# radiocosmology/cora

Hardware: AMD Instinct MI355X
Metric: sky-maps/sec (nside=1024, lmax=2048, 256 freq) (higher is better)
Workload: dtype f64

## Files before the change

### cora_amd/_lib.py

```python
import ctypes
import os

import numpy as np

_HERE = os.path.dirname(os.path.abspath(__file__))
LIB_PATH = os.environ.get("CORAHIP_LIB", os.path.join(_HERE, "libcorahip.so"))

c_int, c_double, c_void_p, c_size_t = ctypes.c_int, ctypes.c_double, ctypes.c_void_p, ctypes.c_size_t
c_u64, c_char_p = ctypes.c_uint64, ctypes.c_char_p
PTR = c_void_p

SIGNATURES = {
    "corahip_abi_version": (c_int, []),
    "corahip_abi_minor": (c_int, []),
    "corahip_last_error": (c_char_p, []),
    "corahip_device_count": (c_int, [ctypes.POINTER(c_int)]),
    "corahip_ctx_create": (c_int, [c_int, ctypes.POINTER(c_void_p)]),
    "corahip_ctx_destroy": (c_int, [c_void_p]),
    "corahip_ctx_set_stream": (c_int, [c_void_p, c_void_p]),
    "corahip_ctx_sync": (c_int, [c_void_p]),
    "corahip_timer_begin": (c_int, [c_void_p]),
    "corahip_timer_end": (c_int, [c_void_p, ctypes.POINTER(ctypes.c_float)]),
    "corahip_profile_enable": (c_int, [c_void_p, c_int]),
    "corahip_profile_get": (c_int, [c_void_p, c_char_p, ctypes.POINTER(c_double), ctypes.POINTER(c_int)]),
    "corahip_profile_reset": (c_int, [c_void_p]),
    "corahip_malloc": (c_int, [c_void_p, c_size_t, ctypes.POINTER(c_void_p)]),
    "corahip_free": (c_int, [c_void_p, c_void_p]),
    "corahip_memcpy_h2d": (c_int, [c_void_p, c_void_p, c_void_p, c_size_t]),
    "corahip_memcpy_d2h": (c_int, [c_void_p, c_void_p, c_void_p, c_size_t]),
    "corahip_clarray_table21cm": (c_int, [c_void_p, PTR, PTR, PTR, c_int, c_int, c_double, c_double, c_double,
                                          PTR, PTR, PTR, PTR, c_int, c_int, PTR, PTR, c_int, PTR]),
    "corahip_clarray_table21cm_pairs": (c_int, [c_void_p, PTR, PTR, PTR, c_int, c_int, c_double, c_double, c_double,
                                                PTR, PTR, PTR, PTR, c_int, c_int, PTR, PTR, c_int, c_int, c_int, c_int,
                                                PTR]),
    "corahip_clarray_pairs_finish": (c_int, [c_void_p, PTR, c_int, c_int, c_int, c_int, PTR]),
    "corahip_clarray_tables_pin": (c_int, [c_void_p, PTR, PTR, PTR, c_u64]),
    "corahip_aps_table21cm_points": (c_int, [c_void_p, PTR, PTR, PTR, c_int, c_int, c_double, c_double, c_double,
                                             ctypes.c_long, PTR, PTR, PTR, PTR, PTR, PTR, PTR]),
    "corahip_clarray_separable": (c_int, [c_void_p, PTR, c_int, PTR, c_int, c_int, PTR, PTR]),
    "corahip_romb_reduce": (c_int, [c_void_p, PTR, c_int, c_int, c_int, PTR, PTR]),
    "corahip_factor_batched": (c_int, [c_void_p, PTR, c_int, c_int, c_double, c_double, PTR, PTR]),
    "corahip_normals_philox": (c_int, [c_void_p, c_u64, c_int, c_int, PTR]),
    "corahip_normals_pcg64": (c_int, [c_void_p, ctypes.POINTER(c_u64), ctypes.POINTER(c_u64), ctypes.c_int64, PTR,
                                      ctypes.POINTER(c_u64)]),
    "corahip_normals_mt19937_legacy": (c_int, [c_void_p, c_void_p, ctypes.c_int64, PTR]),
    "corahip_glibc_exp": (c_int, [c_void_p, PTR, ctypes.c_int64, PTR]),
    "corahip_pcg64_advance": (c_int, [ctypes.POINTER(c_u64), ctypes.POINTER(c_u64), c_u64, ctypes.POINTER(c_u64)]),
    "corahip_draw_alm_philox": (c_int, [c_void_p, PTR, PTR, c_u64, c_int, c_int, c_int, c_int, PTR]),
    "corahip_draw_alm_philox_rows": (c_int, [c_void_p, PTR, PTR, c_u64, c_int, c_int, c_int, c_int, PTR]),
    "corahip_draw_alm": (c_int, [c_void_p, PTR, PTR, PTR, c_int, c_int, c_int, c_int, PTR]),
    "corahip_draw_alm_rows": (c_int, [c_void_p, PTR, PTR, PTR, c_int, c_int, c_int, c_int, PTR]),
    "corahip_draw_alm_numpy_prepare": (c_int, [c_void_p, c_void_p, c_int, c_int, c_size_t, ctypes.POINTER(c_void_p)]),
    "corahip_draw_alm_numpy_run": (c_int, [c_void_p, c_void_p, PTR, c_int, PTR, c_void_p, PTR]),
    "corahip_draw_alm_numpy": (c_int, [c_void_p, PTR, c_int, PTR, c_void_p, c_int, c_int, c_int, c_int, PTR, c_size_t]),
    "corahip_draw_alm_numpy_begin": (c_int, [c_void_p, PTR, c_int, PTR, c_void_p, c_int, c_int, c_int, c_int, PTR, c_size_t,
                                             ctypes.POINTER(c_void_p)]),
    "corahip_draw_alm_numpy_end": (c_int, [c_void_p, c_void_p, c_void_p]),
    "corahip_draw_alm_numpy_begin_set": (c_int, [c_void_p, PTR, PTR, c_void_p, c_int, c_int, c_void_p, PTR, c_size_t,
                                                 ctypes.POINTER(c_void_p)]),
    "corahip_draw_alm_philox_rows_set": (c_int, [c_void_p, PTR, PTR, c_u64, c_int, c_int, c_void_p, PTR]),
    "corahip_mkfullsky_workspace_bytes": (c_int, [c_void_p, c_int, c_int, c_int, c_int, c_int, ctypes.POINTER(c_size_t)]),
    "corahip_mkfullsky": (c_int, [c_void_p, c_void_p, PTR, c_int, c_void_p, c_int, c_int, c_int, PTR, c_void_p, c_size_t]),
    "corahip_shard_plan": (c_int, [c_int, c_int, c_int, c_int, PTR]),
    "corahip_factor_rows_pack": (c_int, [c_void_p, PTR, c_int, c_int, c_int, c_int, PTR]),
    "corahip_factor_rows_unpack": (c_int, [c_void_p, PTR, PTR, c_int, c_int, c_int, c_int, PTR]),
    "corahip_alm_dev_to_square": (c_int, [c_void_p, PTR, c_int, c_int, PTR]),
    "corahip_alm_packed_to_dev": (c_int, [c_void_p, PTR, c_int, c_int, PTR]),
    "corahip_sht_plan_create": (c_int, [c_void_p, c_int, c_int, ctypes.POINTER(c_void_p)]),
    "corahip_sht_plan_create_ex": (c_int, [c_void_p, c_int, c_int, c_int, ctypes.POINTER(c_void_p)]),
    "corahip_sht_plan_cut_exp": (c_int, [c_void_p, ctypes.POINTER(c_int)]),
    "corahip_sht_plan_k4_mfma_count": (c_int, [c_void_p, c_void_p, c_int, ctypes.POINTER(c_u64)]),
    "corahip_sht_plan_destroy": (c_int, [c_void_p, c_void_p]),
    "corahip_alm2map_workspace_bytes": (c_int, [c_void_p, c_int, ctypes.POINTER(c_size_t)]),
    "corahip_alm2map": (c_int, [c_void_p, c_void_p, PTR, c_int, PTR, c_void_p, c_size_t]),
    "corahip_map2alm_workspace_bytes": (c_int, [c_void_p, c_int, ctypes.POINTER(c_size_t)]),
    "corahip_map2alm": (c_int, [c_void_p, c_void_p, PTR, c_int, PTR, PTR, c_void_p, c_size_t]),
    "corahip_alm2map_spin2": (c_int, [c_void_p, c_void_p, PTR, c_int, PTR, c_void_p, c_size_t]),
    "corahip_spin2_ring_scale": (c_int, [c_void_p, c_void_p, PTR, c_int, PTR]),
    "corahip_spin2_combine": (c_int, [c_void_p, c_void_p, PTR, c_int, c_int, PTR, c_int]),
    "corahip_xi_table_average": (c_int, [c_void_p, PTR, PTR, PTR, c_int, c_int, c_double, c_double, PTR, c_int, PTR, PTR,
                                         c_int, c_int, PTR]),
    "corahip_ps_table21cm": (c_int, [c_void_p, PTR, PTR, PTR, c_int, c_int, c_double, PTR, c_int, PTR, c_int, c_double,
                                     PTR, PTR, PTR, PTR]),
    "corahip_dct1_workspace_bytes": (c_int, [ctypes.c_long, c_int, ctypes.POINTER(c_size_t)]),
    "corahip_dct1_rows": (c_int, [c_void_p, PTR, ctypes.c_long, c_int, c_double, c_void_p, c_size_t]),
    "corahip_legendre_project": (c_int, [c_void_p, PTR, PTR, c_int, c_int, PTR, ctypes.c_long, PTR]),
    "corahip_fft_c2c": (c_int, [c_void_p, PTR, c_int, PTR, c_int, c_int]),
    "corahip_irfftn": (c_int, [c_void_p, PTR, c_int, PTR, c_int, PTR]),
    "corahip_rfftn": (c_int, [c_void_p, PTR, c_int, PTR, c_int, PTR]),
    "corahip_randomfield_draw": (c_int, [c_void_p, PTR, ctypes.c_int64, ctypes.c_uint64, PTR]),
    "corahip_fg_mix": (c_int, [c_void_p, PTR, PTR, PTR, c_int, c_int, ctypes.c_int64, PTR]),
    "corahip_randomfield_irfftn": (c_int, [c_void_p, PTR, c_int, PTR, ctypes.c_uint64, PTR, PTR]),
    "corahip_spec_mul_real": (c_int, [c_void_p, PTR, PTR, ctypes.c_int64]),
    "corahip_cube_affine": (c_int, [c_void_p, PTR, PTR, PTR, PTR, PTR, c_int, ctypes.c_int64, PTR]),
    "corahip_raytrace_slices": (c_int, [c_void_p, PTR, c_int, c_int, c_int, PTR, PTR, PTR, PTR, c_double, c_double,
                                        c_int, c_int, c_int, PTR]),
    "corahip_healpix_neighbours": (c_int, [c_void_p, c_int, PTR]),
    "corahip_za_density_sph": (c_int, [c_void_p, PTR, PTR, PTR, PTR, c_int, c_int, c_double, c_double, PTR]),
    "corahip_der1_alm_prep": (c_int, [c_void_p, c_void_p, PTR, c_int, c_int, c_int, PTR]),
    "corahip_der1_combine": (c_int, [c_void_p, c_void_p, PTR, c_int, c_int, PTR, PTR, c_int, PTR, PTR]),
    "corahip_radial_gradient": (c_int, [c_void_p, PTR, PTR, PTR, c_int, ctypes.c_long, PTR]),
    "corahip_sht_plan_rings": (c_int, [c_void_p, PTR, PTR, PTR, PTR]),
    "corahip_sht_plan_ring_classes": (c_int, [c_void_p, PTR]),
    "corahip_sht_lambda": (c_int, [c_void_p, c_void_p, c_int, c_int, PTR]),
    "corahip_sht_lambda_entry": (c_int, [c_void_p, c_void_p, c_int, c_int, c_int, PTR]),
}


class CoraHipError(RuntimeError):

    status = 0


_lib = None


def load():
    global _lib
    if _lib is None:
        if not os.path.exists(LIB_PATH):
            raise ImportError(
                "cora_amd: %s not found. Build it with `make -C cora_amd/csrc` (needs hipcc, gfx950). "
                "There is no CPU fallback for the compute path." % LIB_PATH
            )
        try:
            import torch
        except ImportError:
            pass
        lib = ctypes.CDLL(LIB_PATH)
        for name, (res, args) in SIGNATURES.items():
            fn = getattr(lib, name)
            fn.restype = res
            fn.argtypes = args
        if lib.corahip_abi_version() != 1:
            raise ImportError("cora_amd: ABI version mismatch in %s" % LIB_PATH)
        _lib = lib
    return _lib


def pcg64_advance(state, inc, delta):
    M = 2**64 - 1
    st = (c_u64 * 2)((int(state) >> 64) & M, int(state) & M)
    ic = (c_u64 * 2)((int(inc) >> 64) & M, int(inc) & M)
    out = (c_u64 * 2)()
    _check(load().corahip_pcg64_advance(st, ic, c_u64(int(delta)), out))
    return (int(out[0]) << 64) | int(out[1])


def _check(rc):
    if rc != 0:
        msg = load().corahip_last_error()
        err = CoraHipError("libcorahip status %d: %s" % (rc, msg.decode() if msg else "?"))
        err.status = int(rc)
        raise err


def _torch():
    import torch

    return torch


class _MtState(ctypes.Structure):
    _fields_ = [("key", ctypes.c_uint32 * 624), ("pos", ctypes.c_int32), ("has_gauss", ctypes.c_int32), ("gauss", c_double)]


class _Rng(ctypes.Structure):
    _fields_ = [("kind", ctypes.c_int32), ("reserved", ctypes.c_int32), ("stream", c_void_p), ("seed", c_u64),
                ("state", c_u64 * 2), ("inc", c_u64 * 2), ("legacy", ctypes.POINTER(_MtState))]


class _ChanSet(ctypes.Structure):
    _fields_ = [("nchunks", ctypes.c_int32), ("chunk_nnu", ctypes.c_int32), ("nu0", ctypes.c_int32 * 2)]


def _chanset(chunks):
    cs = _ChanSet()
    chunks = [(int(a), int(n)) for a, n in chunks]
    if len(chunks) not in (1, 2) or (len(chunks) == 2 and chunks[0][1] != chunks[1][1]):
        raise ValueError("a channel set is one block or two equal chunks")
    cs.nchunks, cs.chunk_nnu = len(chunks), chunks[0][1]
    cs.nu0[0] = chunks[0][0]
    cs.nu0[1] = chunks[1][0] if len(chunks) == 2 else 0
    return cs


def _rng_struct(rng):
    r = _Rng()
    M = 2**64 - 1
    if rng[0] == "pcg64":
        r.kind = 2
        r.state[0], r.state[1] = (int(rng[1]) >> 64) & M, int(rng[1]) & M
        r.inc[0], r.inc[1] = (int(rng[2]) >> 64) & M, int(rng[2]) & M
        return r, None
    if rng[0] != "legacy" or rng[1]["bit_generator"] != "MT19937":
        raise ValueError("numpy stream on the device: ('pcg64', state, inc) or ('legacy', MT19937 state dict)")
    ms = _MtState()
    key = np.ascontiguousarray(rng[1]["state"]["key"], dtype=np.uint32)
    ctypes.memmove(ms.key, key.ctypes.data, 624 * 4)
    ms.pos, ms.has_gauss, ms.gauss = int(rng[1]["state"]["pos"]), int(rng[1]["has_gauss"]), float(rng[1]["gauss"])
    r.kind = 3
    r.legacy = ctypes.pointer(ms)
    return r, ms


class Context:

    def __init__(self, device=0):
        torch = _torch()
        self.lib = load()
        if not torch.cuda.is_available():
            raise CoraHipError(
                "cora_amd needs an AMD MI355X (gfx950) GPU: torch.cuda.is_available() is False "
                "and there is no CPU fallback"
            )
        self.device = torch.device("cuda", device)
        torch.cuda.set_device(self.device)
        h = c_void_p()
        _check(self.lib.corahip_ctx_create(device, ctypes.byref(h)))
        self.h = h
        self._plans = {}
        self._workspace = None
        self.use_current_stream()

    def use_current_stream(self):
        torch = _torch()
        s = torch.cuda.current_stream(self.device).cuda_stream
        _check(self.lib.corahip_ctx_set_stream(self.h, c_void_p(s)))

    def sync(self):
        _check(self.lib.corahip_ctx_sync(self.h))

    def timer_begin(self):
        _check(self.lib.corahip_timer_begin(self.h))

    def timer_end(self):
        ms = ctypes.c_float()
        _check(self.lib.corahip_timer_end(self.h, ctypes.byref(ms)))
        return float(ms.value)

    def profile_enable(self, on=True):
        _check(self.lib.corahip_profile_enable(self.h, 1 if on else 0))

    def profile_reset(self):
        _check(self.lib.corahip_profile_reset(self.h))

    def profile_get(self, name):
        ms, n = c_double(), c_int()
        _check(self.lib.corahip_profile_get(self.h, name.encode(), ctypes.byref(ms), ctypes.byref(n)))
        return float(ms.value), int(n.value)

    def empty(self, shape, dtype=None):
        torch = _torch()
        return torch.empty(shape, dtype=dtype or torch.float64, device=self.device)

    def to_device(self, a, dtype=np.float64):
        torch = _torch()
        a = np.ascontiguousarray(a, dtype=dtype)
        return torch.from_numpy(a).to(self.device)

    @staticmethod
    def _p(t):
        assert t.is_contiguous(), "device array must be contiguous"
        return c_void_p(t.data_ptr())

    def _f64(self, t):
        torch = _torch()
        assert t.dtype == torch.float64 and t.device == self.device
        return self._p(t)

    _PINNED_MIN_BYTES = 1 << 24

    @property
    def copy_stream(self):
        torch = _torch()
        if getattr(self, "_copy_stream", None) is None:
            self._copy_stream = torch.cuda.Stream(device=self.device)
        return self._copy_stream

    def to_host_async(self, t):
        torch = _torch()
        host = torch.empty(t.shape, dtype=t.dtype, pin_memory=True)
        ready = torch.cuda.Event()
        ready.record(torch.cuda.current_stream(self.device))
        cs = self.copy_stream
        cs.wait_event(ready)
        with torch.cuda.stream(cs):
            host.copy_(t, non_blocking=True)
            done = torch.cuda.Event()
            done.record(cs)
        t.record_stream(cs)
        return host, done

    def to_host(self, t):
        if t.numel() * t.element_size() < self._PINNED_MIN_BYTES:
            return t.cpu().numpy()
        host, done = self.to_host_async(t)
        done.synchronize()
        return host.numpy()

    def pin_tables(self, dd, dv, vv, generation):
        _check(self.lib.corahip_clarray_tables_pin(self.h, self._f64(dd), self._f64(dv), self._f64(vv), c_u64(int(generation))))

    def unpin_tables(self, generation=0):
        if self.h:
            _check(self.lib.corahip_clarray_tables_pin(self.h, None, None, None, c_u64(int(generation))))

    def clarray_table21cm(self, dd, dv, vv, kperpmin, kperpmax, kparmax, chi, pfd, f, b, F, zint, w, log10l):
        nl = log10l.numel()
        out = self.empty((nl, F, F))
        nkperp, nkpar = dd.shape
        _check(self.lib.corahip_clarray_table21cm(
            self.h, self._f64(dd), self._f64(dv), self._f64(vv), nkperp, nkpar, kperpmin, kperpmax, kparmax,
            self._f64(chi), self._f64(pfd), self._f64(f), self._f64(b), F, zint, self._f64(w), self._f64(log10l),
            nl, self._f64(out)))
        return out

    def clarray_table21cm_pairs(self, dd, dv, vv, kperpmin, kperpmax, kparmax, chi, pfd, f, b, F, zint, w, log10l,
                                pair_first, pair_step, l_block, nblocks=None):
        torch = _torch()
        nl = log10l.numel()
        npl = (F * (F + 1) // 2 + pair_step - 1) // pair_step
        nblk = (nl + l_block - 1) // l_block
        if nblocks is not None:
            assert nblocks >= nblk
            nblk = nblocks
        out = torch.zeros((nblk, npl, l_block), dtype=torch.float64, device=self.device)
        nkperp, nkpar = dd.shape
        _check(self.lib.corahip_clarray_table21cm_pairs(
            self.h, self._f64(dd), self._f64(dv), self._f64(vv), nkperp, nkpar, kperpmin, kperpmax, kparmax,
            self._f64(chi), self._f64(pfd), self._f64(f), self._f64(b), F, zint, self._f64(w), self._f64(log10l),
            nl, pair_first, pair_step, l_block, self._f64(out)))
        return out

    def clarray_pairs_finish(self, slabs, F, nl):
        nranks, npl, l_stride = slabs.shape
        assert npl == (F * (F + 1) // 2 + nranks - 1) // nranks and nl <= l_stride
        out = self.empty((nl, F, F))
        _check(self.lib.corahip_clarray_pairs_finish(self.h, self._f64(slabs), F, nranks, l_stride, nl, self._f64(out)))
        return out

    def aps_table21cm_points(self, dd, dv, vv, kperpmin, kperpmax, kparmax, lx, chi1, chi2, cdd, cdv, cvv):
        n = lx.numel()
        out = self.empty((n,))
        nkperp, nkpar = dd.shape
        _check(self.lib.corahip_aps_table21cm_points(
            self.h, self._f64(dd), self._f64(dv), self._f64(vv), nkperp, nkpar, kperpmin, kperpmax, kparmax, n,
            self._f64(lx), self._f64(chi1), self._f64(chi2), self._f64(cdd), self._f64(cdv), self._f64(cvv),
            self._f64(out)))
        return out

    def clarray_separable(self, al, bcov, F, zint, w):
        nl = al.numel()
        out = self.empty((nl, F, F))
        _check(self.lib.corahip_clarray_separable(self.h, self._f64(al), nl, self._f64(bcov), F, zint,
                                                  self._f64(w), self._f64(out)))
        return out

    def romb_reduce(self, clt, nl, F, zint, w):
        out = self.empty((nl, F, F))
        _check(self.lib.corahip_romb_reduce(self.h, self._f64(clt), nl, F, zint, self._f64(w), self._f64(out)))
        return out

    def ps_table21cm(self, kperp, kpar, spline=None, kstar=0.0, freq_window=0.0, dd=None):
        nkperp, nkpar = kperp.numel(), kpar.numel()
        dv, vv = self.empty((nkperp, nkpar)), self.empty((nkperp, nkpar))
        if dd is None:
            loglog, kx, ky, ky2 = spline
            dd = self.empty((nkperp, nkpar))
            _check(self.lib.corahip_ps_table21cm(self.h, self._f64(kx), self._f64(ky), self._f64(ky2), kx.numel(),
                                                 1 if loglog else 0, float(kstar), self._f64(kperp), nkperp,
                                                 self._f64(kpar), nkpar, float(freq_window), None, self._f64(dd),
                                                 self._f64(dv), self._f64(vv)))
        else:
            _check(self.lib.corahip_ps_table21cm(self.h, None, None, None, 0, 0, 0.0, self._f64(kperp), nkperp,
                                                 self._f64(kpar), nkpar, 0.0, self._f64(dd), None, self._f64(dv),
                                                 self._f64(vv)))
        return dd, dv, vv

    def dct1_rows(self, data, scale=1.0):
        nrows, n = data.shape
        b = c_size_t()
        _check(self.lib.corahip_dct1_workspace_bytes(nrows, n, ctypes.byref(b)))
        ws = self.workspace(int(b.value))
        _check(self.lib.corahip_dct1_rows(self.h, self._f64(data), nrows, n, float(scale), self._p(ws), int(b.value)))
        return data

    def factor_batched(self, C, jitter_rel=1e-14, eig_thresh=1e-16):
        torch = _torch()
        nl, F, F2 = C.shape
        assert F == F2
        T = self.empty((nl, F, F))
        info = torch.empty((nl,), dtype=torch.int32, device=self.device)
        _check(self.lib.corahip_factor_batched(self.h, self._f64(C), nl, F, jitter_rel, eig_thresh, self._f64(T),
                                               self._p(info)))
        return T, info

    def normals_philox(self, seed, lmax, F, out=None):
        n = 2 * F * (lmax + 1) * (lmax + 2) // 2
        g = out if out is not None else self.empty((n,))
        assert g.numel() >= n
        _check(self.lib.corahip_normals_philox(self.h, c_u64(int(seed) & (2**64 - 1)), lmax, F, self._f64(g)))
        return g

    def normals_pcg64(self, state, inc, n, out=None):
        g = out if out is not None else self.empty((n,))
        assert g.numel() >= n
        M = 2**64 - 1
        st = (c_u64 * 2)((int(state) >> 64) & M, int(state) & M)
        ic = (c_u64 * 2)((int(inc) >> 64) & M, int(inc) & M)
        nraw = c_u64(0)
        _check(self.lib.corahip_normals_pcg64(self.h, st, ic, int(n), self._f64(g), ctypes.byref(nraw)))
        return g, int(nraw.value)

    def glibc_exp(self, x):
        y = self.empty(tuple(x.shape))
        _check(self.lib.corahip_glibc_exp(self.h, self._f64(x), int(x.numel()), self._f64(y)))
        return y

    def normals_legacy(self, state, n, out=None):
        import numpy as np

        class MtState(ctypes.Structure):
            _fields_ = [("key", ctypes.c_uint32 * 624), ("pos", ctypes.c_int32), ("has_gauss", ctypes.c_int32),
                        ("gauss", c_double)]

        if state["bit_generator"] != "MT19937":
            raise ValueError("legacy stream on the device: MT19937 only")
        ms = MtState()
        key = np.ascontiguousarray(state["state"]["key"], dtype=np.uint32)
        ctypes.memmove(ms.key, key.ctypes.data, 624 * 4)
        ms.pos, ms.has_gauss, ms.gauss = int(state["state"]["pos"]), int(state["has_gauss"]), float(state["gauss"])
        g = out if out is not None else self.empty((n,))
        assert g.numel() >= n
        _check(self.lib.corahip_normals_mt19937_legacy(self.h, ctypes.byref(ms), int(n), self._f64(g)))
        new = {"bit_generator": "MT19937", "state": {"key": np.frombuffer(ms.key, dtype=np.uint32).copy(), "pos": int(ms.pos)},
               "has_gauss": int(ms.has_gauss), "gauss": float(ms.gauss)}
        return g, new

    def draw_alm(self, T, info, g, lmax, F, nu0=0, nnu=None, out=None):
        nnu = F if nnu is None else nnu
        nalm = (lmax + 1) * (lmax + 2) // 2
        G = (nnu + 3) // 4
        alm = out if out is not None else self.empty((nalm, G, 2, 4))
        _check(self.lib.corahip_draw_alm(self.h, self._f64(T), self._p(info) if info is not None else None,
                                         self._f64(g), lmax, F, nu0, nnu, self._f64(alm)))
        return alm

    def draw_alm_rows(self, T_rows, info, g, lmax, F, nu0, nnu, out=None):
        assert tuple(T_rows.shape) == (lmax + 1, nnu, F), T_rows.shape
        nalm = (lmax + 1) * (lmax + 2) // 2
        G = (nnu + 3) // 4
        alm = out if out is not None else self.empty((nalm, G, 2, 4))
        _check(self.lib.corahip_draw_alm_rows(self.h, self._f64(T_rows), self._p(info) if info is not None else None,
                                              self._f64(g), lmax, F, nu0, nnu, self._f64(alm)))
        return alm

    def draw_alm_numpy_prepare(self, rng, lmax, F, ring_bytes=0):
        r, ms = _rng_struct(rng)
        pend = c_void_p()
        _check(self.lib.corahip_draw_alm_numpy_prepare(self.h, ctypes.byref(r), int(lmax), int(F), int(ring_bytes), ctypes.byref(pend)))
        ctx = self

        class Prepared:
            rng_struct, mt_state, pending, shape, live = r, ms, pend, (int(lmax), int(F)), True

            def abort(self):
                if self.live:
                    self.live = False
                    _check(ctx.lib.corahip_draw_alm_numpy_end(ctx.h, self.pending, ctypes.byref(self.rng_struct)))

        return Prepared()

    def draw_alm_numpy(self, T, info, rng, lmax, F, nu0=0, nnu=None, out=None, rows=False, ring_bytes=0, defer=False,
                       chunks=None, prepared=None):
        import numpy as np

        if chunks is not None:
            rows, nu0, nnu = True, chunks[0][0], sum(c[1] for c in chunks)
        nnu = F if nnu is None else nnu
        assert tuple(T.shape) == ((lmax + 1, nnu, F) if rows else (lmax + 1, F, F)), T.shape
        nalm = (lmax + 1) * (lmax + 2) // 2
        alm = out if out is not None else self.empty((nalm, (nnu + 3) // 4, 2, 4))
        if prepared is not None:
            assert prepared.live and prepared.shape == (int(lmax), int(F)), "the prepared session is for another shape"
            r, ms, pend = prepared.rng_struct, prepared.mt_state, prepared.pending
            cs = _chanset(chunks if chunks is not None and len(chunks) > 1 else [(nu0, nnu)])
            prepared.live = False
            try:
                _check(self.lib.corahip_draw_alm_numpy_run(self.h, pend, self._f64(T), 1 if rows else 0,
                                                           self._p(info) if info is not None else None, ctypes.byref(cs), self._f64(alm)))
            except CoraHipError:
                self.lib.corahip_draw_alm_numpy_end(self.h, pend, ctypes.byref(r))
                raise
        else:
            r, ms = _rng_struct(rng)
            pend = c_void_p()
            if chunks is not None and len(chunks) > 1:
                cs = _chanset(chunks)
                _check(self.lib.corahip_draw_alm_numpy_begin_set(self.h, self._f64(T), self._p(info) if info is not None else None,
                                                                 ctypes.byref(r), lmax, F, ctypes.byref(cs), self._f64(alm),
                                                                 int(ring_bytes), ctypes.byref(pend)))
            else:
                _check(self.lib.corahip_draw_alm_numpy_begin(self.h, self._f64(T), 1 if rows else 0,
                                                             self._p(info) if info is not None else None, ctypes.byref(r), lmax,
                                                             F, nu0, nnu, self._f64(alm), int(ring_bytes), ctypes.byref(pend)))
        keep = [T, info, alm]

        def finish():
            _check(self.lib.corahip_draw_alm_numpy_end(self.h, pend, ctypes.byref(r)))
            keep.clear()
            if ms is not None:
                return {"bit_generator": "MT19937", "state": {"key": np.frombuffer(ms.key, dtype=np.uint32).copy(), "pos": int(ms.pos)},
                        "has_gauss": int(ms.has_gauss), "gauss": float(ms.gauss)}
            return (int(r.state[0]) << 64) | int(r.state[1])

        if defer:
            return alm, finish
        return alm, finish()

    def draw_alm_philox(self, T, info, seed, lmax, F, nu0=0, nnu=None, out=None):
        nnu = F if nnu is None else nnu
        nalm = (lmax + 1) * (lmax + 2) // 2
        G = (nnu + 3) // 4
        alm = out if out is not None else self.empty((nalm, G, 2, 4))
        _check(self.lib.corahip_draw_alm_philox(self.h, self._f64(T), self._p(info) if info is not None else None,
                                                c_u64(int(seed) & (2**64 - 1)), lmax, F, nu0, nnu, self._f64(alm)))
        return alm

    def draw_alm_philox_rows(self, T_rows, info, seed, lmax, F, nu0, nnu, out=None):
        assert tuple(T_rows.shape) == (lmax + 1, nnu, F), T_rows.shape
        nalm = (lmax + 1) * (lmax + 2) // 2
        G = (nnu + 3) // 4
        alm = out if out is not None else self.empty((nalm, G, 2, 4))
        _check(self.lib.corahip_draw_alm_philox_rows(self.h, self._f64(T_rows), self._p(info) if info is not None else None,
                                                     c_u64(int(seed) & (2**64 - 1)), lmax, F, nu0, nnu, self._f64(alm)))
        return alm

    def draw_alm_philox_chunks(self, T_rows, info, seed, lmax, F, chunks, out=None):
        nnu = sum(int(c[1]) for c in chunks)
        assert tuple(T_rows.shape) == (lmax + 1, nnu, F), T_rows.shape
        nalm = (lmax + 1) * (lmax + 2) // 2
        alm = out if out is not None else self.empty((nalm, (nnu + 3) // 4, 2, 4))
        cs = _chanset(chunks)
        _check(self.lib.corahip_draw_alm_philox_rows_set(self.h, self._f64(T_rows), self._p(info) if info is not None else None,
                                                         c_u64(int(seed) & (2**64 - 1)), lmax, F, ctypes.byref(cs),
                                                         self._f64(alm)))
        return alm

    def factor_rows_pack(self, T_local, l_stride, world):
        n_local, F, _ = T_local.shape
        send = self.empty((world, l_stride, F // world, F))
        _check(self.lib.corahip_factor_rows_pack(self.h, self._f64(T_local) if n_local else None, n_local, l_stride, F,
                                                 world, self._f64(send)))
        return send

    def factor_rows_unpack(self, recv, counts):
        world, l_stride, nnu, F = recv.shape
        cnt = (ctypes.c_int32 * world)(*[int(c) for c in counts])
        out = self.empty((int(sum(counts)), nnu, F))
        _check(self.lib.corahip_factor_rows_unpack(self.h, self._f64(recv), cnt, world, l_stride, nnu, F, self._f64(out)))
        return out

    def alm_dev_to_square(self, alm, lmax, nnu):
        torch = _torch()
        L = lmax + 1
        sq = torch.empty((nnu, 1, L, L), dtype=torch.complex128, device=self.device)
        _check(self.lib.corahip_alm_dev_to_square(self.h, self._f64(alm), lmax, nnu, self._p(sq)))
        return sq

    def alm_packed_to_dev(self, packed, lmax):
        torch = _torch()
        assert packed.dtype == torch.complex128
        nnu, nalm = packed.shape
        assert nalm == (lmax + 1) * (lmax + 2) // 2
        alm = self.empty((nalm, (nnu + 3) // 4, 2, 4))
        _check(self.lib.corahip_alm_packed_to_dev(self.h, self._p(packed), lmax, nnu, self._f64(alm)))
        return alm

    sht_cut_exp = 0

    def sht_plan(self, nside, lmax, cut_exp=None):
        cut = int(self.sht_cut_exp if cut_exp is None else cut_exp)
        key = (int(nside), int(lmax)) if cut == 0 else (int(nside), int(lmax), cut)
        if key not in self._plans:
            h = c_void_p()
            _check(self.lib.corahip_sht_plan_create_ex(self.h, key[0], key[1], cut, ctypes.byref(h)))
            self._plans[key] = h
        return self._plans[key]

    def k4_mfma_count(self, nside, lmax, nnu, cut_exp=None):
        n = c_u64()
        _check(self.lib.corahip_sht_plan_k4_mfma_count(self.h, self.sht_plan(nside, lmax, cut_exp), int(nnu), ctypes.byref(n)))
        return int(n.value)

    def alm2map_workspace_bytes(self, plan, nnu):
        b = c_size_t()
        _check(self.lib.corahip_alm2map_workspace_bytes(plan, nnu, ctypes.byref(b)))
        return int(b.value)

    def workspace(self, nbytes):
        torch = _torch()
        if self._workspace is None or self._workspace.numel() < nbytes:
            self._workspace = None
            self._workspace = torch.empty((nbytes,), dtype=torch.uint8, device=self.device)
        return self._workspace

    def alm2map(self, alm, nside, lmax, nnu, out=None, max_workspace_bytes=None, cut_exp=None):
        plan = self.sht_plan(nside, lmax, cut_exp)
        npix = 12 * nside * nside
        maps = out if out is not None else self.empty((nnu, npix))
        need = self.alm2map_workspace_bytes(plan, nnu)
        if max_workspace_bytes is not None:
            need = min(need, int(max_workspace_bytes))
        ws = self.workspace(need)
        _check(self.lib.corahip_alm2map(self.h, plan, self._f64(alm), nnu, self._f64(maps), self._p(ws), need))
        return maps

    def mkfullsky_fused(self, C, nside, rng, nu0=0, nnu=None, alms=False, workspace_bytes=None, workspace=None):
        torch = _torch()
        L, F = int(C.shape[0]), int(C.shape[1])
        lmax = L - 1
        nnu = F if nnu is None else nnu
        plan = self.sht_plan(nside, lmax)

        class MtState(ctypes.Structure):
            _fields_ = [("key", ctypes.c_uint32 * 624), ("pos", ctypes.c_int32), ("has_gauss", ctypes.c_int32),
                        ("gauss", c_double)]

        class Rng(ctypes.Structure):
            _fields_ = [("kind", ctypes.c_int32), ("reserved", ctypes.c_int32), ("stream", c_void_p), ("seed", c_u64),
                        ("state", c_u64 * 2), ("inc", c_u64 * 2), ("legacy", ctypes.POINTER(MtState))]

        r = Rng()
        M = 2**64 - 1
        kind = {"stream": 0, "philox": 1, "pcg64": 2, "legacy": 3}[rng[0]]
        ms = None
        if kind == 3:
            import numpy as np

            ms = MtState()
            key = np.ascontiguousarray(rng[1]["state"]["key"], dtype=np.uint32)
            ctypes.memmove(ms.key, key.ctypes.data, 624 * 4)
            ms.pos, ms.has_gauss, ms.gauss = int(rng[1]["state"]["pos"]), int(rng[1]["has_gauss"]), float(rng[1]["gauss"])
            r.legacy = ctypes.pointer(ms)
        r.kind = kind
        if kind == 0:
            r.stream = self._f64(rng[1])
        elif kind == 1:
            r.seed = int(rng[1]) & M
        elif kind == 2:
            r.state[0], r.state[1] = (int(rng[1]) >> 64) & M, int(rng[1]) & M
            r.inc[0], r.inc[1] = (int(rng[2]) >> 64) & M, int(rng[2]) & M
        b = c_size_t()
        _check(self.lib.corahip_mkfullsky_workspace_bytes(plan, F, nu0, nnu, kind, 1 if alms else 0, ctypes.byref(b)))
        need = int(b.value) if workspace_bytes is None else int(workspace_bytes)
        if workspace is None:
            ws = torch.empty((max(need, 1),), dtype=torch.uint8, device=self.device)
        else:
            ws = workspace
            assert ws.dtype == torch.uint8 and ws.device == self.device and ws.numel() >= need, (ws.numel(), need)
        out = (torch.empty((nnu, 1, L, L), dtype=torch.complex128, device=self.device) if alms
               else self.empty((nnu, 12 * nside * nside)))
        _check(self.lib.corahip_mkfullsky(self.h, plan, self._f64(C), F, ctypes.byref(r), nu0, nnu, 1 if alms else 0,
                                          c_void_p(out.data_ptr()), self._p(ws), need))
        if kind == 3:
            import numpy as np

            return out, {"bit_generator": "MT19937", "state": {"key": np.frombuffer(ms.key, dtype=np.uint32).copy(), "pos": int(ms.pos)},
                         "has_gauss": int(ms.has_gauss), "gauss": float(ms.gauss)}
        return out, ((int(r.state[0]) << 64) | int(r.state[1])) if kind == 2 else None

    def map2alm_workspace_bytes(self, plan, nnu):
        b = c_size_t()
        _check(self.lib.corahip_map2alm_workspace_bytes(plan, nnu, ctypes.byref(b)))
        return int(b.value)

    def map2alm(self, maps, nside, lmax, ring_w=None, chunk=None, out=None):
        torch = _torch()
        plan = self.sht_plan(nside, lmax)
        nnu, npix = maps.shape
        assert npix == 12 * nside * nside
        nalm = (lmax + 1) * (lmax + 2) // 2
        G4 = (nnu + 3) // 4
        if chunk is None:
            per8 = self.map2alm_workspace_bytes(plan, 8)
            chunk = max(8, min((int(96e9 // per8)) * 8, (nnu + 7) // 8 * 8))
        assert chunk % 8 == 0
        if out is None:
            out = self.empty((nalm, G4, 2, 4))
        assert tuple(out.shape) == (nalm, G4, 2, 4), out.shape
        for c0 in range(0, nnu, chunk):
            n = min(chunk, nnu - c0)
            G8 = (n + 7) // 8 * 2
            need = self.map2alm_workspace_bytes(plan, n)
            ws = self.workspace(need)
            part = out if (c0 == 0 and n == nnu and G8 == G4) else self.empty((nalm, G8, 2, 4))
            _check(self.lib.corahip_map2alm(self.h, plan, self._f64(maps[c0:c0 + n]), n,
                                            self._f64(ring_w) if ring_w is not None else None, self._f64(part),
                                            self._p(ws), need))
            if part is not out:
                g0 = c0 // 4
                gn = min(G8, G4 - g0)
                out[:, g0:g0 + gn].copy_(part[:, :gn])
        return out

    def alm2map_spin2(self, alm, nside, lmax, nnu, out=None):
        plan = self.sht_plan(nside, lmax)
        maps = out if out is not None else self.empty((nnu, 12 * nside * nside))
        need = self.alm2map_workspace_bytes(plan, nnu)
        ws = self.workspace(need)
        _check(self.lib.corahip_alm2map_spin2(self.h, plan, self._f64(alm), nnu, self._f64(maps), self._p(ws), need))
        return maps

    def map2alm_spin2(self, maps_qu, nside, lmax, ring_w=None, out=None):
        plan = self.sht_plan(nside, lmax)
        n2, npix = maps_qu.shape
        assert n2 % 2 == 0 and npix == 12 * nside * nside
        nf = n2 // 2
        nalm = (lmax + 1) * (lmax + 2) // 2
        maps6 = self.empty((6 * nf, npix))
        _check(self.lib.corahip_spin2_ring_scale(self.h, plan, self._f64(maps_qu), nf, self._f64(maps6)))
        a6 = self.map2alm(maps6, nside, lmax, ring_w)
        del maps6
        gout = (2 * nf + 7) // 8 * 2
        if out is None:
            out = self.empty((nalm, gout, 2, 4))
        assert tuple(out.shape) == (nalm, gout, 2, 4), out.shape
        _check(self.lib.corahip_spin2_combine(self.h, plan, self._f64(a6), a6.shape[1], nf, self._f64(out), gout))
        return out

    def der1_alm_prep(self, alm, nside, lmax, g0=0, g_in=None, out=None):
        plan = self.sht_plan(nside, lmax)
        nalm = (lmax + 1) * (lmax + 2) // 2
        G = int(alm.shape[1])
        g_in = G - g0 if g_in is None else int(g_in)
        assert tuple(alm.shape) == (nalm, G, 2, 4), alm.shape
        a3 = out if out is not None else self.empty((nalm, 3 * g_in, 2, 4))
        assert tuple(a3.shape) == (nalm, 3 * g_in, 2, 4), a3.shape
        _check(self.lib.corahip_der1_alm_prep(self.h, plan, self._f64(alm), G, int(g0), g_in, self._f64(a3)))
        return a3

    def der1_combine(self, maps3, nside, lmax, g_in, nfields, out_theta, out_phi, scale_theta=None, scale_phi=None,
                     phi_extra=0):
        plan = self.sht_plan(nside, lmax)
        npix = 12 * nside * nside
        assert tuple(maps3.shape) == (12 * g_in, npix), maps3.shape
        assert tuple(out_theta.shape) == (nfields, npix) and tuple(out_phi.shape) == (nfields, npix)
        for s in (scale_theta, scale_phi):
            assert s is None or s.numel() == nfields
        _check(self.lib.corahip_der1_combine(self.h, plan, self._f64(maps3), int(g_in), int(nfields),
                                             None if scale_theta is None else self._f64(scale_theta),
                                             None if scale_phi is None else self._f64(scale_phi), int(phi_extra),
                                             self._f64(out_theta), self._f64(out_phi)))
        return out_theta, out_phi

    def alm2map_der1_bytes(self, nside, lmax, nfields=16):
        g = (int(nfields) + 3) // 4
        nalm = (lmax + 1) * (lmax + 2) // 2
        ws = self.alm2map_workspace_bytes(self.sht_plan(nside, lmax), 12 * g)
        return nalm * 3 * g * 64 + 12 * g * 12 * nside * nside * 8 + ws

    def alm2map_der1(self, alm, nside, lmax, nnu, scale_theta=None, scale_phi=None, phi_extra=0, out=None,
                     max_bytes=None):
        npix = 12 * nside * nside
        G = int(alm.shape[1])
        assert 1 <= nnu <= 4 * G
        if out is None:
            out = (self.empty((nnu, npix)), self.empty((nnu, npix)))
        ot, op = out
        assert tuple(ot.shape) == (nnu, npix) and tuple(op.shape) == (nnu, npix)
        budget = self.alm2map_der1_bytes(nside, lmax, 16) if max_bytes is None else int(max_bytes)
        gall = (nnu + 3) // 4
        gc = gall
        while gc > 1 and self.alm2map_der1_bytes(nside, lmax, 4 * gc) > budget:
            gc -= 1
        plan = self.sht_plan(nside, lmax)
        for g0 in range(0, gall, gc):
            g = min(gc, gall - g0)
            f0, nf = 4 * g0, min(4 * g, nnu - 4 * g0)
            a3 = self.der1_alm_prep(alm, nside, lmax, g0, g)
            maps3 = self.empty((12 * g, npix))
            need = self.alm2map_workspace_bytes(plan, 12 * g)
            ws = self.workspace(need)
            _check(self.lib.corahip_alm2map(self.h, plan, self._f64(a3), 12 * g, self._f64(maps3), self._p(ws), need))
            del a3
            self.der1_combine(maps3, nside, lmax, g, nf, ot[f0:f0 + nf], op[f0:f0 + nf],
                              None if scale_theta is None else scale_theta[f0:f0 + nf],
                              None if scale_phi is None else scale_phi[f0:f0 + nf], phi_extra)
            del maps3
        return ot, op

    @staticmethod
    def gradient_coefficients(x):
        x = np.asarray(x, dtype=np.float64)
        n = x.size
        if x.ndim != 1 or n < 2:
            raise ValueError("gradient needs at least 2 coordinates along the axis (got shape %r)" % (x.shape,))
        d = np.diff(x)
        coef = np.zeros((n, 3))
        hs, hd = d[:-1], d[1:]
        coef[1:-1, 0] = -hd / (hs * (hd + hs))
        coef[1:-1, 1] = (hd - hs) / (hd * hs)
        coef[1:-1, 2] = hs / (hd * (hd + hs))
        coef[0, 1], coef[0, 2] = -1.0 / d[0], 1.0 / d[0]
        coef[-1, 0], coef[-1, 1] = -1.0 / d[-1], 1.0 / d[-1]
        return coef

    def radial_gradient(self, f, x, scale=None, out=None):
        torch = _torch()
        if f.dim() != 2:
            raise ValueError("radial_gradient takes a [n, npix] array (got %r)" % (tuple(f.shape),))
        n, npix = f.shape
        coef = self.gradient_coefficients(x)
        if coef.shape[0] != n:
            raise ValueError("x has %d entries, f %d rows" % (coef.shape[0], n))
        if out is None:
            out = self.empty((n, npix))
        if tuple(out.shape) != (n, npix):
            raise ValueError("out has shape %r, expected %r" % (tuple(out.shape), (n, npix)))
        nbytes = n * npix * 8
        if out.data_ptr() < f.data_ptr() + nbytes and f.data_ptr() < out.data_ptr() + nbytes:
            raise ValueError("radial_gradient: out overlaps f")
        if scale is not None and not isinstance(scale, torch.Tensor):
            scale = self.to_device(np.asarray(scale, dtype=np.float64))
        if scale is not None and scale.numel() != n:
            raise ValueError("scale has %d entries, f %d rows" % (scale.numel(), n))
        cdev = self.to_device(coef)
        _check(self.lib.corahip_radial_gradient(self.h, self._f64(f), self._f64(cdev),
                                                None if scale is None else self._f64(scale), int(n), int(npix),
                                                self._f64(out)))
        return out

    def xi_table_average(self, kx, ky, ky2, kind, x_t, f_t, mu, xa, xw, F, xint):
        nm = mu.numel()
        out = self.empty((nm, F, F))
        _check(self.lib.corahip_xi_table_average(self.h, self._f64(kx), self._f64(ky), self._f64(ky2), kx.numel(), kind,
                                                 float(x_t), float(f_t), self._f64(mu), nm, self._f64(xa), self._f64(xw),
                                                 F, xint, self._f64(out)))
        return out

    def legendre_project(self, mu, wt, lmax, xi):
        nm = mu.numel()
        ncol = xi.numel() // nm
        out = self.empty((lmax + 1, ncol))
        _check(self.lib.corahip_legendre_project(self.h, self._f64(mu), self._f64(wt), nm, lmax, self._f64(xi),
                                                 ncol, self._f64(out)))
        return out

    def _c128(self, t):
        torch = _torch()
        assert t.dtype == torch.complex128 and t.device == self.device
        return self._p(t)

    @staticmethod
    def _dims(shape):
        return (ctypes.c_int64 * len(shape))(*[int(x) for x in shape])

    def fft_c2c(self, data, axis, inverse=False):
        axis = axis % data.dim()
        _check(self.lib.corahip_fft_c2c(self.h, self._c128(data), data.dim(), self._dims(data.shape), axis,
                                        1 if inverse else 0))
        return data

    def irfftn(self, spec, naxes=None, last=None):
        nd = spec.dim()
        naxes = nd if naxes is None else naxes
        rshape = list(spec.shape)
        rshape[-1] = 2 * (spec.shape[-1] - 1) if last is None else int(last)
        if rshape[-1] // 2 + 1 != spec.shape[-1]:
            raise CoraHipError("irfftn: last axis %d does not match %d spectral bins" % (rshape[-1], spec.shape[-1]))
        out = self.empty(tuple(rshape))
        _check(self.lib.corahip_irfftn(self.h, self._c128(spec), nd, self._dims(rshape), naxes, self._f64(out)))
        return out

    def rfftn(self, arr, naxes=None):
        torch = _torch()
        nd = arr.dim()
        naxes = nd if naxes is None else naxes
        cshape = list(arr.shape)
        cshape[-1] = arr.shape[-1] // 2 + 1
        spec = torch.empty(tuple(cshape), dtype=torch.complex128, device=self.device)
        _check(self.lib.corahip_rfftn(self.h, self._f64(arr), nd, self._dims(arr.shape), naxes, self._c128(spec)))
        return spec

    def randomfield_draw(self, kweight, seed):
        torch = _torch()
        spec = torch.empty(tuple(kweight.shape), dtype=torch.complex128, device=self.device)
        _check(self.lib.corahip_randomfield_draw(self.h, self._f64(kweight), kweight.numel(), int(seed),
                                                 self._c128(spec)))
        return spec

    def randomfield_irfftn(self, kweight, seed, last=None, spec=None):
        torch = _torch()
        nd = kweight.dim()
        rshape = list(kweight.shape)
        rshape[-1] = 2 * (kweight.shape[-1] - 1) if last is None else int(last)
        if rshape[-1] // 2 + 1 != kweight.shape[-1]:
            raise CoraHipError("randomfield_irfftn: last axis %d does not match %d spectral bins" % (rshape[-1], kweight.shape[-1]))
        if spec is None:
            spec = torch.empty(tuple(kweight.shape), dtype=torch.complex128, device=self.device)
        out = self.empty(tuple(rshape))
        _check(self.lib.corahip_randomfield_irfftn(self.h, self._f64(kweight), nd, self._dims(rshape), int(seed) & (2**64 - 1),
                                                   self._c128(spec), self._f64(out)))
        return out

    def fg_mix(self, freq_weight, normals, aff):
        torch = _torch()
        F, ncorr = freq_weight.shape
        assert normals.shape[0] == ncorr and tuple(normals.shape[1:]) == tuple(aff.shape)
        out = torch.empty((F,) + tuple(aff.shape), dtype=torch.complex128, device=self.device)
        _check(self.lib.corahip_fg_mix(self.h, self._f64(freq_weight), self._f64(normals), self._c128(aff), F, ncorr,
                                       aff.numel(), self._c128(out)))
        return out

    def spec_mul_real(self, spec, weight):
        assert tuple(spec.shape) == tuple(weight.shape)
        _check(self.lib.corahip_spec_mul_real(self.h, self._c128(spec), self._f64(weight), spec.numel()))
        return spec

    def cube_affine(self, df, vf, a, b, c):
        n0 = df.shape[0]
        out = self.empty(tuple(df.shape))
        _check(self.lib.corahip_cube_affine(self.h, self._f64(df), None if vf is None else self._f64(vf), self._f64(a),
                                            None if vf is None else self._f64(b), self._f64(c), n0, df.numel() // n0,
                                            self._f64(out)))
        return out

    def raytrace_slices(self, cube, zc, scale, tx, ty, wx, wy):
        n0, n1, n2 = cube.shape
        numz, numx, numy = zc.numel(), tx.numel(), ty.numel()
        out = self.empty((numz, numx, numy))
        _check(self.lib.corahip_raytrace_slices(self.h, self._f64(cube), n0, n1, n2, self._f64(zc), self._f64(scale),
                                                self._f64(tx), self._f64(ty), float(wx), float(wy), numz, numx, numy,
                                                self._f64(out)))
        return out

    def healpix_neighbours(self, nside):
        torch = _torch()
        out = torch.empty((12 * int(nside) ** 2, 9), dtype=torch.int32, device=self.device)
        _check(self.lib.corahip_healpix_neighbours(self.h, int(nside), self._p(out)))
        return out

    def za_density_sph(self, psi, delta_bias, delta_m, chi, out, sigma_ang, sigma_chi):
        nchi, npix = delta_bias.shape
        nside = int(round((npix // 12) ** 0.5))
        _check(self.lib.corahip_za_density_sph(self.h, self._f64(psi), self._f64(delta_bias), self._f64(delta_m),
                                               self._f64(chi), int(nchi), nside, float(sigma_ang), float(sigma_chi),
                                               self._f64(out)))
        return out

    def sht_rings(self, nside, lmax):
        plan = self.sht_plan(nside, lmax)
        nring = 4 * nside - 1
        start = np.zeros(nring, dtype=np.int64)
        nphi = np.zeros(nring, dtype=np.int32)
        z = np.zeros(nring)
        phi0 = np.zeros(nring)
        _check(self.lib.corahip_sht_plan_rings(plan, start.ctypes.data_as(c_void_p), nphi.ctypes.data_as(c_void_p),
                                               z.ctypes.data_as(c_void_p), phi0.ctypes.data_as(c_void_p)))
        return dict(start=start, nphi=nphi, z=z, phi0=phi0)

    def sht_ring_classes(self, nside, lmax):
        cls = np.zeros(4 * nside - 1, dtype=np.int32)
        _check(self.lib.corahip_sht_plan_ring_classes(self.sht_plan(nside, lmax), cls.ctypes.data_as(c_void_p)))
        return cls

    def sht_lambda(self, nside, lmax, m, ring_pair):
        plan = self.sht_plan(nside, lmax)
        out = self.empty((lmax - m + 1,))
        _check(self.lib.corahip_sht_lambda(self.h, plan, m, ring_pair, self._f64(out)))
        return out

    def sht_lambda_entry(self, nside, lmax, m, ring_pair, kq):
        plan = self.sht_plan(nside, lmax)
        out = self.empty((lmax - m + 1,))
        _check(self.lib.corahip_sht_lambda_entry(self.h, plan, m, ring_pair, kq, self._f64(out)))
        return out


_contexts = {}


def get_context(device=None):
    torch = _torch()
    if device is None:
        device = torch.cuda.current_device() if torch.cuda.is_available() else 0
    if device not in _contexts:
        _contexts[device] = Context(device)
    ctx = _contexts[device]
    ctx.use_current_stream()
    return ctx
```

### cora_amd/csrc/clarray.hip

```cpp
#include "common.h"

#include <cstring>
#include <type_traits>

#ifndef CL_BUILD_BY_ROW
#define CL_BUILD_BY_ROW 1
#endif
#ifndef CL_BUILD_X4
#define CL_BUILD_X4 1
#endif
#ifndef CL_ABLATE
#define CL_ABLATE 0
#endif
#define CL_MAXZ 17

#define CL_XS 512
#define CL_LPT 9

__global__ void cl_transpose_kernel(const double *__restrict__ dd, const double *__restrict__ dv,
                                    const double *__restrict__ vv, int nkperp, int nkpar, double *__restrict__ tt) {
    __shared__ double tile[32][33];
    const double *src = blockIdx.z == 0 ? dd : (blockIdx.z == 1 ? dv : vv);
    double *dst = tt + (size_t)blockIdx.z * nkpar * CL_XS;
    const int x0 = blockIdx.y * 32, y0 = blockIdx.x * 32;
    const int tx = threadIdx.x & 31, ty = threadIdx.x >> 5;
    for (int r = ty; r < 32; r += 8) {
        const int x = x0 + r, y = y0 + tx;
        tile[r][tx] = (x < nkperp && y < nkpar) ? src[(size_t)x * nkpar + y] : 0.0;
    }
    __syncthreads();
    for (int r = ty; r < 32; r += 8) {
        const int y = y0 + r, x = x0 + tx;
        if (y < nkpar && x < CL_XS) dst[(size_t)y * CL_XS + x] = (x < nkperp) ? tile[tx][r] : 0.0;
    }
}

template <int ZINT>
__global__ void __launch_bounds__(256)
clarray21_kernel(const double *__restrict__ tt, int nkperp, int nkpar, double kperpmin, double xscale, double yscale,
                 const double *__restrict__ chi, const double *__restrict__ pfd, const double *__restrict__ fz,
                 const double *__restrict__ bz, int F, int zint_rt, const double *__restrict__ w,
                 const double *__restrict__ log10l, int nl, int l_base, const int2 *__restrict__ pairs,
                 double *__restrict__ scratch, int nl_total, int l_block) {
    const int zint = ZINT > 0 ? ZINT : zint_rt;
    extern __shared__ __attribute__((aligned(16))) double sm[];
    double *prof = sm;
    double *lxcs_s = sm + zint * (CL_XS + 2);
    double *par = lxcs_s + zint;
    int *ipar = reinterpret_cast<int *>(par + zint * zint * 8);
    const int PS = CL_XS + 2;
    const int tid = threadIdx.x;
    const int i = pairs[blockIdx.x].x, j = pairs[blockIdx.x].y;
    if (i < 0) return;
    const double ux = (double)nkperp - 1e-5, uy = (double)nkpar - 1e-5;
    const size_t tsz = (size_t)nkpar * CL_XS;

    double lxs[CL_LPT], acc[CL_LPT];
#pragma unroll
    for (int k = 0; k < CL_LPT; k++) {
        const int li = l_base + tid + 256 * k;
        lxs[k] = log10l[min(li, nl_total - 1)] * xscale;
        acc[k] = 0.0;
    }
    const int l_end = min(nl_total, l_base + 256 * CL_LPT);
    const double lx_lo = log10l[l_base] * xscale, lx_hi = log10l[l_end - 1] * xscale;
    const int kmax = (l_end - l_base + 255) / 256;

    int noclamp = 1;
    for (int t = tid; t < zint * zint; t += 256) {
        const int a = t / zint, b = t - a * zint;
        const int za = i * zint + a, zb = j * zint + b;
        const double x1 = chi[za], x2 = chi[zb];
        const double xc = 0.5 * (x1 + x2);
        const double lxc = log10(xc * kperpmin) * xscale;
        double yy = fabs(x2 - x1) * yscale;
        yy = yy < 0.0 ? 0.0 : (yy > uy ? uy : yy);
        int y0 = (int)yy;
        double wy = yy - (double)y0;
        if (y0 + 1 > nkpar - 1) {
            y0 = nkpar - 2;
            wy = 1.0;
        }
        const double W = w[a] * w[b] * pfd[za] * pfd[zb] / (xc * xc * M_PI);
        const double cdd = W * bz[za] * bz[zb];
        const double cdv = W * (fz[za] * bz[zb] + fz[zb] * bz[za]);
        const double cvv = W * fz[za] * fz[zb];
        double *pp = par + t * 8;
        pp[0] = cdd * (1.0 - wy);
        pp[1] = cdd * wy;
        pp[2] = cdv * (1.0 - wy);
        pp[3] = cdv * wy;
        pp[4] = cvv * (1.0 - wy);
        pp[5] = cvv * wy;
        pp[6] = lxc;
        double xhi = lx_hi - lxc, xlo = lx_lo - lxc;
        xhi = xhi < 0.0 ? 0.0 : (xhi > ux ? ux : xhi);
        xlo = xlo < 0.0 ? 0.0 : (xlo > ux ? ux : xlo);
        ipar[t * 4 + 0] = y0;
        ipar[t * 4 + 1] = (int)xlo;
        ipar[t * 4 + 2] = min((int)xhi + 2, nkperp);
        const double x2nd = (l_base + 1 < l_end ? log10l[l_base + 1] * xscale : lx_hi) - lxc;
        if (!(x2nd >= 0.0 && lx_hi - lxc <= ux)) noclamp = 0;
    }
    const bool all_fast = __syncthreads_and(noclamp) != 0;
    __shared__ int s_nsp;
    __shared__ double s_lxk[32];
    if (tid < 32) s_lxk[tid] = log10l[min(l_base + tid, nl_total - 1)] * xscale;
    if (tid < 64) {
        bool wide = false;
        if (l_base + tid + 1 < l_end) wide = (log10l[l_base + tid + 1] - log10l[l_base + tid]) * xscale >= 2.0;
        const unsigned long long m = __ballot(wide);
        if (tid == 0) s_nsp = m == ~0ull ? 32 : min(32, (int)__builtin_ctzll(~m));
    }

    for (int a = 0; a < zint; a++) {
        __syncthreads();
#if (CL_ABLATE == 0 || CL_ABLATE >= 3) && CL_BUILD_BY_ROW
        if (ZINT > 0 && all_fast) {
            constexpr int ZN = ZINT > 0 ? ZINT : 1;
            const int nsp = min(s_nsp, l_end - l_base);
            const double lxd = log10l[min(l_base + nsp, nl_total - 1)] * xscale;
            int xlo = nkperp, xhi = 0;
#pragma unroll
            for (int b = 0; b < ZN; b++) {
                const double xx = fmin(fmax(lxd - par[(a * ZN + b) * 8 + 6], 0.0), ux);
                xlo = min(xlo, (int)xx);
                xhi = max(xhi, ipar[(a * ZN + b) * 4 + 2]);
            }
            if (nsp >= l_end - l_base) xlo = xhi;
            auto row_of = [&](int b, int x, double (&v)[6]) {
                const double *r0 = tt + (size_t)ipar[(a * ZN + b) * 4 + 0] * CL_XS + x, *r1 = r0 + CL_XS;
                v[0] = r0[0];
                v[1] = r1[0];
                v[2] = r0[tsz];
                v[3] = r1[tsz];
                v[4] = r0[2 * tsz];
                v[5] = r1[2 * tsz];
            };
            auto combine = [&](int b, const double (&v)[6]) {
                const double *pp = par + (a * ZN + b) * 8;
                return pp[0] * v[0] + pp[1] * v[1] + pp[2] * v[2] + pp[3] * v[3] + pp[4] * v[4] + pp[5] * v[5];
            };
#if CL_BUILD_X4
            {
                constexpr int ZH = (ZN + 1) / 2;
                const int hb = tid >> 7, b0 = hb ? ZH : 0, nb = hb ? ZN - ZH : ZH;
                constexpr int QB = 3;
                for (int x = (xlo & ~1) + 2 * (tid & 127); x < xhi; x += 256) {
#pragma unroll
                    for (int q0 = 0; q0 < ZH; q0 += QB) {
                        double2 v[QB][6];
#pragma unroll
                        for (int q = 0; q < QB; q++) {
#if CL_ABLATE >= 3
                            if (q0 + q < nb) {
                                for (int i6 = 0; i6 < 6; i6++) v[q][i6] = make_double2((double)x, 1.0 + i6);
                            } else
#endif
                            if (q0 + q < nb) {
                                const double *r0 = tt + (size_t)ipar[(a * ZN + b0 + q0 + q) * 4 + 0] * CL_XS + x, *r1 = r0 + CL_XS;
                                v[q][0] = *reinterpret_cast<const double2 *>(r0);
                                v[q][1] = *reinterpret_cast<const double2 *>(r1);
                                v[q][2] = *reinterpret_cast<const double2 *>(r0 + tsz);
                                v[q][3] = *reinterpret_cast<const double2 *>(r1 + tsz);
                                v[q][4] = *reinterpret_cast<const double2 *>(r0 + 2 * tsz);
                                v[q][5] = *reinterpret_cast<const double2 *>(r1 + 2 * tsz);
                            }
                        }
#pragma unroll
                        for (int q = 0; q < QB; q++) {
                            if (q0 + q < nb) {
                                const double *pp = par + (a * ZN + b0 + q0 + q) * 8;
                                double2 o;
                                o.x = pp[0] * v[q][0].x + pp[1] * v[q][1].x + pp[2] * v[q][2].x + pp[3] * v[q][3].x + pp[4] * v[q][4].x + pp[5] * v[q][5].x;
                                o.y = pp[0] * v[q][0].y + pp[1] * v[q][1].y + pp[2] * v[q][2].y + pp[3] * v[q][3].y + pp[4] * v[q][4].y + pp[5] * v[q][5].y;
                                *reinterpret_cast<double2 *>(prof + (b0 + q0 + q) * PS + x) = o;
                            }
                        }
                    }
                }
            }
#else
            for (int x = xlo + tid; x < xhi; x += 256) {
                double v[ZN][6];
#pragma unroll
                for (int b = 0; b < ZN; b++) row_of(b, x, v[b]);
#pragma unroll
                for (int b = 0; b < ZN; b++) prof[b * PS + x] = combine(b, v[b]);
            }
#endif
            for (int e = tid; e < nsp * ZN; e += 256) {
                const int b = e % ZN, k = e / ZN;
                const double xx = fmin(fmax(s_lxk[k] - par[(a * ZN + b) * 8 + 6], 0.0), ux);
                const int x = (int)xx;
                typedef double d2u __attribute__((ext_vector_type(2), aligned(8)));
                const double *r0 = tt + (size_t)ipar[(a * ZN + b) * 4 + 0] * CL_XS + x, *r1 = r0 + CL_XS;
                const d2u t0 = *reinterpret_cast<const d2u *>(r0), t1 = *reinterpret_cast<const d2u *>(r1);
                const d2u t2 = *reinterpret_cast<const d2u *>(r0 + tsz), t3 = *reinterpret_cast<const d2u *>(r1 + tsz);
                const d2u t4 = *reinterpret_cast<const d2u *>(r0 + 2 * tsz), t5 = *reinterpret_cast<const d2u *>(r1 + 2 * tsz);
                const double v0[6] = {t0.x, t1.x, t2.x, t3.x, t4.x, t5.x};
                const double v1[6] = {t0.y, t1.y, t2.y, t3.y, t4.y, t5.y};
                const double p0 = combine(b, v0);
                prof[b * PS + x] = p0;
                prof[b * PS + x + 1] = x + 1 < nkperp ? combine(b, v1) : p0;
            }
            if (tid < ZN) lxcs_s[tid] = par[(a * ZN + tid) * 8 + 6];
            if (xhi == nkperp) {
                __syncthreads();
                if (tid < ZN) prof[tid * PS + nkperp] = prof[tid * PS + nkperp - 1];
            }
        } else
#endif
        for (int b = 0; b < zint; b++) {
            const int t = a * zint + b;
            const double *pp = par + t * 8;
            const double c0 = pp[0], c1 = pp[1], c2 = pp[2], c3 = pp[3], c4 = pp[4], c5 = pp[5];
            const int y0 = ipar[t * 4 + 0], x0r = ipar[t * 4 + 1], nx = ipar[t * 4 + 2];
            const double *r0 = tt + (size_t)y0 * CL_XS, *r1 = r0 + CL_XS;
            double *pb = prof + b * PS;
#if CL_ABLATE == 1
            for (int x = x0r + tid; x < nx; x += 256) pb[x] = c0 + c1 * x;
            (void)r0; (void)r1; (void)c2; (void)c3; (void)c4; (void)c5;
#else
            for (int x = x0r + tid; x < nx; x += 256)
                pb[x] = c0 * r0[x] + c1 * r1[x] + c2 * r0[tsz + x] + c3 * r1[tsz + x] + c4 * r0[2 * tsz + x] +
                        c5 * r1[2 * tsz + x];
#endif
            if (tid == 0) lxcs_s[b] = pp[6];
            if (nx == nkperp && tid == ((nkperp - 1 - x0r) & 255)) pb[nkperp] = pb[nkperp - 1];
        }
        __syncthreads();
        double lxc_r[ZINT > 0 ? ZINT : 1];
        if constexpr (ZINT > 0) {
#pragma unroll
            for (int b = 0; b < ZINT; b++) lxc_r[b] = lxcs_s[b];
        }
        auto interp = [&](int b, double lx, double lxc, bool clamp) {
            double xx = lx - lxc;
            if (clamp) xx = fmin(fmax(xx, 0.0), ux);
            const int x0 = (int)xx;
            const double wx = __builtin_amdgcn_fract(xx);
            const double *pr = prof + b * PS + x0;
            const double s0 = pr[0], s1 = pr[1];
            return fma(wx, s1 - s0, s0);
        };
        auto interp_all = [&](auto fast_c) {
            constexpr bool FAST = decltype(fast_c)::value;
#pragma unroll
            for (int k = 0; k < CL_LPT; k++) {
#if CL_ABLATE == 2 || CL_ABLATE == 4
                if (k >= 1) continue;
#endif
                if (k < kmax && (k < kmax - 1 || l_base + tid + 256 * k < nl_total)) {
                    const bool clamp = !FAST || (k == 0 && tid == 0);
                    double s = 0.0;
                    if constexpr (ZINT > 0) {
#pragma unroll
                        for (int b = 0; b < ZINT; b++) s += interp(b, lxs[k], lxc_r[b], clamp);
                    } else {
                        for (int b = 0; b < zint; b++) s += interp(b, lxs[k], lxcs_s[b], clamp);
                    }
                    acc[k] += s;
                }
            }
        };
        if (all_fast) interp_all(std::true_type{});
        else interp_all(std::false_type{});
    }
#pragma unroll
    for (int k = 0; k < CL_LPT; k++) {
        const int li = l_base + tid + 256 * k;
        if (li < nl_total)
            scratch[((size_t)(li / l_block) * gridDim.x + blockIdx.x) * l_block + li % l_block] = acc[k];
    }
}

#define CL_BAND 32
#ifndef CL_XCD_ORDER
#define CL_XCD_ORDER 1
#endif
__host__ __device__ static inline long cl_band_count(int n) {
    return n >= CL_BAND ? (long)CL_BAND * (n - (CL_BAND - 1)) + (long)(CL_BAND - 1) * CL_BAND / 2 : (long)n * (n + 1) / 2;
}
__host__ __device__ static inline int2 pair_of_index(long p, int F) {
    int B = 0;
    for (;; B++) {
        const long c = cl_band_count(F - CL_BAND * B);
        if (p < c) break;
        p -= c;
    }
    const int n = F - CL_BAND * B;
    const int nfull = n >= CL_BAND ? n - (CL_BAND - 1) : 0;
    int i, dd;
    if (p < (long)nfull * CL_BAND) {
#if CL_XCD_ORDER
        const int xq = (int)(p & 7), sq = (int)(p >> 3);
        i = sq >> 2;
        dd = 4 * xq + (sq & 3);
#else
        i = (int)(p / CL_BAND);
        dd = (int)(p % CL_BAND);
#endif
    } else {
        p -= (long)nfull * CL_BAND;
        int e = n >= CL_BAND ? CL_BAND - 1 : n;
        i = nfull;
        while (p >= e) {
            p -= e;
            e--;
            i++;
        }
        dd = (int)p;
    }
    return make_int2(i, i + CL_BAND * B + dd);
}

__global__ void cl_finish_kernel(const double *__restrict__ scratch, long npairs, int W, long npl, int lstride, int nl,
                                 int F, double *__restrict__ out) {
    __shared__ double tile[32][33];
    const long s0 = (long)blockIdx.x * 32;
    const int l0 = blockIdx.y * 32;
    const int tx = threadIdx.x & 31, ty = threadIdx.x >> 5;
    const long nslot = npl * W;
    for (int r = ty; r < 32; r += 8) {
        const long sl = s0 + r;
        const int l = l0 + tx;
        tile[r][tx] = (sl < nslot && l < nl) ? scratch[(size_t)sl * lstride + l] : 0.0;
    }
    __syncthreads();
    const long sl = s0 + tx;
    const long p = sl < nslot ? (sl % npl) * W + sl / npl : npairs;
    if (p >= npairs) return;
    const int2 ij = pair_of_index(p, F);
    for (int r = ty; r < 32; r += 8) {
        const int l = l0 + r;
        if (l < nl) {
            out[((size_t)l * F + ij.x) * F + ij.y] = tile[tx][r];
        }
    }
}

__global__ void cl_mirror_kernel(double *__restrict__ out, int F) {
    __shared__ double tile[32][33];
    const int nt = (F + 31) / 32;
    int ti = 0, rem = blockIdx.x;
    while (rem >= nt - ti) {
        rem -= nt - ti;
        ti++;
    }
    const int tj = ti + rem;
    double *o = out + (size_t)blockIdx.y * F * F;
    const int tx = threadIdx.x & 31, ty = threadIdx.x >> 5;
    for (int r = ty; r < 32; r += 8) {
        const int i = ti * 32 + r, j = tj * 32 + tx;
        tile[r][tx] = (i < F && j < F) ? o[(size_t)i * F + j] : 0.0;
    }
    __syncthreads();
    for (int r = ty; r < 32; r += 8) {
        const int j = tj * 32 + r, i = ti * 32 + tx;
        if (j < F && i < F && j > i) o[(size_t)j * F + i] = tile[tx][r];
    }
}
static int launch_mirror(corahip_ctx *ctx, double *out, int nl, int F) {
    const int nt = (F + 31) / 32;
    dim3 grid((unsigned)(nt * (nt + 1) / 2), (unsigned)nl);
    cl_mirror_kernel<<<grid, 256, 0, ctx->stream>>>(out, F);
    LAUNCH_CHECK();
    return 0;
}

__global__ void separable_kernel(const double *__restrict__ al, int nl, const double *__restrict__ bcov, int F, int zint,
                                 const double *__restrict__ w, double *__restrict__ out) {
    const long n = (long)nl * F * F;
    const int nz = F * zint;
    for (long q = (long)blockIdx.x * blockDim.x + threadIdx.x; q < n; q += (long)gridDim.x * blockDim.x) {
        const int j = (int)(q % F), i = (int)((q / F) % F);
        const long l = q / ((long)F * F);
        double s = 0.0;
        for (int a = 0; a < zint; a++) {
            double t = 0.0;
            for (int b = 0; b < zint; b++) t += w[b] * bcov[(size_t)(i * zint + a) * nz + j * zint + b];
            s += w[a] * t;
        }
        out[q] = al[l] * s;
    }
}

__global__ void romb_reduce_kernel(const double *__restrict__ clt, int nl, int F, int zint,
                                   const double *__restrict__ w, double *__restrict__ out) {
    const long n = (long)nl * F * F;
    for (long q = (long)blockIdx.x * blockDim.x + threadIdx.x; q < n; q += (long)gridDim.x * blockDim.x) {
        const int j = (int)(q % F), i = (int)((q / F) % F);
        const long l = q / ((long)F * F);
        const double *base = clt + (((size_t)l * F + i) * zint * F + j) * zint;
        double s = 0.0;
        for (int a = 0; a < zint; a++) {
            double t = 0.0;
            for (int b = 0; b < zint; b++) t += w[b] * base[(size_t)a * F * zint + b];
            s += w[a] * t;
        }
        out[q] = s;
    }
}

__global__ void aps21_points_kernel(const double *__restrict__ dd, const double *__restrict__ dv,
                                    const double *__restrict__ vv, int nkperp, int nkpar, double kperpmin,
                                    double xscale, double yscale, long n, const double *__restrict__ lx,
                                    const double *__restrict__ chi1, const double *__restrict__ chi2,
                                    const double *__restrict__ cdd, const double *__restrict__ cdv,
                                    const double *__restrict__ cvv, double *__restrict__ out) {
    const double ux = (double)nkperp - 1e-5, uy = (double)nkpar - 1e-5;
    for (long q = (long)blockIdx.x * blockDim.x + threadIdx.x; q < n; q += (long)gridDim.x * blockDim.x) {
        const double x1 = chi1[q], x2 = chi2[q];
        const double xc = 0.5 * (x1 + x2);
        double xx = (lx[q] - log10(xc * kperpmin)) * xscale;
        double yy = fabs(x2 - x1) * yscale;
        xx = xx < 0.0 ? 0.0 : (xx > ux ? ux : xx);
        yy = yy < 0.0 ? 0.0 : (yy > uy ? uy : yy);
        const int x0 = (int)xx, y0 = (int)yy;
        const double wx = xx - (double)x0, wy = yy - (double)y0;
        const int xb = min(x0 + 1, nkperp - 1), yb = min(y0 + 1, nkpar - 1);
        const size_t o00 = (size_t)x0 * nkpar + y0, o01 = (size_t)x0 * nkpar + yb;
        const size_t o10 = (size_t)xb * nkpar + y0, o11 = (size_t)xb * nkpar + yb;
        const double wa = (1.0 - wx) * (1.0 - wy), wb = (1.0 - wx) * wy, wc = wx * (1.0 - wy), wd = wx * wy;
        const double vdd = wa * dd[o00] + wb * dd[o01] + wc * dd[o10] + wd * dd[o11];
        const double vdv = wa * dv[o00] + wb * dv[o01] + wc * dv[o10] + wd * dv[o11];
        const double vvv = wa * vv[o00] + wb * vv[o01] + wc * vv[o10] + wd * vv[o11];
        out[q] = (cdd[q] * vdd + cdv[q] * vdv + cvv[q] * vvv) / (xc * xc * M_PI);
    }
}

extern "C" {

static int clarray21_pairs(corahip_ctx *ctx, const double *dd, const double *dv, const double *vv, int nkperp,
                           int nkpar, double kperpmin, double kperpmax, double kparmax, const double *chi,
                           const double *pfd, const double *f, const double *b, int F, int zint, const double *w,
                           const double *log10l, int nl, int pair_first, int pair_step, long npl_pad, int l_block,
                           double *out_pairs) {
    const size_t tt_bytes = sizeof(double) * 3 * (size_t)nkpar * CL_XS;
    double *tt = nullptr;
    int2 *dpairs = nullptr;
    int rc;
    if ((rc = corahip_ctx_scratch(ctx, 0, tt_bytes, (void **)&tt))) return rc;
    if ((rc = corahip_ctx_scratch(ctx, 2, sizeof(int2) * npl_pad, (void **)&dpairs))) return rc;
    const long key[4] = {F, pair_first, pair_step, npl_pad};
    if (ctx->pairs_ptr != (void *)dpairs || memcmp(key, ctx->pairs_key, sizeof(key)) != 0) {
        std::vector<int2> pairs((size_t)npl_pad, make_int2(-1, -1));
        long p = 0, k = 0;
        const long npairs_all = (long)F * (F + 1) / 2;
        for (; p < npairs_all; p++)
            if (p >= pair_first && (p - pair_first) % pair_step == 0) pairs[(size_t)k++] = pair_of_index(p, F);
        HIP_TRY(hipMemcpyAsync(dpairs, pairs.data(), sizeof(int2) * npl_pad, hipMemcpyHostToDevice, ctx->stream));
        HIP_TRY(hipStreamSynchronize(ctx->stream));
        memcpy(ctx->pairs_key, key, sizeof(key));
        ctx->pairs_ptr = (void *)dpairs;
    }
    const bool pinned = ctx->tt_pinned && ctx->tt_pin[0] == dd && ctx->tt_pin[1] == dv && ctx->tt_pin[2] == vv;
    if (!(pinned && ctx->tt_valid && ctx->tt_stream == ctx->stream && ctx->scratch_bytes[0] == tt_bytes)) {
        dim3 grid((nkpar + 31) / 32, CL_XS / 32, 3);
        cl_transpose_kernel<<<grid, 256, 0, ctx->stream>>>(dd, dv, vv, nkperp, nkpar, tt);
        LAUNCH_CHECK();
        ctx->tt_valid = pinned;
        ctx->tt_stream = ctx->stream;
    }
    const double xscale = (double)(nkperp - 1) / log10(kperpmax / kperpmin);
    const double yscale = kparmax / M_PI;
    const size_t shm = sizeof(double) * ((size_t)zint * (CL_XS + 2) + zint + (size_t)zint * zint * 10);
    auto kern = zint == 9 ? clarray21_kernel<9> : (zint == 5 ? clarray21_kernel<5> : (zint == 3 ? clarray21_kernel<3> : clarray21_kernel<0>));
    HIP_TRY(hipFuncSetAttribute((const void *)kern, hipFuncAttributeMaxDynamicSharedMemorySize, (int)shm));
    for (int l_base = 0; l_base < nl; l_base += 256 * CL_LPT) {
        kern<<<(unsigned)npl_pad, 256, shm, ctx->stream>>>(tt, nkperp, nkpar, kperpmin, xscale, yscale, chi, pfd, f, b, F, zint, w,
                                                          log10l, nl, l_base, dpairs, out_pairs, nl, l_block);
        LAUNCH_CHECK();
    }
    return 0;
}

int corahip_clarray_tables_pin(corahip_ctx *ctx, const double *dd, const double *dv, const double *vv, uint64_t generation) {
    ARG_CHECK(ctx != nullptr);
    if (dd == nullptr && generation != 0 && !(ctx->tt_pinned && ctx->tt_pin_gen == generation))
        return 0;
    const bool same = ctx->tt_pinned && dd && ctx->tt_pin[0] == dd && ctx->tt_pin[1] == dv && ctx->tt_pin[2] == vv &&
                      ctx->tt_pin_gen == generation;
    if (same) return 0;
    ctx->tt_pin[0] = dd;
    ctx->tt_pin[1] = dv;
    ctx->tt_pin[2] = vv;
    ctx->tt_pin_gen = generation;
    ctx->tt_pinned = dd != nullptr;
    ctx->tt_valid = false;
    return 0;
}

int corahip_clarray_table21cm(corahip_ctx *ctx, const double *dd, const double *dv, const double *vv, int nkperp,
                              int nkpar, double kperpmin, double kperpmax, double kparmax, const double *chi,
                              const double *pfd, const double *f, const double *b, int F, int zint, const double *w,
                              const double *log10l, int nl, double *out) {
    ARG_CHECK(ctx != nullptr && dd && dv && vv && chi && pfd && f && b && w && log10l && out);
    ARG_CHECK(nkperp >= 2 && nkperp < CL_XS && nkpar >= 2 && F >= 1 && zint >= 1 && zint <= CL_MAXZ && nl >= 1);
    ARG_CHECK(kperpmin > 0 && kperpmax > kperpmin && kparmax > 0);
    StageTimer t(ctx, "clarray");
    const long npairs = (long)F * (F + 1) / 2;
    double *scratch = nullptr;
    int rc;
    if ((rc = corahip_ctx_scratch(ctx, 1, sizeof(double) * (size_t)npairs * nl, (void **)&scratch))) return rc;
    if ((rc = clarray21_pairs(ctx, dd, dv, vv, nkperp, nkpar, kperpmin, kperpmax, kparmax, chi, pfd, f, b, F, zint, w,
                              log10l, nl, 0, 1, npairs, nl, scratch)))
        return rc;
    dim3 grid((unsigned)((npairs + 31) / 32), (nl + 31) / 32);
    cl_finish_kernel<<<grid, 256, 0, ctx->stream>>>(scratch, npairs, 1, npairs, nl, nl, F, out);
    LAUNCH_CHECK();
    return launch_mirror(ctx, out, nl, F);
}

int corahip_clarray_table21cm_pairs(corahip_ctx *ctx, const double *dd, const double *dv, const double *vv, int nkperp,
                                    int nkpar, double kperpmin, double kperpmax, double kparmax, const double *chi,
                                    const double *pfd, const double *f, const double *b, int F, int zint,
                                    const double *w, const double *log10l, int nl, int pair_first, int pair_step,
                                    int l_block, double *out_pairs) {
    ARG_CHECK(ctx != nullptr && dd && dv && vv && chi && pfd && f && b && w && log10l && out_pairs);
    ARG_CHECK(nkperp >= 2 && nkperp < CL_XS && nkpar >= 2 && F >= 1 && zint >= 1 && zint <= CL_MAXZ && nl >= 1);
    ARG_CHECK(kperpmin > 0 && kperpmax > kperpmin && kparmax > 0);
    ARG_CHECK(pair_step >= 1 && pair_first >= 0 && pair_first < pair_step && l_block >= 1);
    StageTimer t(ctx, "clarray");
    const long npairs = (long)F * (F + 1) / 2;
    const long npl = (npairs + pair_step - 1) / pair_step;
    return clarray21_pairs(ctx, dd, dv, vv, nkperp, nkpar, kperpmin, kperpmax, kparmax, chi, pfd, f, b, F, zint, w,
                           log10l, nl, pair_first, pair_step, npl, l_block, out_pairs);
}

int corahip_clarray_pairs_finish(corahip_ctx *ctx, const double *pairs_in, int F, int nranks, int l_stride, int nl,
                                 double *out) {
    ARG_CHECK(ctx != nullptr && pairs_in && out && F >= 1 && nranks >= 1 && nl >= 1 && l_stride >= nl);
    StageTimer t(ctx, "clarray");
    const long npairs = (long)F * (F + 1) / 2;
    const long npl = (npairs + nranks - 1) / nranks;
    dim3 grid((unsigned)((npl * nranks + 31) / 32), (nl + 31) / 32);
    cl_finish_kernel<<<grid, 256, 0, ctx->stream>>>(pairs_in, npairs, nranks, npl, l_stride, nl, F, out);
    LAUNCH_CHECK();
    return launch_mirror(ctx, out, nl, F);
}

int corahip_clarray_separable(corahip_ctx *ctx, const double *al, int nl, const double *bcov, int F, int zint,
                              const double *w, double *out) {
    ARG_CHECK(ctx != nullptr && al && bcov && w && out && nl >= 1 && F >= 1 && zint >= 1);
    StageTimer t(ctx, "clarray");
    const long n = (long)nl * F * F;
    separable_kernel<<<(int)std::min<long>((n + 255) / 256, 4096), 256, 0, ctx->stream>>>(al, nl, bcov, F, zint, w, out);
    LAUNCH_CHECK();
    return 0;
}

int corahip_romb_reduce(corahip_ctx *ctx, const double *clt, int nl, int F, int zint, const double *w, double *out) {
    ARG_CHECK(ctx != nullptr && clt && w && out && nl >= 1 && F >= 1 && zint >= 1);
    StageTimer t(ctx, "clarray");
    const long n = (long)nl * F * F;
    romb_reduce_kernel<<<(int)std::min<long>((n + 255) / 256, 4096), 256, 0, ctx->stream>>>(clt, nl, F, zint, w, out);
    LAUNCH_CHECK();
    return 0;
}

int corahip_aps_table21cm_points(corahip_ctx *ctx, const double *dd, const double *dv, const double *vv, int nkperp,
                                 int nkpar, double kperpmin, double kperpmax, double kparmax, long n,
                                 const double *lx, const double *chi1, const double *chi2, const double *cdd,
                                 const double *cdv, const double *cvv, double *out) {
    ARG_CHECK(ctx != nullptr && dd && dv && vv && lx && chi1 && chi2 && cdd && cdv && cvv && out);
    ARG_CHECK(nkperp >= 2 && nkpar >= 2 && n >= 1 && kperpmin > 0 && kperpmax > kperpmin && kparmax > 0);
    StageTimer t(ctx, "clarray");
    const double xscale = (double)(nkperp - 1) / log10(kperpmax / kperpmin);
    const double yscale = kparmax / M_PI;
    aps21_points_kernel<<<(int)std::min<long>((n + 255) / 256, 4096), 256, 0, ctx->stream>>>(
        dd, dv, vv, nkperp, nkpar, kperpmin, xscale, yscale, n, lx, chi1, chi2, cdd, cdv, cvv, out);
    LAUNCH_CHECK();
    return 0;
}

}
```

### cora_amd/csrc/factor.hip

```cpp
#include "common.h"

#include <algorithm>
#include <vector>

#define CH_NB 32

__global__ void __launch_bounds__(256)
chol_kernel(const double *__restrict__ C, int F, double jitter_rel, double *__restrict__ T,
            int32_t *__restrict__ info) {
    extern __shared__ __attribute__((aligned(16))) double lds[];
    double *D = lds;
    double *PA = lds + CH_NB * (CH_NB + 1);
    double *PB = PA + 64 * (CH_NB + 1);
    double *red = PB + 64 * (CH_NB + 1);
    int *flag = reinterpret_cast<int *>(red + 256);

    const int tid = threadIdx.x;
    const size_t off = (size_t)blockIdx.x * F * F;
    const double *A = C + off;
    double *Tl = T + off;

    double dmax = -INFINITY;
    for (int i = tid; i < F; i += 256) dmax = fmax(dmax, A[(size_t)i * F + i]);
    red[tid] = dmax;
    if (tid == 0) *flag = 0;
    __syncthreads();
    for (int s = 128; s > 0; s >>= 1) {
        if (tid < s) red[tid] = fmax(red[tid], red[tid + s]);
        __syncthreads();
    }
    const double jit = red[0] * jitter_rel;
    __syncthreads();
    for (long q = tid; q < (long)F * F; q += 256) {
        const int i = (int)(q / F), j = (int)(q % F);
        double v = 0.0;
        if (j <= i) v = A[q] + (i == j ? jit : 0.0);
        Tl[q] = v;
    }
    __syncthreads();

    for (int kb = 0; kb < F; kb += CH_NB) {
        const int nb = min(CH_NB, F - kb);
        for (int q = tid; q < nb * nb; q += 256) {
            const int i = q / nb, j = q % nb;
            D[i * (CH_NB + 1) + j] = (j <= i) ? Tl[(size_t)(kb + i) * F + kb + j] : 0.0;
        }
        __syncthreads();
        if (tid < 64) {
            const int lane = tid;
            double row[CH_NB];
#pragma unroll
            for (int k = 0; k < CH_NB; k++) row[k] = (lane < nb && k <= lane) ? D[lane * (CH_NB + 1) + k] : 0.0;
            bool bad = false;
#pragma unroll
            for (int j = 0; j < CH_NB; j++) {
                if (j < nb && !bad) {
                    const double d = __shfl(row[j], j);
                    if (!(d > 0.0)) {
                        bad = true;
                    } else {
                        const double lij = row[j] / sqrt(d);
                        row[j] = lane == j ? sqrt(d) : lij;
#pragma unroll
                        for (int k = j + 1; k < CH_NB; k++) row[k] -= lij * __shfl(lij, k);
                    }
                }
            }
#pragma unroll
            for (int k = 0; k < CH_NB; k++)
                if (lane < nb && k <= lane) D[lane * (CH_NB + 1) + k] = row[k];
            if (bad && lane == 0) *flag = 1;
        }
        __syncthreads();
        if (*flag) break;
        for (int q = tid; q < nb * nb; q += 256) {
            const int i = q / nb, j = q % nb;
            if (j <= i) Tl[(size_t)(kb + i) * F + kb + j] = D[i * (CH_NB + 1) + j];
        }
        const int r0 = kb + nb;
        if (r0 >= F) break;
        for (int r = r0 + tid; r < F; r += 256) {
            double x[CH_NB];
            double *row = Tl + (size_t)r * F + kb;
#pragma unroll
            for (int j = 0; j < CH_NB; j++) x[j] = j < nb ? row[j] : 0.0;
#pragma unroll
            for (int j = 0; j < CH_NB; j++) {
                if (j < nb) {
                    double s = x[j];
#pragma unroll
                    for (int p = 0; p < CH_NB; p++)
                        if (p < j) s -= x[p] * D[j * (CH_NB + 1) + p];
                    x[j] = s / D[j * (CH_NB + 1) + j];
                }
            }
#pragma unroll
            for (int j = 0; j < CH_NB; j++)
                if (j < nb) row[j] = x[j];
        }
        __syncthreads();
        const int nt = (F - r0 + 63) / 64;
        for (int ti = 0; ti < nt; ti++) {
            const int i0 = r0 + ti * 64;
            for (int q = tid; q < 64 * CH_NB; q += 256) {
                const int rr = q / CH_NB, cc = q % CH_NB;
                PA[rr * (CH_NB + 1) + cc] = (i0 + rr < F && cc < nb) ? Tl[(size_t)(i0 + rr) * F + kb + cc] : 0.0;
            }
            for (int tj = 0; tj <= ti; tj++) {
                const int j0 = r0 + tj * 64;
                for (int q = tid; q < 64 * CH_NB; q += 256) {
                    const int rr = q / CH_NB, cc = q % CH_NB;
                    PB[rr * (CH_NB + 1) + cc] = (j0 + rr < F && cc < nb) ? Tl[(size_t)(j0 + rr) * F + kb + cc] : 0.0;
                }
                const int ty = tid >> 4, tx = tid & 15;
                double old[4][4];
#pragma unroll
                for (int u = 0; u < 4; u++)
#pragma unroll
                    for (int w = 0; w < 4; w++) {
                        const int i = i0 + ty + 16 * u, j = j0 + tx + 16 * w;
                        old[u][w] = (i < F && j <= i) ? Tl[(size_t)i * F + j] : 0.0;
                    }
                __syncthreads();
                double acc[4][4] = {};
                for (int p = 0; p < CH_NB; p++) {
                    double a[4], b[4];
#pragma unroll
                    for (int u = 0; u < 4; u++) {
                        a[u] = PA[(ty + 16 * u) * (CH_NB + 1) + p];
                        b[u] = PB[(tx + 16 * u) * (CH_NB + 1) + p];
                    }
#pragma unroll
                    for (int u = 0; u < 4; u++)
#pragma unroll
                        for (int w = 0; w < 4; w++) acc[u][w] += a[u] * b[w];
                }
#pragma unroll
                for (int u = 0; u < 4; u++)
#pragma unroll
                    for (int w = 0; w < 4; w++) {
                        const int i = i0 + ty + 16 * u, j = j0 + tx + 16 * w;
                        if (i < F && j <= i) Tl[(size_t)i * F + j] = old[u][w] - acc[u][w];
                    }
                __syncthreads();
            }
        }
    }
    if (tid == 0) info[blockIdx.x] = *flag;
}

#define CHM_S 34
#ifndef CHM_STAMPS
#define CHM_STAMPS 0
#endif
#if CHM_STAMPS
__device__ unsigned long long g_chm_stamps[8];
#define CSTAMP(k) { unsigned long long _t; asm volatile("s_memtime %0\n\ts_waitcnt lgkmcnt(0)" : "=s"(_t)::"memory"); c_acc[k] += _t - c_last; c_last = _t; }
#else
#define CSTAMP(k)
#endif
#ifndef CHM_ABLATE
#define CHM_ABLATE 0
#endif

template <bool TALL>
__global__ void __launch_bounds__(256)
chol_ll_kernel(const double *__restrict__ C, int F, double jitter_rel, double *__restrict__ T,
               int32_t *__restrict__ info) {
    extern __shared__ __attribute__((aligned(16))) double lds[];
    double *D = lds;
    double *red = lds + CH_NB * (CH_NB + 1);
    int *flag = reinterpret_cast<int *>(red + 256);
    double *rdiag = red + 256 + 2;
    double *stage = rdiag + CH_NB;

    const int tid = threadIdx.x, lane = tid & 63, wave = tid >> 6;
    const int ri = lane & 15, kq = lane >> 4;
    const size_t off = (size_t)blockIdx.x * F * F;
    const double *A = C + off;
    double *Tl = T + off;
    double *PA = stage + (size_t)wave * (TALL ? 1 : 2) * 32 * CHM_S, *PB = PA + 32 * CHM_S;
    double *PBS = stage + 4 * 32 * CHM_S;

    double dmax = -INFINITY;
    for (int i = tid; i < F; i += 256) dmax = fmax(dmax, A[(size_t)i * F + i]);
    red[tid] = dmax;
    if (tid == 0) *flag = 0;
    __syncthreads();
    for (int s = 128; s > 0; s >>= 1) {
        if (tid < s) red[tid] = fmax(red[tid], red[tid + s]);
        __syncthreads();
    }
    const double jit = red[0] * jitter_rel;
    __syncthreads();

#if CHM_STAMPS
    unsigned long long c_acc[8] = {0, 0, 0, 0, 0, 0, 0, 0}, c_last;
    { unsigned long long _t; asm volatile("s_memtime %0\n\ts_waitcnt lgkmcnt(0)" : "=s"(_t)::"memory"); c_last = _t; }
#endif
    const int nblk = (F + 31) / 32;
    const int srow = lane >> 1, scol = 16 * (lane & 1);
    auto load_block = [&](int row0, int col0, double2 (&v)[8]) {
        const double *src = Tl + (size_t)(row0 + srow < F ? row0 + srow : 0) * F + col0 + scol;
#pragma unroll
        for (int q = 0; q < 8; q++) v[q] = *reinterpret_cast<const double2 *>(src + 2 * q);
    };
    auto store_block = [&](double *P, const double2 (&v)[8], double sign, int row0) {
        const double sg = row0 + srow < F ? sign : 0.0;
#pragma unroll
        for (int q = 0; q < 8; q++)
            *reinterpret_cast<double2 *>(P + srow * CHM_S + scol + 2 * q) = make_double2(sg * v[q].x, sg * v[q].y);
    };

    for (int j = 0; j < nblk; j++) {
        const int kb = 32 * j;
        const int nb = min(CH_NB, F - kb);
        if (TALL) {
            const int ntile = (nblk - j + 1) / 2;
            const int nround = (ntile + 3) / 4;
            const int brow = 8 * wave + (lane >> 3), bcol = 4 * (lane & 7);
            auto load_bq = [&](int col0, double2 (&v)[2]) {
                const double *src = Tl + (size_t)(kb + brow < F ? kb + brow : 0) * F + col0 + bcol;
                v[0] = *reinterpret_cast<const double2 *>(src);
                v[1] = *reinterpret_cast<const double2 *>(src + 2);
            };
            auto store_bq = [&](double *P, const double2 (&v)[2]) {
                const double sg = kb + brow < F ? 1.0 : 0.0;
                *reinterpret_cast<double2 *>(P + brow * CHM_S + bcol) = make_double2(sg * v[0].x, sg * v[0].y);
                *reinterpret_cast<double2 *>(P + brow * CHM_S + bcol + 2) = make_double2(sg * v[1].x, sg * v[1].y);
            };
            for (int u = 0; u < nround; u++) {
                const int t = wave + 4 * u;
                const bool has = t < ntile;
                const int i0 = 32 * (j + 2 * t);
                d4_t acc[4][2];
#pragma unroll
                for (int a = 0; a < 4; a++)
#pragma unroll
                    for (int b = 0; b < 2; b++)
#pragma unroll
                        for (int r = 0; r < 4; r++) {
                            const int row = i0 + 16 * a + kq + 4 * r, col = kb + 16 * b + ri;
                            double v = 0.0;
                            if (has && row < F && col <= row) v = A[(size_t)row * F + col] + (row == col ? jit : 0.0);
                            acc[a][b][r] = v;
                        }
                if (j > 0 && CHM_ABLATE != 3) {
                    double2 va0[8], va1[8], vb[2];
                    if (has) {
                        load_block(i0, 0, va0);
                        load_block(i0 + 32, 0, va1);
                    }
                    load_bq(0, vb);
                    for (int k = 0; k < j; k++) {
                        double *PBc = PBS + (k & 1) * 32 * CHM_S;
                        store_bq(PBc, vb);
                        __syncthreads();
                        if (k + 1 < j) load_bq(32 * (k + 1), vb);
                        if (has) {
                            store_block(PA, va0, -1.0, i0);
                            if (k + 1 < j) load_block(i0, 32 * (k + 1), va0);
#pragma unroll
                            for (int s = 0; s < 8; s++) {
                                double af[2], bf[2];
#pragma unroll
                                for (int a = 0; a < 2; a++) {
                                    af[a] = PA[(16 * a + ri) * CHM_S + 4 * s + kq];
                                    bf[a] = PBc[(16 * a + ri) * CHM_S + 4 * s + kq];
                                }
#pragma unroll
                                for (int a = 0; a < 2; a++)
#pragma unroll
                                    for (int b = 0; b < 2; b++)
                                        acc[a][b] = __builtin_amdgcn_mfma_f64_16x16x4f64(af[a], bf[b], acc[a][b], 0, 0, 0);
                            }
                            store_block(PA, va1, -1.0, i0 + 32);
                            if (k + 1 < j) load_block(i0 + 32, 32 * (k + 1), va1);
#pragma unroll
                            for (int s = 0; s < 8; s++) {
                                double af[2], bf[2];
#pragma unroll
                                for (int a = 0; a < 2; a++) {
                                    af[a] = PA[(16 * a + ri) * CHM_S + 4 * s + kq];
                                    bf[a] = PBc[(16 * a + ri) * CHM_S + 4 * s + kq];
                                }
#pragma unroll
                                for (int a = 0; a < 2; a++)
#pragma unroll
                                    for (int b = 0; b < 2; b++)
                                        acc[2 + a][b] = __builtin_amdgcn_mfma_f64_16x16x4f64(af[a], bf[b], acc[2 + a][b], 0, 0, 0);
                            }
                        }
                    }
                    __syncthreads();
                }
                if (has) {
#pragma unroll
                    for (int hb = 0; hb < 2; hb++) {
                        const int r0b = i0 + 32 * hb;
                        if (r0b >= F) continue;
                        if (t == 0 && hb == 0) {
#pragma unroll
                            for (int a = 0; a < 2; a++)
#pragma unroll
                                for (int b = 0; b < 2; b++)
#pragma unroll
                                    for (int r = 0; r < 4; r++)
                                        D[(16 * a + kq + 4 * r) * (CH_NB + 1) + 16 * b + ri] = acc[a][b][r];
                        } else {
#pragma unroll
                            for (int a = 0; a < 2; a++)
#pragma unroll
                                for (int b = 0; b < 2; b++)
#pragma unroll
                                    for (int r = 0; r < 4; r++) {
                                        const int row = r0b + 16 * a + kq + 4 * r, col = kb + 16 * b + ri;
                                        if (row < F && col < F) Tl[(size_t)row * F + col] = acc[2 * hb + a][b][r];
                                    }
                            if (kb + srow < F) {
                                double *z = Tl + (size_t)(kb + srow) * F + r0b + scol;
#pragma unroll
                                for (int q = 0; q < 8; q++)
                                    if (r0b + scol + 2 * q < F) *reinterpret_cast<double2 *>(z + 2 * q) = make_double2(0.0, 0.0);
                            }
                        }
                    }
                }
            }
        } else
        for (int i = j + wave; i < nblk; i += 4) {
            const int i0 = 32 * i;
            d4_t acc[2][2];
#pragma unroll
            for (int a = 0; a < 2; a++)
#pragma unroll
                for (int b = 0; b < 2; b++)
#pragma unroll
                    for (int r = 0; r < 4; r++) {
                        const int row = i0 + 16 * a + kq + 4 * r, col = kb + 16 * b + ri;
                        double v = 0.0;
                        if (row < F && col <= row) v = A[(size_t)row * F + col] + (row == col ? jit : 0.0);
                        acc[a][b][r] = v;
                    }
            if (j > 0 && CHM_ABLATE != 3) {
                double2 va[8], vb[8];
                load_block(i0, 0, va);
                load_block(kb, 0, vb);
                for (int k = 0; k < j; k++) {
                    store_block(PA, va, -1.0, i0);
                    store_block(PB, vb, 1.0, kb);
                    if (k + 1 < j) {
                        load_block(i0, 32 * (k + 1), va);
                        load_block(kb, 32 * (k + 1), vb);
                    }
#pragma unroll
                    for (int s = 0; s < 8; s++) {
                        double af[2], bf[2];
#pragma unroll
                        for (int a = 0; a < 2; a++) {
                            af[a] = PA[(16 * a + ri) * CHM_S + 4 * s + kq];
                            bf[a] = PB[(16 * a + ri) * CHM_S + 4 * s + kq];
                        }
#pragma unroll
                        for (int a = 0; a < 2; a++)
#pragma unroll
                            for (int b = 0; b < 2; b++)
                                acc[a][b] = __builtin_amdgcn_mfma_f64_16x16x4f64(af[a], bf[b], acc[a][b], 0, 0, 0);
                    }
                }
            }
            if (i == j) {
#pragma unroll
                for (int a = 0; a < 2; a++)
#pragma unroll
                    for (int b = 0; b < 2; b++)
#pragma unroll
                        for (int r = 0; r < 4; r++) D[(16 * a + kq + 4 * r) * (CH_NB + 1) + 16 * b + ri] = acc[a][b][r];
            } else {
#pragma unroll
                for (int a = 0; a < 2; a++)
#pragma unroll
                    for (int b = 0; b < 2; b++)
#pragma unroll
                        for (int r = 0; r < 4; r++) {
                            const int row = i0 + 16 * a + kq + 4 * r, col = kb + 16 * b + ri;
                            if (row < F && col < F) Tl[(size_t)row * F + col] = acc[a][b][r];
                        }
                if (kb + srow < F) {
                    double *z = Tl + (size_t)(kb + srow) * F + i0 + scol;
#pragma unroll
                    for (int q = 0; q < 8; q++)
                        if (i0 + scol + 2 * q < F) *reinterpret_cast<double2 *>(z + 2 * q) = make_double2(0.0, 0.0);
                }
            }
        }
        CSTAMP(0);
        __syncthreads();
        CSTAMP(1);
        if (tid < 64 && CHM_ABLATE != 1) {
            auto bcast = [](double v, int src) {
                const int lo = __builtin_amdgcn_readlane(__double2loint(v), src);
                const int hi = __builtin_amdgcn_readlane(__double2hiint(v), src);
                return __hiloint2double(hi, lo);
            };
            double row[CH_NB];
#pragma unroll
            for (int k = 0; k < CH_NB; k++) row[k] = (lane < nb && k <= lane) ? D[lane * (CH_NB + 1) + k] : 0.0;
            bool bad = false;
#pragma unroll
            for (int jj = 0; jj < CH_NB; jj++) {
                if (jj < nb && !bad) {
                    const double d = bcast(row[jj], jj);
                    if (!(d > 0.0)) {
                        bad = true;
                    } else {
                        double y = __builtin_amdgcn_rsq(d);
                        const double hd = 0.5 * d;
                        y = fma(y, fma(-hd * y, y, 0.5), y);
                        y = fma(y, fma(-hd * y, y, 0.5), y);
                        const double lij = row[jj] * y;
                        row[jj] = lij;
                        if (lane == jj) rdiag[jj] = y;
#pragma unroll
                        for (int k = jj + 1; k < CH_NB; k++) row[k] = fma(-lij, bcast(lij, k), row[k]);
                    }
                }
            }
#pragma unroll
            for (int k = 0; k < CH_NB; k++)
                if (lane < nb && k <= lane) D[lane * (CH_NB + 1) + k] = row[k];
            if (bad && lane == 0) *flag = 1;
        }
        CSTAMP(2);
        __syncthreads();
        CSTAMP(3);
        if (*flag) break;
        for (int q = tid; q < nb * nb; q += 256) {
            const int i = q / nb, jj = q % nb;
            Tl[(size_t)(kb + i) * F + kb + jj] = (jj <= i) ? D[i * (CH_NB + 1) + jj] : 0.0;
        }
        const int r0 = kb + nb;
        for (int r = r0 + tid; r < F && CHM_ABLATE != 2; r += 256) {
            double x[CH_NB];
            double *row = Tl + (size_t)r * F + kb;
#pragma unroll
            for (int jj = 0; jj < CH_NB; jj += 2) {
                const double2 v = *reinterpret_cast<const double2 *>(row + jj);
                x[jj] = v.x;
                x[jj + 1] = v.y;
            }
#pragma unroll
            for (int jj = 0; jj < CH_NB; jj++) {
                if (jj < nb) {
                    double s[4] = {x[jj], 0.0, 0.0, 0.0};
#pragma unroll
                    for (int p = 0; p < CH_NB; p++)
                        if (p < jj) s[p & 3] = fma(-x[p], D[jj * (CH_NB + 1) + p], s[p & 3]);
                    x[jj] = ((s[0] + s[1]) + (s[2] + s[3])) * rdiag[jj];
                }
            }
#pragma unroll
            for (int jj = 0; jj < CH_NB; jj += 2) *reinterpret_cast<double2 *>(row + jj) = make_double2(x[jj], x[jj + 1]);
        }
        CSTAMP(4);
        __syncthreads();
        CSTAMP(5);
    }
    if (tid == 0) info[blockIdx.x] = *flag;
#if CHM_STAMPS
    if (lane == 0) {
        for (int k = 0; k < 6; k++) atomicAdd(&g_chm_stamps[k], c_acc[k]);
        atomicAdd(&g_chm_stamps[7], 1ull);
    }
#endif
}

__global__ void __launch_bounds__(256)
chol_coop_kernel(const double *__restrict__ C, int F, double jitter_rel, double *T, int32_t *__restrict__ info, int mat0, int nrem,
                 int G, unsigned *bar, int *gflag, double *rd, int *xcc_min, int *xcc_max) {
    extern __shared__ __attribute__((aligned(16))) double lds[];
    double *D = lds;
    double *red = lds + CH_NB * (CH_NB + 1);
    double *rdiag = red + 256 + 2;
    double *stage = rdiag + CH_NB;

    const int tid = threadIdx.x, lane = tid & 63, wave = tid >> 6;
    const int ri = lane & 15, kq = lane >> 4;
    const int xslot = blockIdx.x >> 3;
    const int mi = (xslot / G) * 8 + (blockIdx.x & 7), wgl = xslot % G;
    if (mi >= nrem) return;
    const int gw = 4 * wgl + wave, NW = 4 * G;
    const size_t off = (size_t)(mat0 + mi) * F * F;
    const double *A = C + off;
    double *Tl = T + off;
    double *PA = stage + (size_t)wave * 2 * 32 * CHM_S, *PB = PA + 32 * CHM_S;

    double dmax = -INFINITY;
    for (int i = tid; i < F; i += 256) dmax = fmax(dmax, A[(size_t)i * F + i]);
    red[tid] = dmax;
    __syncthreads();
    for (int s = 128; s > 0; s >>= 1) {
        if (tid < s) red[tid] = fmax(red[tid], red[tid + s]);
        __syncthreads();
    }
    const double jit = red[0] * jitter_rel;
    __syncthreads();

    unsigned nsync = 0;
    bool same_xcc = false;
    auto group_sync = [&]() {
        if (same_xcc) asm volatile("s_waitcnt vmcnt(0) lgkmcnt(0)" ::: "memory");
        else __threadfence();
        __syncthreads();
        nsync++;
        if (tid == 0) {
            __hip_atomic_fetch_add(&bar[mi], 1u, __ATOMIC_RELAXED, __HIP_MEMORY_SCOPE_AGENT);
            unsigned polls = 0;
            while (__hip_atomic_load(&bar[mi], __ATOMIC_RELAXED, __HIP_MEMORY_SCOPE_AGENT) < nsync * (unsigned)G) {
                __builtin_amdgcn_s_sleep(2);
                if ((++polls & 1023u) == 0) {
                    if (__hip_atomic_load(&gflag[mi], __ATOMIC_RELAXED, __HIP_MEMORY_SCOPE_AGENT) == 3) break;
                    if (polls >= (1u << 21)) {
                        __hip_atomic_store(&gflag[mi], 3, __ATOMIC_RELAXED, __HIP_MEMORY_SCOPE_AGENT);
                        break;
                    }
                }
            }
        }
        __syncthreads();
        if (same_xcc) asm volatile("buffer_inv sc1" ::: "memory");
        else __threadfence();
    };
    {
        const int xcc = (int)__builtin_amdgcn_s_getreg((3 << 11) | 20) & 15;
        if (tid == 0) {
            __hip_atomic_fetch_min(&xcc_min[mi], xcc, __ATOMIC_RELAXED, __HIP_MEMORY_SCOPE_AGENT);
            __hip_atomic_fetch_max(&xcc_max[mi], xcc, __ATOMIC_RELAXED, __HIP_MEMORY_SCOPE_AGENT);
        }
        group_sync();
        same_xcc = __hip_atomic_load(&xcc_min[mi], __ATOMIC_RELAXED, __HIP_MEMORY_SCOPE_AGENT) ==
                   __hip_atomic_load(&xcc_max[mi], __ATOMIC_RELAXED, __HIP_MEMORY_SCOPE_AGENT);
        if (__hip_atomic_load(&gflag[mi], __ATOMIC_RELAXED, __HIP_MEMORY_SCOPE_AGENT)) {
            if (wgl == 0 && tid == 0) info[mat0 + mi] = 3;
            return;
        }
    }

    const int nblk = (F + 31) / 32;
    const int srow = lane >> 1, scol = 16 * (lane & 1);
    auto load_block = [&](int row0, int col0, double2 (&v)[8]) {
        const double *src = Tl + (size_t)(row0 + srow < F ? row0 + srow : 0) * F + col0 + scol;
#pragma unroll
        for (int q = 0; q < 8; q++) v[q] = *reinterpret_cast<const double2 *>(src + 2 * q);
    };
    auto store_block = [&](double *P, const double2 (&v)[8], double sign, int row0) {
        const double sg = row0 + srow < F ? sign : 0.0;
#pragma unroll
        for (int q = 0; q < 8; q++)
            *reinterpret_cast<double2 *>(P + srow * CHM_S + scol + 2 * q) = make_double2(sg * v[q].x, sg * v[q].y);
    };
    int failed = 0;
    for (int j = 0; j < nblk; j++) {
        const int kb = 32 * j;
        const int nb = min(CH_NB, F - kb);
        for (int i = j + gw; i < nblk; i += NW) {
            const int i0 = 32 * i;
            d4_t acc[2][2];
#pragma unroll
            for (int a = 0; a < 2; a++)
#pragma unroll
                for (int b = 0; b < 2; b++)
#pragma unroll
                    for (int r = 0; r < 4; r++) {
                        const int row = i0 + 16 * a + kq + 4 * r, col = kb + 16 * b + ri;
                        double v = 0.0;
                        if (row < F && col <= row) v = A[(size_t)row * F + col] + (row == col ? jit : 0.0);
                        acc[a][b][r] = v;
                    }
            if (j > 0) {
                double2 va[8], vb[8];
                load_block(i0, 0, va);
                load_block(kb, 0, vb);
                for (int k = 0; k < j; k++) {
                    store_block(PA, va, -1.0, i0);
                    store_block(PB, vb, 1.0, kb);
                    if (k + 1 < j) {
                        load_block(i0, 32 * (k + 1), va);
                        load_block(kb, 32 * (k + 1), vb);
                    }
#pragma unroll
                    for (int s = 0; s < 8; s++) {
                        double af[2], bf[2];
#pragma unroll
                        for (int a = 0; a < 2; a++) {
                            af[a] = PA[(16 * a + ri) * CHM_S + 4 * s + kq];
                            bf[a] = PB[(16 * a + ri) * CHM_S + 4 * s + kq];
                        }
#pragma unroll
                        for (int a = 0; a < 2; a++)
#pragma unroll
                            for (int b = 0; b < 2; b++)
                                acc[a][b] = __builtin_amdgcn_mfma_f64_16x16x4f64(af[a], bf[b], acc[a][b], 0, 0, 0);
                    }
                }
            }
            if (i == j) {
#pragma unroll
                for (int a = 0; a < 2; a++)
#pragma unroll
                    for (int b = 0; b < 2; b++)
#pragma unroll
                        for (int r = 0; r < 4; r++) D[(16 * a + kq + 4 * r) * (CH_NB + 1) + 16 * b + ri] = acc[a][b][r];
            } else {
#pragma unroll
                for (int a = 0; a < 2; a++)
#pragma unroll
                    for (int b = 0; b < 2; b++)
#pragma unroll
                        for (int r = 0; r < 4; r++) {
                            const int row = i0 + 16 * a + kq + 4 * r, col = kb + 16 * b + ri;
                            if (row < F && col < F) Tl[(size_t)row * F + col] = acc[a][b][r];
                        }
                if (kb + srow < F) {
                    double *z = Tl + (size_t)(kb + srow) * F + i0 + scol;
#pragma unroll
                    for (int q = 0; q < 8; q++)
                        if (i0 + scol + 2 * q < F) *reinterpret_cast<double2 *>(z + 2 * q) = make_double2(0.0, 0.0);
                }
            }
        }
        if (gw == 0) {
            auto bcast = [](double v, int src) {
                const int lo = __builtin_amdgcn_readlane(__double2loint(v), src);
                const int hi = __builtin_amdgcn_readlane(__double2hiint(v), src);
                return __hiloint2double(hi, lo);
            };
            double row[CH_NB];
#pragma unroll
            for (int k = 0; k < CH_NB; k++) row[k] = (lane < nb && k <= lane) ? D[lane * (CH_NB + 1) + k] : 0.0;
            bool bad = false;
#pragma unroll
            for (int jj = 0; jj < CH_NB; jj++) {
                if (jj < nb && !bad) {
                    const double d = bcast(row[jj], jj);
                    if (!(d > 0.0)) {
                        bad = true;
                    } else {
                        double y = __builtin_amdgcn_rsq(d);
                        const double hd = 0.5 * d;
                        y = fma(y, fma(-hd * y, y, 0.5), y);
                        y = fma(y, fma(-hd * y, y, 0.5), y);
                        const double lij = row[jj] * y;
                        row[jj] = lij;
                        if (lane == jj) __hip_atomic_store(&rd[mi * CH_NB + jj], y, __ATOMIC_RELAXED, __HIP_MEMORY_SCOPE_AGENT);
#pragma unroll
                        for (int k = jj + 1; k < CH_NB; k++) row[k] = fma(-lij, bcast(lij, k), row[k]);
                    }
                }
            }
            if (lane < nb) {
                double *o = Tl + (size_t)(kb + lane) * F + kb;
#pragma unroll
                for (int k = 0; k < CH_NB; k++)
                    if (k < nb) o[k] = k <= lane ? row[k] : 0.0;
            }
            if (bad && lane == 0) __hip_atomic_store(&gflag[mi], 1, __ATOMIC_RELAXED, __HIP_MEMORY_SCOPE_AGENT);
        }
        group_sync();
        failed = __hip_atomic_load(&gflag[mi], __ATOMIC_RELAXED, __HIP_MEMORY_SCOPE_AGENT);
        if (failed) break;
        for (int q = tid; q < CH_NB * CH_NB; q += 256) {
            const int i = q >> 5, jj = q & 31;
            D[i * (CH_NB + 1) + jj] = (i < nb && jj <= i) ? Tl[(size_t)(kb + i) * F + kb + jj] : 0.0;
        }
        if (tid < CH_NB) rdiag[tid] = tid < nb ? __hip_atomic_load(&rd[mi * CH_NB + tid], __ATOMIC_RELAXED, __HIP_MEMORY_SCOPE_AGENT) : 0.0;
        __syncthreads();
        for (int r = kb + nb + wgl * 256 + tid; r < F; r += 256 * G) {
            double x[CH_NB];
            double *row = Tl + (size_t)r * F + kb;
#pragma unroll
            for (int jj = 0; jj < CH_NB; jj += 2) {
                const double2 v = *reinterpret_cast<const double2 *>(row + jj);
                x[jj] = v.x;
                x[jj + 1] = v.y;
            }
#pragma unroll
            for (int jj = 0; jj < CH_NB; jj++) {
                if (jj < nb) {
                    double s[4] = {x[jj], 0.0, 0.0, 0.0};
#pragma unroll
                    for (int p = 0; p < CH_NB; p++)
                        if (p < jj) s[p & 3] = fma(-x[p], D[jj * (CH_NB + 1) + p], s[p & 3]);
                    x[jj] = ((s[0] + s[1]) + (s[2] + s[3])) * rdiag[jj];
                }
            }
#pragma unroll
            for (int jj = 0; jj < CH_NB; jj += 2) *reinterpret_cast<double2 *>(row + jj) = make_double2(x[jj], x[jj + 1]);
        }
        group_sync();
    }
    if (wgl == 0 && tid == 0) {
        info[mat0 + mi] = failed;
        xcc_max[mi] = same_xcc ? 0x100 : 0x200;
    }
}

__global__ void __launch_bounds__(256)
jacobi_root_kernel(const double *__restrict__ C, const int32_t *__restrict__ list, int F, double jitter_rel,
                   double eig_thresh, double *__restrict__ Wall, double *__restrict__ Vall,
                   double *__restrict__ T) {
    extern __shared__ __attribute__((aligned(16))) double lds[];
    double *cs = lds;
    double *red = lds + 2 * (F / 2 + 1);
    double *ev = red + 256;
    int *perm = reinterpret_cast<int *>(ev + F);
    int *order = perm + (F + 2);
    const int tid = threadIdx.x;
    const int l = list[blockIdx.x];
    const double *A = C + (size_t)l * F * F;
    double *W = Wall + (size_t)blockIdx.x * F * F;
    double *V = Vall + (size_t)blockIdx.x * F * F;
    double *Tl = T + (size_t)l * F * F;

    double dmax = -INFINITY;
    for (int i = tid; i < F; i += 256) dmax = fmax(dmax, A[(size_t)i * F + i]);
    red[tid] = dmax;
    __syncthreads();
    for (int s = 128; s > 0; s >>= 1) {
        if (tid < s) red[tid] = fmax(red[tid], red[tid + s]);
        __syncthreads();
    }
    const double jit = red[0] * jitter_rel;
    __syncthreads();
    for (long q = tid; q < (long)F * F; q += 256) {
        const int i = (int)(q / F), j = (int)(q % F);
        const double v = (j <= i) ? A[(size_t)i * F + j] : A[(size_t)j * F + i];
        W[q] = v + (i == j ? jit : 0.0);
        V[q] = (i == j) ? 1.0 : 0.0;
    }
    const int np = (F + 1) / 2;
    const int nplayers = 2 * np;
    for (int i = tid; i < nplayers; i += 256) perm[i] = i;
    __syncthreads();

    for (int sweep = 0; sweep < 60; sweep++) {
        double offs = 0.0, dia = 0.0;
        for (long q = tid; q < (long)F * F; q += 256) {
            const int i = (int)(q / F), j = (int)(q % F);
            const double v = W[q];
            if (i == j) dia += v * v;
            else offs += v * v;
        }
        red[tid] = offs;
        __syncthreads();
        for (int s = 128; s > 0; s >>= 1) {
            if (tid < s) red[tid] += red[tid + s];
            __syncthreads();
        }
        offs = red[0];
        __syncthreads();
        red[tid] = dia;
        __syncthreads();
        for (int s = 128; s > 0; s >>= 1) {
            if (tid < s) red[tid] += red[tid + s];
            __syncthreads();
        }
        dia = red[0];
        __syncthreads();
        if (offs <= 1e-30 * dia || offs == 0.0) break;

        for (int round = 0; round < nplayers - 1; round++) {
            for (int k = tid; k < np; k += 256) {
                int p = perm[k], q = perm[nplayers - 1 - k];
                if (p > q) { int t = p; p = q; q = t; }
                double c = 1.0, s = 0.0;
                if (q < F) {
                    const double apq = W[(size_t)p * F + q];
                    if (apq != 0.0) {
                        const double app = W[(size_t)p * F + p], aqq = W[(size_t)q * F + q];
                        const double tau = (aqq - app) / (2.0 * apq);
                        const double t = (tau >= 0.0 ? 1.0 : -1.0) / (fabs(tau) + sqrt(1.0 + tau * tau));
                        c = 1.0 / sqrt(1.0 + t * t);
                        s = t * c;
                    }
                }
                cs[2 * k] = c;
                cs[2 * k + 1] = s;
            }
            __syncthreads();
            for (int it = tid; it < np * F; it += 256) {
                const int k = it / F, j = it % F;
                int p = perm[k], q = perm[nplayers - 1 - k];
                if (p > q) { int t = p; p = q; q = t; }
                if (q >= F) continue;
                const double c = cs[2 * k], s = cs[2 * k + 1];
                const double wp = W[(size_t)p * F + j], wq = W[(size_t)q * F + j];
                W[(size_t)p * F + j] = c * wp - s * wq;
                W[(size_t)q * F + j] = s * wp + c * wq;
            }
            __syncthreads();
            for (int it = tid; it < np * F; it += 256) {
                const int k = it / F, i = it % F;
                int p = perm[k], q = perm[nplayers - 1 - k];
                if (p > q) { int t = p; p = q; q = t; }
                if (q >= F) continue;
                const double c = cs[2 * k], s = cs[2 * k + 1];
                const double wp = W[(size_t)i * F + p], wq = W[(size_t)i * F + q];
                W[(size_t)i * F + p] = c * wp - s * wq;
                W[(size_t)i * F + q] = s * wp + c * wq;
                const double vp = V[(size_t)i * F + p], vq = V[(size_t)i * F + q];
                V[(size_t)i * F + p] = c * vp - s * vq;
                V[(size_t)i * F + q] = s * vp + c * vq;
            }
            __syncthreads();
            if (tid == 0) {
                const int last = perm[nplayers - 1];
                for (int k = nplayers - 1; k > 1; k--) perm[k] = perm[k - 1];
                perm[1] = last;
            }
            __syncthreads();
        }
    }
    for (int i = tid; i < F; i += 256) ev[i] = W[(size_t)i * F + i];
    __syncthreads();
    double emax = -INFINITY;
    for (int i = tid; i < F; i += 256) emax = fmax(emax, ev[i]);
    red[tid] = emax;
    __syncthreads();
    for (int s = 128; s > 0; s >>= 1) {
        if (tid < s) red[tid] = fmax(red[tid], red[tid + s]);
        __syncthreads();
    }
    emax = red[0];
    __syncthreads();
    for (int i = tid; i < F; i += 256) {
        int rank = 0;
        const double e = ev[i];
        for (int j = 0; j < F; j++) {
            const double f = ev[j];
            if (f < e || (f == e && j < i)) rank++;
        }
        order[i] = rank;
    }
    __syncthreads();
    for (long q = tid; q < (long)F * F; q += 256) {
        const int i = (int)(q / F), j = (int)(q % F);
        double e = ev[j];
        if (e < emax * eig_thresh) e = 0.0;
        Tl[(size_t)i * F + order[j]] = V[q] * sqrt(e);
    }
}

extern "C" int corahip_factor_batched(corahip_ctx *ctx, const double *C, int nl, int F, double jitter_rel,
                                      double eig_thresh, double *T, int32_t *info) {
    ARG_CHECK(ctx != nullptr && C != nullptr && T != nullptr && info != nullptr);
    ARG_CHECK(nl >= 1 && F >= 1);
    StageTimer t(ctx, "factor");
    static const bool no_mfma = getenv("CORAHIP_K2_VALU") != nullptr;
    if (F >= 64 && (F % 2) == 0 && !no_mfma) {
        static const char *tall_env = getenv("CORAHIP_K2_TALL");
        const bool tall = tall_env ? atoi(tall_env) != 0 : F >= 384;
        const size_t shm = sizeof(double) * (CH_NB * (CH_NB + 1) + 256 + 2 + CH_NB + (tall ? 6 : 8) * 32 * CHM_S) + 16;
        const char *coop_env = getenv("CORAHIP_K2_COOP");
        const int nblk = (F + 31) / 32;
        const int G = (nblk + 3) / 4;
        int nrem = 0;
        if (tall && (F % 32) == 0 && !(coop_env && atoi(coop_env) == 0) && !CHM_STAMPS) {
            const int slots = 2 * ctx->num_cu;
            const int r = nl % slots;
            if (nl > slots && r > 0 && ((r + 7) / 8) * 8 * G <= ctx->num_cu && r <= 16) nrem = r;
            if (coop_env && atoi(coop_env) == 2 && ((nl + 7) / 8) * 8 * G <= ctx->num_cu) nrem = nl;
        }
        const size_t shm2 = sizeof(double) * (CH_NB * (CH_NB + 1) + 256 + 2 + CH_NB + 8 * 32 * CHM_S) + 16;
        if (nrem > 0) {
            HIP_TRY(hipFuncSetAttribute((const void *)chol_coop_kernel, hipFuncAttributeMaxDynamicSharedMemorySize, (int)shm2));
            int per_cu = 0;
            HIP_TRY(hipOccupancyMaxActiveBlocksPerMultiprocessor(&per_cu, (const void *)chol_coop_kernel, 256, shm2));
            if ((long)per_cu * ctx->num_cu < (long)((nrem + 7) / 8) * 8 * G) nrem = 0;
        }
        const int nmain = nl - nrem;
        if (tall) {
            HIP_TRY(hipFuncSetAttribute((const void *)chol_ll_kernel<true>, hipFuncAttributeMaxDynamicSharedMemorySize, (int)shm));
            if (nmain > 0) chol_ll_kernel<true><<<nmain, 256, shm, ctx->stream>>>(C, F, jitter_rel, T, info);
            if (nrem > 0) {
                void *ws = nullptr;
                const size_t wsb = (size_t)nrem * (sizeof(unsigned) + 3 * sizeof(int) + CH_NB * sizeof(double)) + 64;
                int rcs = corahip_ctx_scratch(ctx, 8, wsb, &ws);
                if (rcs) return rcs;
                HIP_TRY(hipMemsetAsync(ws, 0, wsb, ctx->stream));
                double *rd = reinterpret_cast<double *>(ws);
                unsigned *bar = reinterpret_cast<unsigned *>(rd + (size_t)nrem * CH_NB);
                int *gflag = reinterpret_cast<int *>(bar + nrem);
                int *xmin = gflag + nrem, *xmax = xmin + nrem;
                HIP_TRY(hipMemsetAsync(xmin, 0x7f, sizeof(int) * nrem, ctx->stream));
                chol_coop_kernel<<<((nrem + 7) / 8) * 8 * G, 256, shm2, ctx->stream>>>(C, F, jitter_rel, T, info, nmain, nrem, G, bar, gflag, rd,
                                                                                     xmin, xmax);
                if (getenv("CORAHIP_K2_COOP_DEBUG")) {
                    std::vector<int> hx(nrem);
                    HIP_TRY(hipMemcpyAsync(hx.data(), xmax, sizeof(int) * nrem, hipMemcpyDeviceToHost, ctx->stream));
                    HIP_TRY(hipStreamSynchronize(ctx->stream));
                    int same = 0;
                    for (int v : hx) same += v == 0x100;
                    fprintf(stderr, "K2 cooperative kernel: %d matrices, %d workgroups each, %d groups on one XCC\n", nrem, G, same);
                }
            }
        } else {
            HIP_TRY(hipFuncSetAttribute((const void *)chol_ll_kernel<false>, hipFuncAttributeMaxDynamicSharedMemorySize, (int)shm));
            chol_ll_kernel<false><<<nl, 256, shm, ctx->stream>>>(C, F, jitter_rel, T, info);
        }
        LAUNCH_CHECK();
#if CHM_STAMPS
        {
            unsigned long long hs[8], z[8] = {0};
            HIP_TRY(hipStreamSynchronize(ctx->stream));
            HIP_TRY(hipMemcpyFromSymbol(hs, HIP_SYMBOL(g_chm_stamps), sizeof(hs)));
            const double per = 1.0 / (double)std::max<unsigned long long>(hs[7], 1);
            fprintf(stderr, "K2 F=%d nl=%d tall=%d: cycles/wave  A %.0f  bar %.0f  B %.0f  bar %.0f  C %.0f  bar %.0f\n", F, nl, (int)tall,
                    hs[0] * per, hs[1] * per, hs[2] * per, hs[3] * per, hs[4] * per, hs[5] * per);
            HIP_TRY(hipMemcpyToSymbol(HIP_SYMBOL(g_chm_stamps), z, sizeof(z)));
        }
#endif
    } else {
        const size_t shm = sizeof(double) * (CH_NB * (CH_NB + 1) + 2 * 64 * (CH_NB + 1) + 256) + 16;
        chol_kernel<<<nl, 256, shm, ctx->stream>>>(C, F, jitter_rel, T, info);
        LAUNCH_CHECK();
    }
    std::vector<int32_t> hinfo(nl);
    HIP_TRY(hipMemcpyAsync(hinfo.data(), info, sizeof(int32_t) * nl, hipMemcpyDeviceToHost, ctx->stream));
    HIP_TRY(hipStreamSynchronize(ctx->stream));
    {
        bool redo = false;
        for (int l = 0; l < nl; l++)
            if (hinfo[l] == 3) {
                const size_t shm = sizeof(double) * (CH_NB * (CH_NB + 1) + 256 + 2 + CH_NB + 6 * 32 * CHM_S) + 16;
                chol_ll_kernel<true><<<1, 256, shm, ctx->stream>>>(C + (size_t)l * F * F, F, jitter_rel, T + (size_t)l * F * F, info + l);
                LAUNCH_CHECK();
                redo = true;
            }
        if (redo) {
            HIP_TRY(hipMemcpyAsync(hinfo.data(), info, sizeof(int32_t) * nl, hipMemcpyDeviceToHost, ctx->stream));
            HIP_TRY(hipStreamSynchronize(ctx->stream));
        }
    }
    std::vector<int32_t> list;
    for (int l = 0; l < nl; l++)
        if (hinfo[l] != 0) list.push_back(l);
    if (list.empty()) return 0;
    const size_t per = (size_t)2 * F * F * sizeof(double);
    const size_t batch = std::max<size_t>(1, std::min<size_t>(list.size(), ((size_t)1 << 31) / per));
    int32_t *dlist = nullptr;
    double *scratch = nullptr;
    HIP_TRY(hipMalloc((void **)&dlist, sizeof(int32_t) * list.size()));
    HIP_TRY(hipMalloc((void **)&scratch, per * batch));
    HIP_TRY(hipMemcpyAsync(dlist, list.data(), sizeof(int32_t) * list.size(), hipMemcpyHostToDevice, ctx->stream));
    const size_t shm = sizeof(double) * (2 * (F / 2 + 1) + 256 + F) + sizeof(int) * (2 * F + 4) + 16;
    for (size_t b0 = 0; b0 < list.size(); b0 += batch) {
        const int nb = (int)std::min(batch, list.size() - b0);
        jacobi_root_kernel<<<nb, 256, shm, ctx->stream>>>(C, dlist + b0, F, jitter_rel, eig_thresh, scratch,
                                                         scratch + (size_t)nb * F * F, T);
        LAUNCH_CHECK();
    }
    HIP_TRY(hipStreamSynchronize(ctx->stream));
    (void)hipFree(dlist);
    (void)hipFree(scratch);
    return 0;
}
```

### cora_amd/parallel.py

```python
from dataclasses import dataclass


@dataclass
class ShardPlan:
    rank: int
    world: int
    l_lo: int
    l_hi: int
    l_shard: int
    l_pad: int
    nu0: int
    nnu: int
    L: int = 0
    chunks: tuple = ()


def fold_chunks(F, rank, world):
    if F % (2 * world) or (F // (2 * world)) % 4:
        raise ValueError("fold=True needs F divisible by 8 * world (F = %d, world = %d)" % (F, world))
    c = F // (2 * world)
    return ((rank * c, c), ((2 * world - 1 - rank) * c, c))


def fold_permutation(F, world):
    import numpy as np

    return np.concatenate([np.arange(a, a + n) for q in range(world) for a, n in fold_chunks(F, q, world)])


def shard_plan(L, F, rank, world, fold=False):
    l_shard = (L + world - 1) // world
    l_lo = min(rank * l_shard, L)
    l_hi = min(l_lo + l_shard, L)
    if fold and world > 1:
        ch = fold_chunks(F, rank, world)
        return ShardPlan(rank, world, l_lo, l_hi, l_shard, l_shard * world, ch[0][0], 2 * ch[0][1], L, ch)
    base, extra = divmod(F, world)
    nnu = base + (1 if rank < extra else 0)
    nu0 = rank * base + min(rank, extra)
    return ShardPlan(rank, world, l_lo, l_hi, l_shard, l_shard * world, nu0, nnu, L, ((nu0, nnu),))


import contextlib as _contextlib
import threading as _threading

_STAGE = {"name": None, "since": None, "last": None, "beat": None, "thread": None}


def dist_timeout():
    import datetime
    import os

    return datetime.timedelta(seconds=float(os.environ.get("CORA_DIST_TIMEOUT_S", "300")))


def start_watchdog(rank=0, world=1, exit_fn=None):
    import os
    import sys
    import time

    if _STAGE["thread"] is not None:
        return _STAGE["thread"]
    limit = dist_timeout().total_seconds()
    leave = exit_fn or (lambda code: os._exit(code))

    def run():
        while True:
            time.sleep(min(1.0, limit / 4.0))
            name, since = _STAGE["name"], _STAGE["since"]
            if name is not None and since is not None and time.time() - since > limit:
                sys.stderr.write("cora_amd.parallel: stage '%s' has not completed after %.0f s on rank %d of %d (last completed "
                                 "stage: %s): a peer is missing or a collective hangs - aborting\n"
                                 % (name, limit, rank, world, _STAGE["last"]))
                sys.stderr.flush()
                leave(3)
                return

    t = _threading.Thread(target=run, name="cora-dist-watchdog", daemon=True)
    _STAGE["thread"] = t
    t.start()
    return t


@_contextlib.contextmanager
def exchange_stage(name, sync=None):
    import os
    import time

    prev = (_STAGE["name"], _STAGE["since"])
    _STAGE["name"], _STAGE["since"] = name, time.time()
    try:
        yield
        if os.environ.get("CORA_DIST_SYNC_EXCHANGES") if sync is None else sync:
            import torch

            if torch.cuda.is_available():
                torch.cuda.synchronize()
        _STAGE["last"] = name
    finally:
        _STAGE["name"], _STAGE["since"] = prev


def allgather_factors(T_local, info_local, plan):
    import torch
    import torch.distributed as dist

    F = T_local.shape[1]
    pad_T = torch.zeros((plan.l_shard, F, F), dtype=T_local.dtype, device=T_local.device)
    pad_i = torch.zeros((plan.l_shard,), dtype=info_local.dtype, device=info_local.device)
    n = plan.l_hi - plan.l_lo
    pad_T[:n].copy_(T_local)
    pad_i[:n].copy_(info_local)
    T_all = torch.empty((plan.l_pad, F, F), dtype=T_local.dtype, device=T_local.device)
    i_all = torch.empty((plan.l_pad,), dtype=info_local.dtype, device=info_local.device)
    with exchange_stage("all-gather of the factor shards"):
        dist.all_gather_into_tensor(T_all, pad_T)
        dist.all_gather_into_tensor(i_all, pad_i)
    return T_all[: plan.L], i_all[: plan.L]


def allgather_channels(shard, F):
    import torch
    import torch.distributed as dist

    if shard.is_complex():
        return torch.view_as_complex(allgather_channels(torch.view_as_real(shard).contiguous(), F))
    world = dist.get_world_size()
    nmax = (F + world - 1) // world
    pad = torch.zeros((nmax,) + tuple(shard.shape[1:]), dtype=shard.dtype, device=shard.device)
    pad[: shard.shape[0]].copy_(shard)
    full = torch.empty((world * nmax,) + tuple(shard.shape[1:]), dtype=shard.dtype, device=shard.device)
    with exchange_stage("all-gather of the channel shards"):
        dist.all_gather_into_tensor(full, pad)
    parts = []
    for r in range(world):
        sp = shard_plan(1, F, r, world)
        parts.append(full[r * nmax : r * nmax + sp.nnu])
    return torch.cat(parts, dim=0)


def _all_to_all(send, world):
    import torch
    import torch.distributed as dist

    send = send.contiguous()
    recv = torch.empty_like(send)
    if dist.get_backend() == "nccl":
        dist.all_to_all_single(recv, send)
        return recv
    rank = dist.get_rank()
    parts = [torch.empty_like(send) for _ in range(world)]
    dist.all_gather(parts, send)
    for q in range(world):
        recv[q].copy_(parts[q][rank])
    return recv


def exchange_pair_slabs(slabs, plan):
    assert slabs.shape[0] == plan.world and slabs.shape[2] == plan.l_shard
    with exchange_stage("all-to-all #1 (C_l pair slabs -> multipole shards)"):
        return _all_to_all(slabs, plan.world)


def _rows_pack(T_local, l_stride, world):
    import torch

    if T_local.is_cuda:
        from . import _lib

        return _lib.get_context(T_local.device.index).factor_rows_pack(T_local.contiguous(), l_stride, world)
    n, F, _ = T_local.shape
    pad = torch.zeros((l_stride, F, F), dtype=T_local.dtype)
    pad[:n].copy_(T_local)
    return pad.view(l_stride, world, F // world, F).permute(1, 0, 2, 3).contiguous()


def _rows_unpack(recv, counts):
    import torch

    if recv.is_cuda and recv.shape[0] <= 64:
        from . import _lib

        return _lib.get_context(recv.device.index).factor_rows_unpack(recv, counts)
    return torch.cat([recv[r, : counts[r]] for r in range(recv.shape[0])], dim=0).contiguous()


def exchange_factor_rows(T_local, info_local, plan):
    import torch
    import torch.distributed as dist

    F = T_local.shape[1]
    W = plan.world
    assert F % W == 0 and plan.nnu == F // W
    if len(plan.chunks) > 1:
        perm = torch.as_tensor(fold_permutation(F, W), device=T_local.device)
        T_local = T_local.index_select(1, perm)
    n = plan.l_hi - plan.l_lo
    pad_i = torch.zeros((plan.l_shard,), dtype=info_local.dtype, device=info_local.device)
    pad_i[:n].copy_(info_local)
    send = _rows_pack(T_local, plan.l_shard, W)
    with exchange_stage("all-to-all #2 (factor row blocks -> channel shards)"):
        recv = _all_to_all(send, W)
        i_all = torch.empty((plan.l_pad,), dtype=info_local.dtype, device=info_local.device)
        dist.all_gather_into_tensor(i_all, pad_i)
    counts = [max(0, min(plan.L, (r + 1) * plan.l_shard) - min(plan.L, r * plan.l_shard)) for r in range(W)]
    return _rows_unpack(recv, counts), i_all[: plan.L]


def device_memory_bytes(default=288e9):
    try:
        import torch

        if torch.cuda.is_available():
            return float(torch.cuda.get_device_properties(torch.cuda.current_device()).total_memory)
    except Exception:
        pass
    return float(default)


def numpy_ring_bytes(F, lmax, device_bytes=None):
    import os

    if device_bytes is None:
        device_bytes = device_memory_bytes()
    L = lmax + 1
    if os.environ.get("CORAHIP_RING_MB"):
        ring = float(max(1, int(os.environ["CORAHIP_RING_MB"])) << 20)
        return int(min(8 * F * L * (L + 1), 2 * max(ring / 2, 16.0 * F * L)))
    stream = 8 * F * L * (L + 1)
    ring = 2.0**31 if stream <= device_bytes / 8 else max(device_bytes / 16, 2.0**31)
    slot = max(ring / 2, 16.0 * F * L)
    return int(min(stream, 2 * slot))


def rank_memory_bytes(kinds, F, nside, lmax, world, sum_mode="joint", rng="philox", fold=False, device_bytes=288e9):
    L = lmax + 1
    nalm = L * (L + 1) // 2
    npix = 12 * nside * nside
    npair, nring = 2 * nside, 4 * nside - 1
    nnu = -(-F // world)
    lsh = -(-L // world)
    ntab = sum(1 for k in kinds if k == "table21cm")
    joint = len(kinds) > 1 and sum_mode == "joint"
    out = {}
    out["maps"] = 8 * npix * nnu
    out["a_lm"] = 16 * nalm * (-(-nnu // 4) * 4) * (1 if (joint or len(kinds) == 1) else 2)
    out["synthesis workspace (F_m cells)"] = nring * (-(-nnu // 8) * 2) * L * 64
    out["plan (recurrence coefficients, polar seeds, first-l tables, ring FFT tables)"] = (
        2 * 16 * nalm + (2 * 16 + 64) * L * npair + 4 * L * npair + int(1.0e8 * (nside / 1024.0) ** 2))
    if ntab:
        out["21cm tables + their transposed copy"] = 2 * 3 * 500 * 32768 * 8
        pairs = F * (F + 1) // 2
        out["C_l: pair slabs (sent + received), block of this rank's multipoles, its factors"] = (
            (2 * 8 * (-(-pairs // world)) * (lsh * world) if world > 1 else 8 * pairs * L) + 2 * 8 * lsh * F * F)
    if joint:
        out["summed covariance block"] = 8 * lsh * F * F
    ndraw = 1 if joint else len(kinds)
    if world > 1:
        out["factor rows [L, nnu, F] (+ exchange slabs)"] = (ndraw * 8 * L * nnu * F + 2 * 8 * world * lsh * nnu * F
                                                             + (8 * lsh * F * F if fold else 0))
    elif not ntab:
        out["factor rows [L, nnu, F] (+ exchange slabs)"] = ndraw * 8 * L * nnu * F
    if rng == "numpy":
        nn = 2 * F * nalm
        out["numpy normal stream: ring of l ranges + generator tables"] = numpy_ring_bytes(F, lmax, device_bytes) + int(0.38 * nn)
    out["total"] = sum(out.values())
    return out


class SkyShard:

    def __init__(self, model, freq, nside, lmax, zromb=3, rank=0, world=1, ctx=None, distributed=None, emulate_world=0,
                 alm_buf=None, maps_buf=None, fold=False, emulate_rank=None):
        import numpy as np

        from . import _lib
        from .core import skysim

        self.ctx = ctx if ctx is not None else _lib.get_context()
        ctx = self.ctx
        self.freq = np.asarray(freq, dtype=np.float64)
        self.F = F = self.freq.size
        self.nside, self.lmax, self.L = int(nside), int(lmax), int(lmax) + 1
        self.rank, self.world = rank, world
        self.distributed = (world > 1) if distributed is None else bool(distributed)
        self.emulate_world = int(emulate_world)
        L = self.L
        self.fold = bool(fold)
        self.plan = shard_plan(L, F, rank, world, fold=self.fold)
        if self.emulate_world > 1:
            N = self.emulate_world
            er = N - 1 if emulate_rank is None else int(emulate_rank)
            self.plan = shard_plan(L, F, er, N, fold=self.fold)
            p0 = shard_plan(L, F, 0, N)
            self.plan.l_lo, self.plan.l_hi = p0.l_lo, p0.l_hi
        sp = self.plan
        self.nu0, self.nnu = sp.nu0, sp.nnu
        self.chunks = tuple(sp.chunks)
        self.folded = len(self.chunks) > 1
        self.channels = np.concatenate([np.arange(a, a + n) for a, n in self.chunks])
        self.zint = zint = 2**zromb + 1 if zromb else 1
        fsort = np.sort(self.freq)
        zhalf = abs(fsort[1] - fsort[0]) / 2.0 if F > 1 else 0.0
        za = (self.freq[:, None] + np.linspace(-zhalf, zhalf, zint)[None, :]).ravel() if zromb else self.freq.copy()
        self.w = ctx.to_device(skysim.romberg_weights(zromb))
        cplan = model._clarray_plan(model.angular_powerspectrum)
        if cplan is None:
            raise NotImplementedError(
                "SkyShard needs a model whose angular_powerspectrum is the library's table (21cm) or separable "
                "(ForegroundSCK) form; %s overrides it - integrate C_l with skysim.clarray_device and use "
                "skysim.mkfullsky_device(nu_range=...) instead" % type(model).__name__)
        nshard = max(world, self.emulate_world, 1)
        self.pair_sharded = (cplan["kind"] == "table21cm" and (self.distributed or self.emulate_world > 1)
                             and F % nshard == 0)
        if self.folded and not (self.pair_sharded or cplan["kind"] != "table21cm"):
            raise ValueError("fold=True needs the row-block exchange (F divisible by the number of ranks)")
        larr = np.arange(L, dtype=np.float64)
        if cplan["kind"] == "table21cm":
            p = cplan["prepare"](ctx, za)
            lx_full = np.log10(np.where(larr == 0.0, 1e-10, larr))
            self._lx = ctx.to_device(lx_full if self.pair_sharded else lx_full[sp.l_lo:sp.l_hi])
            self._k1 = [ctx.to_device(p[k]) for k in ("chi", "pfd", "f", "b")]
            self._tabs = (p["dd"], p["dv"], p["vv"], p["kperpmin"], p["kperpmax"], p["kparmax"])
            self._sep = None
        else:
            al, bcov = cplan["prepare"](larr.copy(), za)
            self._sep = (ctx.to_device(al[sp.l_lo:sp.l_hi]), ctx.to_device(bcov), ctx.to_device(al))
        nalm = L * (L + 1) // 2
        self.npix = 12 * self.nside * self.nside
        ctx.sht_plan(self.nside, self.lmax)
        self.alm_buf = alm_buf if alm_buf is not None else ctx.empty((nalm, (self.nnu + 3) // 4, 2, 4))
        self.maps_buf = maps_buf if maps_buf is not None else ctx.empty((self.nnu, self.npix))
        ctx.workspace(ctx.alm2map_workspace_bytes(ctx.sht_plan(self.nside, self.lmax), self.nnu))
        self._emulated = None
        if self.emulate_world > 1:
            import torch

            rows = self.pair_sharded
            Tf = ctx.empty((L, self.nnu, F) if rows else (L, F, F))
            inf = torch.empty((L,), dtype=torch.int32, device=ctx.device)
            eye = 0.1 * torch.eye(F, device=ctx.device, dtype=torch.float64)
            lc = max(1, min(L, (1 << 28) // (F * F)))
            for l0 in range(0, L, lc):
                Cc = ctx.empty((min(lc, L - l0), F, F)).normal_()
                Tc, ic = ctx.factor_batched(Cc @ Cc.transpose(1, 2) + eye)
                Tf[l0:l0 + Tc.shape[0]].copy_(Tc[:, self._chan_index(), :] if rows else Tc)
                inf[l0:l0 + Tc.shape[0]].copy_(ic)
                del Cc, Tc, ic
            self._emulated = (Tf, inf, rows)
            nl0 = sp.l_hi - sp.l_lo
            self._emu_C = ctx.empty((nl0, F, F))
            for l0 in range(0, nl0, lc):
                Cc = ctx.empty((min(lc, nl0 - l0), F, F)).normal_()
                self._emu_C[l0:l0 + Cc.shape[0]].copy_(Cc @ Cc.transpose(1, 2) + eye)
                del Cc

    def _chan_index(self):
        import torch

        if getattr(self, "_chan_idx", None) is None:
            self._chan_idx = torch.as_tensor(self.channels, device=self.ctx.device)
        return self._chan_idx

    def _clarray_local(self):
        ctx = self.ctx
        if self._sep is not None:
            return ctx.clarray_separable(self._sep[0], self._sep[1], self.F, self.zint, self.w)
        return ctx.clarray_table21cm(*self._tabs, *self._k1, self.F, self.zint, self.w, self._lx)

    def _separable_factors(self):
        import torch

        ctx = self.ctx
        one = torch.ones((1,), dtype=torch.float64, device=ctx.device)
        bbar = ctx.clarray_separable(one, self._sep[1], self.F, self.zint, self.w)
        tb, ib = ctx.factor_batched(bbar)
        rows = tb[0].index_select(0, self._chan_index())
        T = torch.sqrt(self._sep[2])[:, None, None] * rows[None, :, :]
        info = ib.expand(self.L).contiguous()
        return T.contiguous(), info, True

    def _clarray_pairs(self, first, step):
        return self.ctx.clarray_table21cm_pairs(*self._tabs, *self._k1, self.F, self.zint, self.w, self._lx, first, step,
                                                self.plan.l_shard, nblocks=step)

    def covariance_shard(self):
        ctx, sp = self.ctx, self.plan
        if self.emulate_world > 1:
            N = self.emulate_world
            if self._sep is None and self.pair_sharded:
                slab = self._clarray_pairs(N - 1, N)
                ctx.clarray_pairs_finish(slab.new_zeros((N,) + tuple(slab.shape[1:])), self.F, sp.l_hi - sp.l_lo)
            else:
                self._clarray_local()
            return self._emu_C
        if self.distributed and self._sep is None and self.pair_sharded:
            mine = exchange_pair_slabs(self._clarray_pairs(self.rank, self.world), sp)
            return ctx.clarray_pairs_finish(mine, self.F, sp.l_hi - sp.l_lo)
        return self._clarray_local()

    def share_factors(self, T, info):
        sp = self.plan
        if not self.distributed:
            return T, info, False
        if self.F % max(self.world, 1) == 0:
            Tr, ia = exchange_factor_rows(T, info, sp)
            return Tr, ia, True
        Ta, ia = allgather_factors(T, info, sp)
        return Ta, ia, False

    def factors(self):
        ctx, sp = self.ctx, self.plan
        if self._sep is not None:
            return self._separable_factors()
        if self.emulate_world > 1:
            N = self.emulate_world
            if self.pair_sharded:
                slab = self._clarray_pairs(N - 1, N)
                C = ctx.clarray_pairs_finish(slab.new_zeros((N,) + tuple(slab.shape[1:])), self.F, sp.l_hi - sp.l_lo)
                del C
            else:
                self._clarray_local()
            ctx.factor_batched(self._emu_C)
            return self._emulated
        if not self.distributed:
            T, info = ctx.factor_batched(self._clarray_local())
            return T, info, False
        if self.pair_sharded:
            mine = exchange_pair_slabs(self._clarray_pairs(self.rank, self.world), sp)
            T, info = ctx.factor_batched(ctx.clarray_pairs_finish(mine, self.F, sp.l_hi - sp.l_lo))
            Tr, ia = exchange_factor_rows(T, info, sp)
            return Tr, ia, True
        T, info = ctx.factor_batched(self._clarray_local())
        Ta, ia = allgather_factors(T, info, sp)
        return Ta, ia, False

    def draw(self, seed, factors=None, out=None):
        ctx = self.ctx
        out = self.alm_buf if out is None else out
        T, info, rows = factors if factors is not None else self.factors()
        if rows and self.folded:
            return ctx.draw_alm_philox_chunks(T, info, seed, self.lmax, self.F, self.chunks, out=out)
        if rows:
            return ctx.draw_alm_philox_rows(T, info, seed, self.lmax, self.F, self.nu0, self.nnu, out=out)
        return ctx.draw_alm_philox(T, info, seed, self.lmax, self.F, nu0=self.nu0, nnu=self.nnu, out=out)

    def realise(self, seed, factors=None):
        self.draw(seed, factors)
        return self.ctx.alm2map(self.alm_buf, self.nside, self.lmax, self.nnu, out=self.maps_buf)

    def realise_numpy(self, rng, factors=None, prepared=None):
        _, finish = self.draw_numpy(rng, factors, defer=True, prepared=prepared)
        try:
            return self.ctx.alm2map(self.alm_buf, self.nside, self.lmax, self.nnu, out=self.maps_buf)
        finally:
            finish()

    def prepare_numpy(self, rng):
        from .core import skysim

        return skysim.prepare_numpy_stream(self.ctx, rng, self.lmax, self.F)

    def draw_numpy(self, rng, factors=None, out=None, defer=False, prepared=None):
        from .core import skysim

        if factors is None:
            if prepared is None:
                prepared = self.prepare_numpy(rng)
            try:
                factors = self.factors()
            except BaseException:
                if prepared is not None:
                    prepared.abort()
                raise
        T, info, rows = factors
        return skysim.draw_numpy_stream(self.ctx, T, info, rng, self.lmax, self.F, nu0=self.nu0, nnu=self.nnu,
                                        out=self.alm_buf if out is None else out, rows=rows, defer=defer,
                                        chunks=self.chunks if (rows and self.folded) else None, prepared=prepared)


class SkySum:

    _SEED_STRIDE = 0x9E3779B97F4A7C15

    def __init__(self, components, freq, nside, lmax, rank=0, world=1, ctx=None, distributed=None, emulate_world=0,
                 mode="joint", fold=False, emulate_rank=None):
        from . import _lib

        if mode not in ("joint", "separate"):
            raise ValueError("mode must be 'joint' or 'separate'")
        self.mode = mode
        self.ctx = ctx if ctx is not None else _lib.get_context()
        self.shards = []
        alm_buf = maps_buf = None
        for model, zromb in components:
            sh = SkyShard(model, freq, nside, lmax, zromb=zromb, rank=rank, world=world, ctx=self.ctx,
                          distributed=distributed, emulate_world=emulate_world, alm_buf=alm_buf, maps_buf=maps_buf,
                          fold=fold, emulate_rank=emulate_rank)
            alm_buf, maps_buf = sh.alm_buf, sh.maps_buf
            self.shards.append(sh)
        s0 = self.shards[0]
        self.alm_buf, self.maps_buf = alm_buf, maps_buf
        self.nu0, self.nnu, self.F, self.nside, self.lmax, self.npix = s0.nu0, s0.nnu, s0.F, s0.nside, s0.lmax, s0.npix
        self.channels, self.chunks, self.folded = s0.channels, s0.chunks, s0.folded
        self._tmp = self.ctx.empty(tuple(alm_buf.shape)) if (len(self.shards) > 1 and mode == "separate") else None

    def covariance_shard(self):
        total = None
        for sh in self.shards:
            C = sh.covariance_shard()
            if sh.emulate_world > 1:
                total = C
                continue
            jit = C.diagonal(dim1=1, dim2=2).amax(dim=1) * 1e-14
            if total is None:
                total = C
            else:
                total.add_(C)
                del C
            total.diagonal(dim1=1, dim2=2).add_(jit[:, None])
        return total

    def factors(self):
        if self.mode == "separate":
            return [sh.factors() for sh in self.shards]
        s0 = self.shards[0]
        C = self.covariance_shard()
        T, info = self.ctx.factor_batched(C, jitter_rel=0.0)
        del C
        if s0.emulate_world > 1:
            return [s0._emulated]
        return [s0.share_factors(T, info)]

    def draw(self, seed, factors=None):
        factors = factors if factors is not None else self.factors()
        if self.mode == "joint":
            return self.shards[0].draw(int(seed), factors[0], out=self.alm_buf)
        for k, (sh, fac) in enumerate(zip(self.shards, factors)):
            sk = (int(seed) + k * self._SEED_STRIDE) & (2**64 - 1)
            if k == 0:
                sh.draw(sk, fac, out=self.alm_buf)
            else:
                sh.draw(sk, fac, out=self._tmp)
                self.alm_buf.add_(self._tmp)
        return self.alm_buf

    def realise(self, seed, factors=None):
        self.draw(seed, factors)
        return self.ctx.alm2map(self.alm_buf, self.nside, self.lmax, self.nnu, out=self.maps_buf)

    def realise_numpy(self, rng, factors=None):
        factors = factors if factors is not None else self.factors()
        finish = lambda: None
        if self.mode == "joint":
            _, finish = self.shards[0].draw_numpy(rng, factors[0], out=self.alm_buf, defer=True)
        else:
            for k, (sh, fac) in enumerate(zip(self.shards, factors)):
                last = k == len(self.shards) - 1
                if k == 0:
                    r = sh.draw_numpy(rng, fac, out=self.alm_buf, defer=last)
                else:
                    r = sh.draw_numpy(rng, fac, out=self._tmp, defer=last)
                    self.alm_buf.add_(self._tmp)
                if last:
                    finish = r[1]
        try:
            return self.ctx.alm2map(self.alm_buf, self.nside, self.lmax, self.nnu, out=self.maps_buf)
        finally:
            finish()


def getsky_shard(sky, seed, rank=0, world=1, lmax=None, fold=False):
    lmax = 3 * sky.nside - 1 if lmax is None else lmax
    zromb = getattr(sky, "oversample", 3)
    import numpy as np

    shard = SkyShard(sky, sky.nu_pixels, sky.nside, lmax, zromb=zromb if zromb is not None else 3, rank=rank, world=world,
                     fold=fold)
    maps = shard.realise(int(seed))
    freq = np.asarray(sky.nu_pixels, dtype=np.float64)[shard.channels]
    mean = shard.ctx.to_device(np.asarray(sky.mean_nu(freq), dtype=np.float64) * np.ones(shard.nnu))
    return maps + mean[:, None], (shard.channels if shard.folded else shard.nu0)


def mkfullsky_sharded(corr_local, global_shape, nside, rng=None, alms=False, ctx=None):
    import numpy as np
    import torch
    import torch.distributed as dist

    from . import _lib
    from .core import skysim
    from .util.nputil import DeviceRNG

    ctx = ctx if ctx is not None else _lib.get_context()
    world, rank = dist.get_world_size(), dist.get_rank()
    L, F, F2 = (int(v) for v in global_shape)
    if F2 != F:
        raise Exception("Correlation matrix is incorrect shape.")
    if not isinstance(corr_local, torch.Tensor):
        corr_local = ctx.to_device(np.asarray(corr_local, dtype=np.float64))
    n_local = int(corr_local.shape[0])
    counts = [None] * world
    dist.all_gather_object(counts, n_local)
    if sum(counts) != L:
        raise Exception("l blocks of the ranks do not add up to global_shape[0]")
    lc = max(max(counts), 1)
    sp = shard_plan(L, F, rank, world)
    nu0, nnu = sp.nu0, sp.nnu
    T_loc, i_loc = skysim.factor_device(corr_local) if n_local else (ctx.empty((0, F, F)), torch.empty(
        (0,), dtype=torch.int32, device=ctx.device))
    pad_i = torch.zeros((lc,), dtype=torch.int32, device=ctx.device)
    pad_i[:n_local].copy_(i_loc)
    i_all = torch.empty((world * lc,), dtype=torch.int32, device=ctx.device)
    rows = F % world == 0
    with exchange_stage("mkfullsky_sharded: factor exchange (l-distributed input -> channel shards)"):
        dist.all_gather_into_tensor(i_all, pad_i)
        if rows:
            recv = _all_to_all(_rows_pack(T_loc, lc, world), world)
        else:
            pad_T = torch.zeros((lc, F, F), dtype=torch.float64, device=ctx.device)
            pad_T[:n_local].copy_(T_loc)
            recv = torch.empty((world * lc, F, F), dtype=torch.float64, device=ctx.device)
            dist.all_gather_into_tensor(recv, pad_T)
    if rows:
        T = _rows_unpack(recv, counts)
    else:
        recv = recv.view(world, lc, F, F)
        T = torch.cat([recv[r, : counts[r]] for r in range(world)], dim=0).contiguous()
    info = torch.cat([i_all[r * lc : r * lc + counts[r]] for r in range(world)]).contiguous()
    lmax = L - 1
    if rng is None:
        box = [int(np.random.randint(0, 2**62)) if rank == 0 else 0]
        dist.broadcast_object_list(box, src=0)
        rng = DeviceRNG(box[0])
    if isinstance(rng, DeviceRNG):
        seed = rng.next_seed()
        alm = (ctx.draw_alm_philox_rows(T, info, seed, lmax, F, nu0, nnu) if rows
               else ctx.draw_alm_philox(T, info, seed, lmax, F, nu0=nu0, nnu=nnu))
    else:
        alm = skysim.draw_numpy_stream(ctx, T, info, rng, lmax, F, nu0=nu0, nnu=nnu, rows=rows)
    if alms:
        return ctx.alm_dev_to_square(alm, lmax, nnu), nu0
    return ctx.alm2map(alm, int(nside), lmax, nnu), nu0
```

### include/corahip.h

```cpp
#ifndef CORAHIP_H
#define CORAHIP_H

#include <stddef.h>
#include <stdint.h>

#ifdef __cplusplus
extern "C" {
#endif

#define CORAHIP_ABI_VERSION 1
#define CORAHIP_ABI_MINOR 6

#define CORAHIP_EINVAL (-1)
#define CORAHIP_ENOMEM (-2)
#define CORAHIP_ESTATE (-3)

typedef struct corahip_ctx corahip_ctx;
typedef struct corahip_sht_plan corahip_sht_plan;

int corahip_abi_version(void);
int corahip_abi_minor(void);
const char *corahip_last_error(void);
int corahip_device_count(int *count);
int corahip_ctx_create(int device_id, corahip_ctx **ctx);
int corahip_ctx_destroy(corahip_ctx *ctx);
int corahip_ctx_set_stream(corahip_ctx *ctx, void *hip_stream);
int corahip_ctx_sync(corahip_ctx *ctx);
int corahip_timer_begin(corahip_ctx *ctx);
int corahip_timer_end(corahip_ctx *ctx, float *elapsed_ms);
int corahip_profile_enable(corahip_ctx *ctx, int enable);
int corahip_profile_get(corahip_ctx *ctx, const char *name, double *total_ms, int *launches);
int corahip_profile_reset(corahip_ctx *ctx);

int corahip_malloc(corahip_ctx *ctx, size_t bytes, void **dptr);
int corahip_free(corahip_ctx *ctx, void *dptr);
int corahip_memcpy_h2d(corahip_ctx *ctx, void *dst, const void *host_src, size_t bytes);
int corahip_memcpy_d2h(corahip_ctx *ctx, void *host_dst, const void *src, size_t bytes);


int corahip_clarray_table21cm(corahip_ctx *ctx, const double *dd, const double *dv, const double *vv,
                              int nkperp, int nkpar, double kperpmin, double kperpmax, double kparmax,
                              const double *chi, const double *pfd, const double *f, const double *b,
                              int F, int zint, const double *w, const double *log10l, int nl,
                              double *out);

int corahip_clarray_table21cm_pairs(corahip_ctx *ctx, const double *dd, const double *dv, const double *vv,
                                    int nkperp, int nkpar, double kperpmin, double kperpmax, double kparmax,
                                    const double *chi, const double *pfd, const double *f, const double *b,
                                    int F, int zint, const double *w, const double *log10l, int nl,
                                    int pair_first, int pair_step, int l_block, double *out_pairs);
int corahip_clarray_pairs_finish(corahip_ctx *ctx, const double *pairs_in, int F, int nranks, int l_stride,
                                 int nl, double *out);

int corahip_clarray_tables_pin(corahip_ctx *ctx, const double *dd, const double *dv, const double *vv,
                               uint64_t generation);

int corahip_aps_table21cm_points(corahip_ctx *ctx, const double *dd, const double *dv, const double *vv,
                                 int nkperp, int nkpar, double kperpmin, double kperpmax, double kparmax,
                                 long n, const double *lx, const double *chi1, const double *chi2,
                                 const double *cdd, const double *cdv, const double *cvv, double *out);

int corahip_clarray_separable(corahip_ctx *ctx, const double *al, int nl, const double *bcov, int F,
                              int zint, const double *w, double *out);

int corahip_romb_reduce(corahip_ctx *ctx, const double *clt, int nl, int F, int zint, const double *w,
                        double *out);

int corahip_factor_batched(corahip_ctx *ctx, const double *C, int nl, int F, double jitter_rel,
                           double eig_thresh, double *T, int32_t *info);

int corahip_normals_philox(corahip_ctx *ctx, uint64_t seed, int lmax, int F, double *g);

int corahip_normals_pcg64(corahip_ctx *ctx, const uint64_t host_state[2], const uint64_t host_inc[2], int64_t n,
                          double *g, uint64_t *host_n_raw);
int corahip_glibc_exp(corahip_ctx *ctx, const double *x, int64_t n, double *y);
int corahip_pcg64_advance(const uint64_t host_state[2], const uint64_t host_inc[2], uint64_t delta,
                          uint64_t host_out_state[2]);

typedef struct corahip_mt_state {
    uint32_t key[624];
    int32_t pos, has_gauss;
    double gauss;
} corahip_mt_state;
int corahip_normals_mt19937_legacy(corahip_ctx *ctx, corahip_mt_state *host_state, int64_t n, double *g);

int corahip_draw_alm(corahip_ctx *ctx, const double *T, const int32_t *info, const double *g, int lmax,
                     int F, int nu0, int nnu, double *alm_dev);

int corahip_draw_alm_rows(corahip_ctx *ctx, const double *T_rows, const int32_t *info, const double *g, int lmax,
                          int F, int nu0, int nnu, double *alm_dev);

int corahip_draw_alm_philox(corahip_ctx *ctx, const double *T, const int32_t *info, uint64_t seed, int lmax,
                            int F, int nu0, int nnu, double *alm_dev);

int corahip_draw_alm_philox_rows(corahip_ctx *ctx, const double *T_rows, const int32_t *info, uint64_t seed,
                                 int lmax, int F, int nu0, int nnu, double *alm_dev);

typedef struct corahip_chanset {
    int32_t nchunks, chunk_nnu;
    int32_t nu0[2];
} corahip_chanset;
int corahip_draw_alm_philox_rows_set(corahip_ctx *ctx, const double *T_rows, const int32_t *info, uint64_t seed,
                                     int lmax, int F, const corahip_chanset *set, double *alm_dev);

#define CORAHIP_RNG_STREAM 0
#define CORAHIP_RNG_PHILOX 1
#define CORAHIP_RNG_PCG64 2
#define CORAHIP_RNG_MT19937 3
typedef struct corahip_rng {
    int32_t kind, reserved;
    const double *stream;
    uint64_t seed;
    uint64_t state[2], inc[2];
    corahip_mt_state *legacy;
} corahip_rng;
int corahip_mkfullsky_workspace_bytes(const corahip_sht_plan *plan, int F, int nu0, int nnu, int rng_kind, int alms,
                                      size_t *bytes);
int corahip_mkfullsky(corahip_ctx *ctx, const corahip_sht_plan *plan, const double *C, int F, corahip_rng *host_rng,
                      int nu0, int nnu, int alms, double *out, void *workspace, size_t workspace_bytes);

typedef struct corahip_draw_pending corahip_draw_pending;
int corahip_draw_alm_numpy(corahip_ctx *ctx, const double *T, int rows, const int32_t *info, corahip_rng *host_rng,
                           int lmax, int F, int nu0, int nnu, double *alm_dev, size_t ring_bytes);
int corahip_draw_alm_numpy_begin(corahip_ctx *ctx, const double *T, int rows, const int32_t *info, const corahip_rng *host_rng,
                                 int lmax, int F, int nu0, int nnu, double *alm_dev, size_t ring_bytes,
                                 corahip_draw_pending **pending);
int corahip_draw_alm_numpy_end(corahip_ctx *ctx, corahip_draw_pending *pending, corahip_rng *host_rng);
int corahip_draw_alm_numpy_prepare(corahip_ctx *ctx, const corahip_rng *host_rng, int lmax, int F, size_t ring_bytes,
                                   corahip_draw_pending **pending);
int corahip_draw_alm_numpy_run(corahip_ctx *ctx, corahip_draw_pending *pending, const double *T, int rows, const int32_t *info,
                               const corahip_chanset *set, double *alm_dev);
int corahip_draw_alm_numpy_begin_set(corahip_ctx *ctx, const double *T_rows, const int32_t *info, const corahip_rng *host_rng,
                                     int lmax, int F, const corahip_chanset *set, double *alm_dev, size_t ring_bytes,
                                     corahip_draw_pending **pending);

typedef struct corahip_shard {
    int32_t l_lo, l_hi;
    int32_t l_shard, l_pad;
    int32_t nu0, nnu;
    int32_t rows_exchange;
    int32_t L;
} corahip_shard;
int corahip_shard_plan(int L, int F, int rank, int world, corahip_shard *out);
int corahip_factor_rows_pack(corahip_ctx *ctx, const double *T_local, int n_local, int l_stride, int F, int world,
                             double *send);
int corahip_factor_rows_unpack(corahip_ctx *ctx, const double *recv, const int32_t *host_counts, int world,
                               int l_stride, int nnu, int F, double *T_rows);

int corahip_alm_dev_to_square(corahip_ctx *ctx, const double *alm_dev, int lmax, int nnu, double *square);
int corahip_alm_packed_to_dev(corahip_ctx *ctx, const double *packed, int lmax, int nnu, double *alm_dev);

int corahip_sht_plan_create(corahip_ctx *ctx, int nside, int lmax, corahip_sht_plan **plan);
int corahip_sht_plan_create_ex(corahip_ctx *ctx, int nside, int lmax, int cut_exp, corahip_sht_plan **plan);
int corahip_sht_plan_cut_exp(const corahip_sht_plan *plan, int *cut_exp);
int corahip_sht_plan_destroy(corahip_ctx *ctx, corahip_sht_plan *plan);
int corahip_sht_plan_k4_mfma_count(corahip_ctx *ctx, const corahip_sht_plan *plan, int nnu,
                                   uint64_t *mfma_instructions);
int corahip_alm2map_workspace_bytes(const corahip_sht_plan *plan, int nnu, size_t *bytes);
int corahip_alm2map(corahip_ctx *ctx, const corahip_sht_plan *plan, const double *alm_dev, int nnu,
                    double *maps, void *workspace, size_t workspace_bytes);

int corahip_map2alm_workspace_bytes(const corahip_sht_plan *plan, int nnu, size_t *bytes);
int corahip_map2alm(corahip_ctx *ctx, const corahip_sht_plan *plan, const double *maps, int nnu,
                    const double *ring_w, double *alm_dev, void *workspace, size_t workspace_bytes);

int corahip_alm2map_spin2(corahip_ctx *ctx, corahip_sht_plan *plan, const double *alm_dev, int nnu,
                          double *maps, void *workspace, size_t workspace_bytes);

int corahip_spin2_ring_scale(corahip_ctx *ctx, corahip_sht_plan *plan, const double *maps_qu, int nfields,
                             double *maps6);
int corahip_spin2_combine(corahip_ctx *ctx, corahip_sht_plan *plan, const double *alm6_dev, int g6, int nfields,
                          double *alm_eb_dev, int gout);

int corahip_ps_table21cm(corahip_ctx *ctx, const double *knots_x, const double *knots_y, const double *knots_y2,
                         int nknot, int loglog, double kstar, const double *kperp, int nkperp, const double *kpar,
                         int nkpar, double freq_window, const double *dd_in, double *dd, double *dv, double *vv);
int corahip_dct1_workspace_bytes(long nrows, int n, size_t *bytes);
int corahip_dct1_rows(corahip_ctx *ctx, double *data, long nrows, int n, double scale, void *workspace,
                      size_t workspace_bytes);

int corahip_xi_table_average(corahip_ctx *ctx, const double *knots_x, const double *knots_y,
                             const double *knots_y2, int nk, int kind, double x_t, double f_t,
                             const double *mu, int nm, const double *xa, const double *xw, int F, int xint,
                             double *out);
int corahip_legendre_project(corahip_ctx *ctx, const double *mu, const double *wt, int nm, int lmax,
                             const double *xi, long ncol, double *out);

int corahip_fft_c2c(corahip_ctx *ctx, double *data, int ndim, const int64_t *dims, int axis, int inverse);
int corahip_irfftn(corahip_ctx *ctx, double *spec, int ndim, const int64_t *rdims, int naxes, double *out);
int corahip_rfftn(corahip_ctx *ctx, const double *in, int ndim, const int64_t *rdims, int naxes, double *spec);
int corahip_randomfield_draw(corahip_ctx *ctx, const double *kweight, int64_t count, uint64_t seed,
                             double *spec);
int corahip_fg_mix(corahip_ctx *ctx, const double *freq_weight, const double *normals, const double *aff,
                   int F, int ncorr, int64_t M, double *out);
int corahip_randomfield_irfftn(corahip_ctx *ctx, const double *kweight, int ndim, const int64_t *rdims, uint64_t seed,
                               double *spec, double *out);
int corahip_spec_mul_real(corahip_ctx *ctx, double *spec, const double *weight, int64_t count);
int corahip_cube_affine(corahip_ctx *ctx, const double *df, const double *vf, const double *a, const double *b,
                        const double *c, int n0, int64_t plane, double *out);
int corahip_raytrace_slices(corahip_ctx *ctx, const double *cube, int n0, int n1, int n2, const double *zc,
                            const double *scale, const double *tx, const double *ty, double wx, double wy,
                            int numz, int numx, int numy, double *out);

int corahip_healpix_neighbours(corahip_ctx *ctx, int nside, int32_t *out);
int corahip_za_density_sph(corahip_ctx *ctx, const double *psi, const double *delta_bias, const double *delta_m,
                           const double *chi, int nchi, int nside, double sigma_ang, double sigma_chi, double *out);

int corahip_der1_alm_prep(corahip_ctx *ctx, corahip_sht_plan *plan, const double *alm_dev, int g_src, int g0, int g_in,
                          double *alm3_dev);
int corahip_der1_combine(corahip_ctx *ctx, corahip_sht_plan *plan, const double *maps3, int g_in, int nfields,
                         const double *s_theta, const double *s_phi, int phi_extra, double *out_theta, double *out_phi);
int corahip_radial_gradient(corahip_ctx *ctx, const double *f, const double *x_coef, const double *s_r, int n, long npix,
                            double *out);

int corahip_sht_plan_rings(const corahip_sht_plan *plan, int64_t *host_start, int32_t *host_nphi,
                           double *host_z, double *host_phi0);
int corahip_sht_plan_ring_classes(const corahip_sht_plan *plan, int32_t *host_len);
int corahip_sht_lambda(corahip_ctx *ctx, const corahip_sht_plan *plan, int m, int ring_pair, double *out);
int corahip_sht_lambda_entry(corahip_ctx *ctx, const corahip_sht_plan *plan, int m, int ring_pair, int kq, double *out);

#ifdef __cplusplus
}
#endif
#endif
```

Before: 3179.

## Skip covariance mirror pass and read upper triangle directly in Cholesky kernels

The clarray stage now has variants that leave only the upper triangle filled and skip the mirror kernel. The Cholesky kernels take an `up` flag and read the transposed (upper) element instead of the lower one, which removes one full read-write pass over the nl×F×F covariance. A new single-stage Cholesky kernel (chol_ls_kernel) is also added for the non-tall case with F≤256, using a different LDS staging layout and two workgroups per CU. The transposed reads are strided in memory, which may hurt coalescing during the initial loads.

```diff
diff --git a/cora_amd/_lib.py b/cora_amd/_lib.py
--- a/cora_amd/_lib.py
+++ b/cora_amd/_lib.py
@@ -30,16 +30,20 @@
     "corahip_memcpy_d2h": (c_int, [c_void_p, c_void_p, c_void_p, c_size_t]),
     "corahip_clarray_table21cm": (c_int, [c_void_p, PTR, PTR, PTR, c_int, c_int, c_double, c_double, c_double,
                                           PTR, PTR, PTR, PTR, c_int, c_int, PTR, PTR, c_int, PTR]),
+    "corahip_clarray_table21cm_upper": (c_int, [c_void_p, PTR, PTR, PTR, c_int, c_int, c_double, c_double, c_double,
+                                          PTR, PTR, PTR, PTR, c_int, c_int, PTR, PTR, c_int, PTR]),
     "corahip_clarray_table21cm_pairs": (c_int, [c_void_p, PTR, PTR, PTR, c_int, c_int, c_double, c_double, c_double,
                                                 PTR, PTR, PTR, PTR, c_int, c_int, PTR, PTR, c_int, c_int, c_int, c_int,
                                                 PTR]),
     "corahip_clarray_pairs_finish": (c_int, [c_void_p, PTR, c_int, c_int, c_int, c_int, PTR]),
+    "corahip_clarray_pairs_finish_upper": (c_int, [c_void_p, PTR, c_int, c_int, c_int, c_int, PTR]),
     "corahip_clarray_tables_pin": (c_int, [c_void_p, PTR, PTR, PTR, c_u64]),
     "corahip_aps_table21cm_points": (c_int, [c_void_p, PTR, PTR, PTR, c_int, c_int, c_double, c_double, c_double,
                                              ctypes.c_long, PTR, PTR, PTR, PTR, PTR, PTR, PTR]),
     "corahip_clarray_separable": (c_int, [c_void_p, PTR, c_int, PTR, c_int, c_int, PTR, PTR]),
     "corahip_romb_reduce": (c_int, [c_void_p, PTR, c_int, c_int, c_int, PTR, PTR]),
     "corahip_factor_batched": (c_int, [c_void_p, PTR, c_int, c_int, c_double, c_double, PTR, PTR]),
+    "corahip_factor_batched_upper": (c_int, [c_void_p, PTR, c_int, c_int, c_double, c_double, PTR, PTR]),
     "corahip_normals_philox": (c_int, [c_void_p, c_u64, c_int, c_int, PTR]),
     "corahip_normals_pcg64": (c_int, [c_void_p, ctypes.POINTER(c_u64), ctypes.POINTER(c_u64), ctypes.c_int64, PTR,
                                       ctypes.POINTER(c_u64)]),
@@ -306,11 +310,11 @@
         if self.h:
             _check(self.lib.corahip_clarray_tables_pin(self.h, None, None, None, c_u64(int(generation))))
 
-    def clarray_table21cm(self, dd, dv, vv, kperpmin, kperpmax, kparmax, chi, pfd, f, b, F, zint, w, log10l):
+    def clarray_table21cm(self, dd, dv, vv, kperpmin, kperpmax, kparmax, chi, pfd, f, b, F, zint, w, log10l, upper=False):
         nl = log10l.numel()
         out = self.empty((nl, F, F))
         nkperp, nkpar = dd.shape
-        _check(self.lib.corahip_clarray_table21cm(
+        _check((self.lib.corahip_clarray_table21cm_upper if upper else self.lib.corahip_clarray_table21cm)(
             self.h, self._f64(dd), self._f64(dv), self._f64(vv), nkperp, nkpar, kperpmin, kperpmax, kparmax,
             self._f64(chi), self._f64(pfd), self._f64(f), self._f64(b), F, zint, self._f64(w), self._f64(log10l),
             nl, self._f64(out)))
@@ -333,11 +337,11 @@
             nl, pair_first, pair_step, l_block, self._f64(out)))
         return out
 
-    def clarray_pairs_finish(self, slabs, F, nl):
+    def clarray_pairs_finish(self, slabs, F, nl, upper=False):
         nranks, npl, l_stride = slabs.shape
         assert npl == (F * (F + 1) // 2 + nranks - 1) // nranks and nl <= l_stride
         out = self.empty((nl, F, F))
-        _check(self.lib.corahip_clarray_pairs_finish(self.h, self._f64(slabs), F, nranks, l_stride, nl, self._f64(out)))
+        _check((self.lib.corahip_clarray_pairs_finish_upper if upper else self.lib.corahip_clarray_pairs_finish)(self.h, self._f64(slabs), F, nranks, l_stride, nl, self._f64(out)))
         return out
 
     def aps_table21cm_points(self, dd, dv, vv, kperpmin, kperpmax, kparmax, lx, chi1, chi2, cdd, cdv, cvv):
@@ -386,14 +390,14 @@
         _check(self.lib.corahip_dct1_rows(self.h, self._f64(data), nrows, n, float(scale), self._p(ws), int(b.value)))
         return data
 
-    def factor_batched(self, C, jitter_rel=1e-14, eig_thresh=1e-16):
+    def factor_batched(self, C, jitter_rel=1e-14, eig_thresh=1e-16, upper=False):
         torch = _torch()
         nl, F, F2 = C.shape
         assert F == F2
         T = self.empty((nl, F, F))
         info = torch.empty((nl,), dtype=torch.int32, device=self.device)
-        _check(self.lib.corahip_factor_batched(self.h, self._f64(C), nl, F, jitter_rel, eig_thresh, self._f64(T),
-                                               self._p(info)))
+        fn = self.lib.corahip_factor_batched_upper if upper else self.lib.corahip_factor_batched
+        _check(fn(self.h, self._f64(C), nl, F, jitter_rel, eig_thresh, self._f64(T), self._p(info)))
         return T, info
 
     def normals_philox(self, seed, lmax, F, out=None):
diff --git a/cora_amd/csrc/clarray.hip b/cora_amd/csrc/clarray.hip
--- a/cora_amd/csrc/clarray.hip
+++ b/cora_amd/csrc/clarray.hip
@@ -492,10 +492,10 @@
     return 0;
 }
 
-int corahip_clarray_table21cm(corahip_ctx *ctx, const double *dd, const double *dv, const double *vv, int nkperp,
+static int clarray_table21cm_impl(corahip_ctx *ctx, const double *dd, const double *dv, const double *vv, int nkperp,
                               int nkpar, double kperpmin, double kperpmax, double kparmax, const double *chi,
                               const double *pfd, const double *f, const double *b, int F, int zint, const double *w,
-                              const double *log10l, int nl, double *out) {
+                              const double *log10l, int nl, double *out, bool mirror) {
     ARG_CHECK(ctx != nullptr && dd && dv && vv && chi && pfd && f && b && w && log10l && out);
     ARG_CHECK(nkperp >= 2 && nkperp < CL_XS && nkpar >= 2 && F >= 1 && zint >= 1 && zint <= CL_MAXZ && nl >= 1);
     ARG_CHECK(kperpmin > 0 && kperpmax > kperpmin && kparmax > 0);
@@ -510,7 +510,23 @@
     dim3 grid((unsigned)((npairs + 31) / 32), (nl + 31) / 32);
     cl_finish_kernel<<<grid, 256, 0, ctx->stream>>>(scratch, npairs, 1, npairs, nl, nl, F, out);
     LAUNCH_CHECK();
-    return launch_mirror(ctx, out, nl, F);
+    return mirror ? launch_mirror(ctx, out, nl, F) : 0;
+}
+
+int corahip_clarray_table21cm(corahip_ctx *ctx, const double *dd, const double *dv, const double *vv, int nkperp,
+                              int nkpar, double kperpmin, double kperpmax, double kparmax, const double *chi,
+                              const double *pfd, const double *f, const double *b, int F, int zint, const double *w,
+                              const double *log10l, int nl, double *out) {
+    return clarray_table21cm_impl(ctx, dd, dv, vv, nkperp, nkpar, kperpmin, kperpmax, kparmax, chi, pfd, f, b, F, zint, w, log10l,
+                                  nl, out, true);
+}
+
+int corahip_clarray_table21cm_upper(corahip_ctx *ctx, const double *dd, const double *dv, const double *vv, int nkperp,
+                                    int nkpar, double kperpmin, double kperpmax, double kparmax, const double *chi,
+                                    const double *pfd, const double *f, const double *b, int F, int zint, const double *w,
+                                    const double *log10l, int nl, double *out) {
+    return clarray_table21cm_impl(ctx, dd, dv, vv, nkperp, nkpar, kperpmin, kperpmax, kparmax, chi, pfd, f, b, F, zint, w, log10l,
+                                  nl, out, false);
 }
 
 int corahip_clarray_table21cm_pairs(corahip_ctx *ctx, const double *dd, const double *dv, const double *vv, int nkperp,
@@ -529,8 +545,8 @@
                            log10l, nl, pair_first, pair_step, npl, l_block, out_pairs);
 }
 
-int corahip_clarray_pairs_finish(corahip_ctx *ctx, const double *pairs_in, int F, int nranks, int l_stride, int nl,
-                                 double *out) {
+static int clarray_pairs_finish_impl(corahip_ctx *ctx, const double *pairs_in, int F, int nranks, int l_stride, int nl,
+                                     double *out, bool mirror) {
     ARG_CHECK(ctx != nullptr && pairs_in && out && F >= 1 && nranks >= 1 && nl >= 1 && l_stride >= nl);
     StageTimer t(ctx, "clarray");
     const long npairs = (long)F * (F + 1) / 2;
@@ -538,7 +554,17 @@
     dim3 grid((unsigned)((npl * nranks + 31) / 32), (nl + 31) / 32);
     cl_finish_kernel<<<grid, 256, 0, ctx->stream>>>(pairs_in, npairs, nranks, npl, l_stride, nl, F, out);
     LAUNCH_CHECK();
-    return launch_mirror(ctx, out, nl, F);
+    return mirror ? launch_mirror(ctx, out, nl, F) : 0;
+}
+
+int corahip_clarray_pairs_finish(corahip_ctx *ctx, const double *pairs_in, int F, int nranks, int l_stride, int nl,
+                                 double *out) {
+    return clarray_pairs_finish_impl(ctx, pairs_in, F, nranks, l_stride, nl, out, true);
+}
+
+int corahip_clarray_pairs_finish_upper(corahip_ctx *ctx, const double *pairs_in, int F, int nranks, int l_stride, int nl,
+                                       double *out) {
+    return clarray_pairs_finish_impl(ctx, pairs_in, F, nranks, l_stride, nl, out, false);
 }
 
 int corahip_clarray_separable(corahip_ctx *ctx, const double *al, int nl, const double *bcov, int F, int zint,
diff --git a/cora_amd/csrc/factor.hip b/cora_amd/csrc/factor.hip
--- a/cora_amd/csrc/factor.hip
+++ b/cora_amd/csrc/factor.hip
@@ -7,7 +7,7 @@
 
 __global__ void __launch_bounds__(256)
 chol_kernel(const double *__restrict__ C, int F, double jitter_rel, double *__restrict__ T,
-            int32_t *__restrict__ info) {
+            int32_t *__restrict__ info, int up) {
     extern __shared__ __attribute__((aligned(16))) double lds[];
     double *D = lds;
     double *PA = lds + CH_NB * (CH_NB + 1);
@@ -34,7 +34,7 @@
     for (long q = tid; q < (long)F * F; q += 256) {
         const int i = (int)(q / F), j = (int)(q % F);
         double v = 0.0;
-        if (j <= i) v = A[q] + (i == j ? jit : 0.0);
+        if (j <= i) v = A[up ? (size_t)j * F + i : (size_t)q] + (i == j ? jit : 0.0);
         Tl[q] = v;
     }
     __syncthreads();
@@ -166,7 +166,7 @@
 template <bool TALL>
 __global__ void __launch_bounds__(256)
 chol_ll_kernel(const double *__restrict__ C, int F, double jitter_rel, double *__restrict__ T,
-               int32_t *__restrict__ info) {
+               int32_t *__restrict__ info, int up) {
     extern __shared__ __attribute__((aligned(16))) double lds[];
     double *D = lds;
     double *red = lds + CH_NB * (CH_NB + 1);
@@ -179,6 +179,7 @@
     const size_t off = (size_t)blockIdx.x * F * F;
     const double *A = C + off;
     double *Tl = T + off;
+    const int a_sr = up ? 1 : F, a_sc = up ? F : 1;
     double *PA = stage + (size_t)wave * (TALL ? 1 : 2) * 32 * CHM_S, *PB = PA + 32 * CHM_S;
     double *PBS = stage + 4 * 32 * CHM_S;
 
@@ -242,7 +243,7 @@
                         for (int r = 0; r < 4; r++) {
                             const int row = i0 + 16 * a + kq + 4 * r, col = kb + 16 * b + ri;
                             double v = 0.0;
-                            if (has && row < F && col <= row) v = A[(size_t)row * F + col] + (row == col ? jit : 0.0);
+                            if (has && row < F && col <= row) v = A[(unsigned)(row * a_sr + col * a_sc)] + (row == col ? jit : 0.0);
                             acc[a][b][r] = v;
                         }
                 if (j > 0 && CHM_ABLATE != 3) {
@@ -339,7 +340,7 @@
                     for (int r = 0; r < 4; r++) {
                         const int row = i0 + 16 * a + kq + 4 * r, col = kb + 16 * b + ri;
                         double v = 0.0;
-                        if (row < F && col <= row) v = A[(size_t)row * F + col] + (row == col ? jit : 0.0);
+                        if (row < F && col <= row) v = A[(unsigned)(row * a_sr + col * a_sc)] + (row == col ? jit : 0.0);
                         acc[a][b][r] = v;
                     }
             if (j > 0 && CHM_ABLATE != 3) {
@@ -475,8 +476,249 @@
 #endif
 }
 
+#define CHS_P 33
+__global__ void __launch_bounds__(256, 2)
+chol_ls_kernel(const double *__restrict__ C, int F, double jitter_rel, double *__restrict__ T,
+               int32_t *__restrict__ info, int up) {
+    extern __shared__ __attribute__((aligned(16))) double lds[];
+    double *D = lds;
+    double *red = lds + CH_NB * (CH_NB + 1);
+    int *flag = reinterpret_cast<int *>(red + 256);
+    double *rdiag = red + 256 + 2;
+    double *stage = rdiag + CH_NB;
+
+    const int tid = threadIdx.x, lane = tid & 63;
+    const int wave = __builtin_amdgcn_readfirstlane(tid >> 6);
+    const int ri = lane & 15, kq = lane >> 4;
+    const size_t off = (size_t)blockIdx.x * F * F;
+    const double *A = C + off;
+    double *Tl = T + off;
+    const int a_sr = up ? 1 : F, a_sc = up ? F : 1;
+    double *PBS = stage;
+    double *PA = stage + 2 * 32 * CHM_S + (size_t)wave * 2 * 16 * CHM_S;
+    double *PN = stage + (size_t)wave * 64 * CHS_P;
+
+    double dmax = -INFINITY;
+    for (int i = tid; i < F; i += 256) dmax = fmax(dmax, A[(size_t)i * F + i]);
+    red[tid] = dmax;
+    if (tid == 0) *flag = 0;
+    __syncthreads();
+    for (int s = 128; s > 0; s >>= 1) {
+        if (tid < s) red[tid] = fmax(red[tid], red[tid + s]);
+        __syncthreads();
+    }
+    const double jit = red[0] * jitter_rel;
+    __syncthreads();
+
+#if CHM_STAMPS
+    unsigned long long c_acc[8] = {0, 0, 0, 0, 0, 0, 0, 0}, c_last;
+    { unsigned long long _t; asm volatile("s_memtime %0\n\ts_waitcnt lgkmcnt(0)" : "=s"(_t)::"memory"); c_last = _t; }
+#endif
+    const int nblk = (F + 31) / 32;
+    const int lrow = lane >> 4, lcol = 2 * (lane & 15);
+    auto fresh_lane = [&]() {
+        int l;
+        asm volatile("v_mov_b32 %0, %1" : "=v"(l) : "v"(lane));
+        return l;
+    };
+    auto init_acc = [&](int jn, d4_t (&acc)[4][2]) {
+        const int kbn = 32 * jn;
+        const int fl = fresh_lane(), ri = fl & 15, kq = fl >> 4;
+#pragma unroll
+        for (int t = 0; t < 4; t++)
+#pragma unroll
+            for (int b = 0; b < 2; b++)
+#pragma unroll
+                for (int r = 0; r < 4; r++) {
+                    const int row = kbn + 16 * (wave + 4 * t) + kq + 4 * r, col = kbn + 16 * b + ri;
+                    double v = 0.0;
+                    if (row < F && col <= row) v = A[(unsigned)(row * a_sr + col * a_sc)] + (row == col ? jit : 0.0);
+                    acc[t][b][r] = v;
+                }
+    };
+    d4_t acc[4][2];
+    init_acc(0, acc);
+
+    for (int j = 0; j < nblk; j++) {
+        const int kb = 32 * j;
+        const int nb = min(CH_NB, F - kb);
+        const int ns = (F - kb + 15) / 16;
+        const int nt = ns > wave ? (ns - wave + 3) / 4 : 0;
+        if (j > 0 && CHM_ABLATE != 3) {
+            int lrow = lane >> 4, lcol = 2 * (lane & 15), ri = lane & 15, kq = lane >> 4;
+            auto load_strip = [&](int t, int k, double2 (&v)[4]) {
+#pragma unroll
+                for (int q = 0; q < 4; q++) {
+                    const int rr = min(kb + 16 * (wave + 4 * t) + 4 * q + lrow, F - 1);
+                    v[q] = *reinterpret_cast<const double2 *>(Tl + (unsigned)(rr * F + 32 * k + lcol));
+                }
+            };
+            auto store_strip = [&](double *P, const double2 (&v)[4]) {
+#pragma unroll
+                for (int q = 0; q < 4; q++)
+                    *reinterpret_cast<double2 *>(P + (4 * q + lrow) * CHM_S + lcol) = make_double2(-v[q].x, -v[q].y);
+            };
+            auto load_bq = [&](int k, double2 &v0, double2 &v1) {
+                const int r0 = min(kb + 8 * wave + lrow, F - 1), r1 = min(kb + 8 * wave + 4 + lrow, F - 1);
+                v0 = *reinterpret_cast<const double2 *>(Tl + (unsigned)(r0 * F + 32 * k + lcol));
+                v1 = *reinterpret_cast<const double2 *>(Tl + (unsigned)(r1 * F + 32 * k + lcol));
+            };
+            auto store_bq = [&](double *P, const double2 &v0, const double2 &v1) {
+                *reinterpret_cast<double2 *>(P + (8 * wave + lrow) * CHM_S + lcol) = v0;
+                *reinterpret_cast<double2 *>(P + (8 * wave + 4 + lrow) * CHM_S + lcol) = v1;
+            };
+            double2 va[4][4], vb0, vb1;
+#pragma unroll
+            for (int t = 0; t < 4; t++)
+                if (t < nt) load_strip(t, 0, va[t]);
+            load_bq(0, vb0, vb1);
+            for (int k = 0; k < j; k++) {
+                {
+                    const int fl = fresh_lane();
+                    lrow = fl >> 4, lcol = 2 * (fl & 15), ri = fl & 15, kq = fl >> 4;
+                }
+                double *PBc = PBS + (k & 1) * 32 * CHM_S;
+                store_bq(PBc, vb0, vb1);
+                __syncthreads();
+                if (k + 1 < j) load_bq(k + 1, vb0, vb1);
+#pragma unroll
+                for (int t = 0; t < 4; t++)
+                    if (t < nt) {
+                        double *P = PA + (t & 1) * 16 * CHM_S;
+                        store_strip(P, va[t]);
+                        if (k + 1 < j) load_strip(t, k + 1, va[t]);
+#pragma unroll
+                        for (int s = 0; s < 8; s++) {
+                            const double af = P[ri * CHM_S + 4 * s + kq];
+                            const double b0 = PBc[ri * CHM_S + 4 * s + kq], b1 = PBc[(16 + ri) * CHM_S + 4 * s + kq];
+                            acc[t][0] = __builtin_amdgcn_mfma_f64_16x16x4f64(af, b0, acc[t][0], 0, 0, 0);
+                            acc[t][1] = __builtin_amdgcn_mfma_f64_16x16x4f64(af, b1, acc[t][1], 0, 0, 0);
+                        }
+                    }
+            }
+        }
+        __syncthreads();
+#pragma unroll
+        for (int t = 0; t < 4; t++)
+            if (t < nt) {
+                const int fl = fresh_lane(), ri = fl & 15, kq = fl >> 4;
+                const int s = wave + 4 * t;
+#pragma unroll
+                for (int b = 0; b < 2; b++)
+#pragma unroll
+                    for (int r = 0; r < 4; r++) {
+                        if (s < 2) D[(16 * s + kq + 4 * r) * (CH_NB + 1) + 16 * b + ri] = acc[t][b][r];
+                        else PN[(16 * t + kq + 4 * r) * CHS_P + 16 * b + ri] = acc[t][b][r];
+                    }
+            }
+        init_acc(j + 1, acc);
+        CSTAMP(0);
+        __syncthreads();
+        CSTAMP(1);
+        if (wave == 0 && CHM_ABLATE != 1) {
+            auto bcast = [](double v, int src) {
+                const int lo = __builtin_amdgcn_readlane(__double2loint(v), src);
+                const int hi = __builtin_amdgcn_readlane(__double2hiint(v), src);
+                return __hiloint2double(hi, lo);
+            };
+            double row[CH_NB];
+#pragma unroll
+            for (int k = 0; k < CH_NB; k++) row[k] = (lane < nb && k <= lane) ? D[lane * (CH_NB + 1) + k] : 0.0;
+            bool bad = false;
+#pragma unroll
+            for (int jj = 0; jj < CH_NB; jj++) {
+                if (jj < nb && !bad) {
+                    const double d = bcast(row[jj], jj);
+                    if (!(d > 0.0)) {
+                        bad = true;
+                    } else {
+                        double y = __builtin_amdgcn_rsq(d);
+                        const double hd = 0.5 * d;
+                        y = fma(y, fma(-hd * y, y, 0.5), y);
+                        y = fma(y, fma(-hd * y, y, 0.5), y);
+                        const double lij = row[jj] * y;
+                        row[jj] = lij;
+                        if (lane == jj) rdiag[jj] = y;
+#pragma unroll
+                        for (int k = jj + 1; k < CH_NB; k++) row[k] = fma(-lij, bcast(lij, k), row[k]);
+                    }
+                }
+            }
+#pragma unroll
+            for (int k = 0; k < CH_NB; k++)
+                if (lane < nb && k <= lane) D[lane * (CH_NB + 1) + k] = row[k];
+            if (bad && lane == 0) *flag = 1;
+        }
+        CSTAMP(2);
+        __syncthreads();
+        CSTAMP(3);
+        if (*flag) break;
+        for (int q = tid; q < nb * nb; q += 256) {
+            const int i = q / nb, jj = q % nb;
+            Tl[(size_t)(kb + i) * F + kb + jj] = (jj <= i) ? D[i * (CH_NB + 1) + jj] : 0.0;
+        }
+        {
+            const int nz2 = (F - kb - 32) / 2;
+            for (int q = tid; q < 32 * nz2; q += 256) {
+                const int i = q / nz2, c = q % nz2;
+                *reinterpret_cast<double2 *>(Tl + (size_t)(kb + i) * F + kb + 32 + 2 * c) = make_double2(0.0, 0.0);
+            }
+        }
+        {
+            const int fl = fresh_lane();
+            const int s = wave + 4 * (fl >> 4);
+            if (s >= 2 && kb + 16 * s + (fl & 15) < F && CHM_ABLATE != 2) {
+                double x[CH_NB];
+                double *prow = PN + fl * CHS_P;
+#pragma unroll
+                for (int jj = 0; jj < CH_NB; jj++) x[jj] = prow[jj];
+#pragma unroll
+                for (int jj = 0; jj < CH_NB; jj++) {
+                    if (jj < nb) {
+                        double sm[4] = {x[jj], 0.0, 0.0, 0.0};
+#pragma unroll
+                        for (int pp = 0; pp < CH_NB; pp++)
+                            if (pp < jj) sm[pp & 3] = fma(-x[pp], D[jj * (CH_NB + 1) + pp], sm[pp & 3]);
+                        x[jj] = ((sm[0] + sm[1]) + (sm[2] + sm[3])) * rdiag[jj];
+                    }
+                }
+#pragma unroll
+                for (int jj = 0; jj < CH_NB; jj++) prow[jj] = x[jj];
+            }
+        }
+        __builtin_amdgcn_fence(__ATOMIC_RELEASE, "wavefront");
+        __builtin_amdgcn_wave_barrier();
+        __builtin_amdgcn_fence(__ATOMIC_ACQUIRE, "wavefront");
+#pragma unroll
+        for (int t = 0; t < 4; t++) {
+            const int s = wave + 4 * t;
+            if (t < nt && s >= 2) {
+                const int fl = fresh_lane(), lrow = fl >> 4, lcol = 2 * (fl & 15);
+#pragma unroll
+                for (int q = 0; q < 4; q++) {
+                    const int rl = 4 * q + lrow, rr = kb + 16 * s + rl;
+                    if (rr < F) {
+                        const double *pp = PN + (16 * t + rl) * CHS_P + lcol;
+                        *reinterpret_cast<double2 *>(Tl + (unsigned)(rr * F + kb + lcol)) = make_double2(pp[0], pp[1]);
+                    }
+                }
+            }
+        }
+        CSTAMP(4);
+        __syncthreads();
+        CSTAMP(5);
+    }
+    if (tid == 0) info[blockIdx.x] = *flag;
+#if CHM_STAMPS
+    if (lane == 0) {
+        for (int k = 0; k < 6; k++) atomicAdd(&g_chm_stamps[k], c_acc[k]);
+        atomicAdd(&g_chm_stamps[7], 1ull);
+    }
+#endif
+}
+
 __global__ void __launch_bounds__(256)
-chol_coop_kernel(const double *__restrict__ C, int F, double jitter_rel, double *T, int32_t *__restrict__ info, int mat0, int nrem,
+chol_coop_kernel(const double *__restrict__ C, int F, double jitter_rel, double *T, int32_t *__restrict__ info, int up, int mat0, int nrem,
                  int G, unsigned *bar, int *gflag, double *rd, int *xcc_min, int *xcc_max) {
     extern __shared__ __attribute__((aligned(16))) double lds[];
     double *D = lds;
@@ -493,6 +735,7 @@
     const size_t off = (size_t)(mat0 + mi) * F * F;
     const double *A = C + off;
     double *Tl = T + off;
+    const int a_sr = up ? 1 : F, a_sc = up ? F : 1;
     double *PA = stage + (size_t)wave * 2 * 32 * CHM_S, *PB = PA + 32 * CHM_S;
 
     double dmax = -INFINITY;
@@ -574,7 +817,7 @@
                     for (int r = 0; r < 4; r++) {
                         const int row = i0 + 16 * a + kq + 4 * r, col = kb + 16 * b + ri;
                         double v = 0.0;
-                        if (row < F && col <= row) v = A[(size_t)row * F + col] + (row == col ? jit : 0.0);
+                        if (row < F && col <= row) v = A[(unsigned)(row * a_sr + col * a_sc)] + (row == col ? jit : 0.0);
                         acc[a][b][r] = v;
                     }
             if (j > 0) {
@@ -708,7 +951,7 @@
 __global__ void __launch_bounds__(256)
 jacobi_root_kernel(const double *__restrict__ C, const int32_t *__restrict__ list, int F, double jitter_rel,
                    double eig_thresh, double *__restrict__ Wall, double *__restrict__ Vall,
-                   double *__restrict__ T) {
+                   double *__restrict__ T, int up) {
     extern __shared__ __attribute__((aligned(16))) double lds[];
     double *cs = lds;
     double *red = lds + 2 * (F / 2 + 1);
@@ -734,7 +977,7 @@
     __syncthreads();
     for (long q = tid; q < (long)F * F; q += 256) {
         const int i = (int)(q / F), j = (int)(q % F);
-        const double v = (j <= i) ? A[(size_t)i * F + j] : A[(size_t)j * F + i];
+        const double v = ((j <= i) != (up != 0)) ? A[(size_t)i * F + j] : A[(size_t)j * F + i];
         W[q] = v + (i == j ? jit : 0.0);
         V[q] = (i == j) ? 1.0 : 0.0;
     }
@@ -851,8 +1094,8 @@
     }
 }
 
-extern "C" int corahip_factor_batched(corahip_ctx *ctx, const double *C, int nl, int F, double jitter_rel,
-                                      double eig_thresh, double *T, int32_t *info) {
+static int factor_batched_impl(corahip_ctx *ctx, const double *C, int nl, int F, double jitter_rel, double eig_thresh, double *T,
+                               int32_t *info, int up) {
     ARG_CHECK(ctx != nullptr && C != nullptr && T != nullptr && info != nullptr);
     ARG_CHECK(nl >= 1 && F >= 1);
     StageTimer t(ctx, "factor");
@@ -881,7 +1124,7 @@
         const int nmain = nl - nrem;
         if (tall) {
             HIP_TRY(hipFuncSetAttribute((const void *)chol_ll_kernel<true>, hipFuncAttributeMaxDynamicSharedMemorySize, (int)shm));
-            if (nmain > 0) chol_ll_kernel<true><<<nmain, 256, shm, ctx->stream>>>(C, F, jitter_rel, T, info);
+            if (nmain > 0) chol_ll_kernel<true><<<nmain, 256, shm, ctx->stream>>>(C, F, jitter_rel, T, info, up);
             if (nrem > 0) {
                 void *ws = nullptr;
                 const size_t wsb = (size_t)nrem * (sizeof(unsigned) + 3 * sizeof(int) + CH_NB * sizeof(double)) + 64;
@@ -893,7 +1136,7 @@
                 int *gflag = reinterpret_cast<int *>(bar + nrem);
                 int *xmin = gflag + nrem, *xmax = xmin + nrem;
                 HIP_TRY(hipMemsetAsync(xmin, 0x7f, sizeof(int) * nrem, ctx->stream));
-                chol_coop_kernel<<<((nrem + 7) / 8) * 8 * G, 256, shm2, ctx->stream>>>(C, F, jitter_rel, T, info, nmain, nrem, G, bar, gflag, rd,
+                chol_coop_kernel<<<((nrem + 7) / 8) * 8 * G, 256, shm2, ctx->stream>>>(C, F, jitter_rel, T, info, up, nmain, nrem, G, bar, gflag, rd,
                                                                                      xmin, xmax);
                 if (getenv("CORAHIP_K2_COOP_DEBUG")) {
                     std::vector<int> hx(nrem);
@@ -904,9 +1147,13 @@
                     fprintf(stderr, "K2 cooperative kernel: %d matrices, %d workgroups each, %d groups on one XCC\n", nrem, G, same);
                 }
             }
+        } else if (F <= 256) {
+            const size_t shms = sizeof(double) * (CH_NB * (CH_NB + 1) + 256 + 2 + CH_NB + 4 * 64 * CHS_P) + 16;
+            HIP_TRY(hipFuncSetAttribute((const void *)chol_ls_kernel, hipFuncAttributeMaxDynamicSharedMemorySize, (int)shms));
+            chol_ls_kernel<<<nl, 256, shms, ctx->stream>>>(C, F, jitter_rel, T, info, up);
         } else {
             HIP_TRY(hipFuncSetAttribute((const void *)chol_ll_kernel<false>, hipFuncAttributeMaxDynamicSharedMemorySize, (int)shm));
-            chol_ll_kernel<false><<<nl, 256, shm, ctx->stream>>>(C, F, jitter_rel, T, info);
+            chol_ll_kernel<false><<<nl, 256, shm, ctx->stream>>>(C, F, jitter_rel, T, info, up);
         }
         LAUNCH_CHECK();
 #if CHM_STAMPS
@@ -922,7 +1169,7 @@
 #endif
     } else {
         const size_t shm = sizeof(double) * (CH_NB * (CH_NB + 1) + 2 * 64 * (CH_NB + 1) + 256) + 16;
-        chol_kernel<<<nl, 256, shm, ctx->stream>>>(C, F, jitter_rel, T, info);
+        chol_kernel<<<nl, 256, shm, ctx->stream>>>(C, F, jitter_rel, T, info, up);
         LAUNCH_CHECK();
     }
     std::vector<int32_t> hinfo(nl);
@@ -933,7 +1180,7 @@
         for (int l = 0; l < nl; l++)
             if (hinfo[l] == 3) {
                 const size_t shm = sizeof(double) * (CH_NB * (CH_NB + 1) + 256 + 2 + CH_NB + 6 * 32 * CHM_S) + 16;
-                chol_ll_kernel<true><<<1, 256, shm, ctx->stream>>>(C + (size_t)l * F * F, F, jitter_rel, T + (size_t)l * F * F, info + l);
+                chol_ll_kernel<true><<<1, 256, shm, ctx->stream>>>(C + (size_t)l * F * F, F, jitter_rel, T + (size_t)l * F * F, info + l, up);
                 LAUNCH_CHECK();
                 redo = true;
             }
@@ -957,7 +1204,7 @@
     for (size_t b0 = 0; b0 < list.size(); b0 += batch) {
         const int nb = (int)std::min(batch, list.size() - b0);
         jacobi_root_kernel<<<nb, 256, shm, ctx->stream>>>(C, dlist + b0, F, jitter_rel, eig_thresh, scratch,
-                                                         scratch + (size_t)nb * F * F, T);
+                                                         scratch + (size_t)nb * F * F, T, up);
         LAUNCH_CHECK();
     }
     HIP_TRY(hipStreamSynchronize(ctx->stream));
@@ -965,3 +1212,13 @@
     (void)hipFree(scratch);
     return 0;
 }
+
+extern "C" int corahip_factor_batched(corahip_ctx *ctx, const double *C, int nl, int F, double jitter_rel,
+                                      double eig_thresh, double *T, int32_t *info) {
+    return factor_batched_impl(ctx, C, nl, F, jitter_rel, eig_thresh, T, info, 0);
+}
+
+extern "C" int corahip_factor_batched_upper(corahip_ctx *ctx, const double *C, int nl, int F, double jitter_rel,
+                                            double eig_thresh, double *T, int32_t *info) {
+    return factor_batched_impl(ctx, C, nl, F, jitter_rel, eig_thresh, T, info, 1);
+}
diff --git a/cora_amd/parallel.py b/cora_amd/parallel.py
--- a/cora_amd/parallel.py
+++ b/cora_amd/parallel.py
@@ -362,11 +362,11 @@
             self._chan_idx = torch.as_tensor(self.channels, device=self.ctx.device)
         return self._chan_idx
 
-    def _clarray_local(self):
+    def _clarray_local(self, upper=False):
         ctx = self.ctx
         if self._sep is not None:
             return ctx.clarray_separable(self._sep[0], self._sep[1], self.F, self.zint, self.w)
-        return ctx.clarray_table21cm(*self._tabs, *self._k1, self.F, self.zint, self.w, self._lx)
+        return ctx.clarray_table21cm(*self._tabs, *self._k1, self.F, self.zint, self.w, self._lx, upper=upper)
 
     def _separable_factors(self):
         import torch
@@ -417,21 +417,22 @@
             N = self.emulate_world
             if self.pair_sharded:
                 slab = self._clarray_pairs(N - 1, N)
-                C = ctx.clarray_pairs_finish(slab.new_zeros((N,) + tuple(slab.shape[1:])), self.F, sp.l_hi - sp.l_lo)
+                C = ctx.clarray_pairs_finish(slab.new_zeros((N,) + tuple(slab.shape[1:])), self.F, sp.l_hi - sp.l_lo,
+                                             upper=True)
                 del C
             else:
-                self._clarray_local()
-            ctx.factor_batched(self._emu_C)
+                self._clarray_local(upper=True)
+            ctx.factor_batched(self._emu_C, upper=True)
             return self._emulated
         if not self.distributed:
-            T, info = ctx.factor_batched(self._clarray_local())
+            T, info = ctx.factor_batched(self._clarray_local(upper=True), upper=True)
             return T, info, False
         if self.pair_sharded:
             mine = exchange_pair_slabs(self._clarray_pairs(self.rank, self.world), sp)
-            T, info = ctx.factor_batched(ctx.clarray_pairs_finish(mine, self.F, sp.l_hi - sp.l_lo))
+            T, info = ctx.factor_batched(ctx.clarray_pairs_finish(mine, self.F, sp.l_hi - sp.l_lo, upper=True), upper=True)
             Tr, ia = exchange_factor_rows(T, info, sp)
             return Tr, ia, True
-        T, info = ctx.factor_batched(self._clarray_local())
+        T, info = ctx.factor_batched(self._clarray_local(upper=True), upper=True)
         Ta, ia = allgather_factors(T, info, sp)
         return Ta, ia, False
 
diff --git a/include/corahip.h b/include/corahip.h
--- a/include/corahip.h
+++ b/include/corahip.h
@@ -52,6 +52,14 @@
 int corahip_clarray_pairs_finish(corahip_ctx *ctx, const double *pairs_in, int F, int nranks, int l_stride,
                                  int nl, double *out);
 
+int corahip_clarray_table21cm_upper(corahip_ctx *ctx, const double *dd, const double *dv, const double *vv,
+                                    int nkperp, int nkpar, double kperpmin, double kperpmax, double kparmax,
+                                    const double *chi, const double *pfd, const double *f, const double *b,
+                                    int F, int zint, const double *w, const double *log10l, int nl,
+                                    double *out);
+int corahip_clarray_pairs_finish_upper(corahip_ctx *ctx, const double *pairs_in, int F, int nranks, int l_stride,
+                                       int nl, double *out);
+
 int corahip_clarray_tables_pin(corahip_ctx *ctx, const double *dd, const double *dv, const double *vv,
                                uint64_t generation);
 
@@ -68,6 +76,8 @@
 
 int corahip_factor_batched(corahip_ctx *ctx, const double *C, int nl, int F, double jitter_rel,
                            double eig_thresh, double *T, int32_t *info);
+int corahip_factor_batched_upper(corahip_ctx *ctx, const double *C, int nl, int F, double jitter_rel,
+                                 double eig_thresh, double *T, int32_t *info);
 
 int corahip_normals_philox(corahip_ctx *ctx, uint64_t seed, int lmax, int F, double *g);
 
```

Result: no change. 3203 (median of 6 runs) (+0.7%).
